# i2Nav-WHU/IC-GVINS

Measured on NVIDIA H100. Metric: frames/sec (KLT+BA) 1280x560 300-feat 10-KF window, higher is better.
Workload: dtype u8/int32 fixed point + f32 (KLT), f64 (BA)

## Files before the change

### ic_gvins_b200/_lib.py

```python
from __future__ import annotations

import ctypes as C
import os

_HERE = os.path.dirname(os.path.abspath(__file__))
LIB_PATH = os.path.join(_HERE, "libicgvins_b200_prof.so" if os.environ.get("ICG_LIB_VARIANT") == "prof" else "libicgvins_b200.so")

u8p = C.POINTER(C.c_uint8)
f32p = C.POINTER(C.c_float)
f64p = C.POINTER(C.c_double)
i32p = C.POINTER(C.c_int32)
vp = C.c_void_p

_lib = None


class IcgError(RuntimeError):
    pass


def lib() -> C.CDLL:
    global _lib
    if _lib is None:
        if not os.path.exists(LIB_PATH):
            raise IcgError(f"{LIB_PATH} not built: run `python -m ic_gvins_b200.build` (there is no CPU fallback)")
        _lib = C.CDLL(LIB_PATH, mode=C.RTLD_GLOBAL)
        _declare(_lib)
        _declare_r2(_lib)
    return _lib


def check(rc: int, what: str = "") -> None:
    if rc != 0:
        msg = lib().icg_last_error().decode("utf-8", "replace")
        raise IcgError(f"{what} failed with code {rc}: {msg}")


def _declare(L: C.CDLL) -> None:
    L.icg_last_error.restype = C.c_char_p
    L.icg_version.restype = C.c_int
    L.icg_launch_count.restype = C.c_uint64
    L.icg_launch_count_reset.restype = None
    L.icg_klt_create.argtypes = [C.POINTER(vp), C.c_int, C.c_int, C.c_int, C.c_int, C.c_int, vp]
    L.icg_klt_destroy.argtypes = [vp]
    L.icg_klt_destroy.restype = None
    L.icg_klt_calc_optical_flow_pyr_lk.argtypes = [vp, vp, vp, C.c_int, vp, vp, vp, vp, C.c_int, C.c_int, C.c_int, C.c_int,
                                                   C.c_double, C.c_int]
    L.icg_klt_track_fb.argtypes = [vp, vp, vp, C.c_int, vp, vp, vp, vp, C.c_int]
    L.icg_klt_upload.argtypes = [vp, C.c_int, vp, C.c_int]
    L.icg_klt_upload_level0.argtypes = [vp, C.c_int, vp, C.c_int]
    L.icg_klt_upload_batch.argtypes = [vp, C.c_int, C.c_int, vp, C.c_int]
    L.icg_klt_slot_level0.argtypes = [vp, C.c_int, C.POINTER(vp), C.POINTER(C.c_int)]
    L.icg_klt_slot_level.argtypes = [vp, C.c_int, C.c_int, C.POINTER(vp), C.POINTER(C.c_int), C.POINTER(C.c_int), C.POINTER(C.c_int)]
    L.icg_klt_build_pyramids.argtypes = [vp, C.c_int, C.c_int]
    L.icg_klt_track_batch_dev.argtypes = [vp, C.c_int, vp, vp, vp, vp, vp, vp, C.c_int]
    L.icg_klt_sync.argtypes = [vp]
    L.icg_klt_download_level.argtypes = [vp, C.c_int, C.c_int, vp, C.c_int]
    L.icg_detect_create.argtypes = [C.POINTER(vp), C.c_int, C.c_int, C.c_int, C.c_int, C.c_int, C.c_int, vp]
    L.icg_detect_destroy.argtypes = [vp]
    L.icg_detect_destroy.restype = None
    L.icg_detect_blocks.argtypes = [vp, vp, vp, C.c_int, C.c_int, vp, vp, C.c_double, C.c_double, C.c_int, vp, vp]
    L.icg_detect_blocks_dev.argtypes = [vp, C.c_int, vp, C.c_int, C.c_size_t, vp, C.c_int, vp, vp, C.c_double, C.c_double, C.c_int, vp, vp]
    L.icg_corner_subpix.argtypes = [vp, vp, C.c_int, vp, C.c_int]
    L.icg_detect_features.argtypes = [vp, vp, C.c_int, vp, C.c_int, vp, C.c_int, C.c_int, C.c_int, C.c_int, vp, vp]
    L.icg_detect_features_dev.argtypes = [vp, C.c_int, vp, C.c_int, C.c_size_t, vp, vp, vp, vp, vp, vp, vp, vp, C.c_int, vp, vp]
    L.icg_detect_mask_dev.argtypes = [vp, C.c_int, C.POINTER(vp), C.POINTER(C.c_int)]
    L.icg_camera_undistort_points.argtypes = [vp, vp, C.c_int]
    L.icg_camera_distort_points.argtypes = [vp, vp, C.c_int]
    L.icg_camera_distort_camera_points.argtypes = [vp, vp, vp, C.c_int]
    L.icg_camera_pixel2cam.argtypes = [vp, vp, vp, C.c_int]
    L.icg_camera_world2pixel.argtypes = [vp, vp, vp, vp, vp, C.c_int]
    L.icg_tracking_histogram.argtypes = [vp, C.c_int, C.c_int, C.c_int, vp]
    L.icg_triangulate_points.argtypes = [vp, vp, vp, vp, C.c_int, vp]
    L.icg_find_fundamental_mat_ransac.argtypes = [vp, vp, C.c_int, C.c_double, C.c_double, C.c_int, vp, vp]
    L.icg_clahe_create.argtypes = [C.POINTER(vp), C.c_int, C.c_int, C.c_int, C.c_int, C.c_double, C.c_int, vp]
    L.icg_clahe_destroy.argtypes = [vp]
    L.icg_clahe_destroy.restype = None
    L.icg_clahe_apply.argtypes = [vp, vp, C.c_int, vp, C.c_int]
    L.icg_clahe_apply_dev.argtypes = [vp, vp, C.c_int, vp, C.c_int]
    L.icg_clahe_sync.argtypes = [vp]
    L.icg_imu_preintegrate.argtypes = [vp, vp, vp, vp, vp, C.c_int, vp, vp]
    L.icg_ba_create.argtypes = [C.POINTER(vp), C.c_int, C.c_int, C.c_int, C.c_int, C.c_int, C.c_int, C.c_int, vp]
    L.icg_ba_destroy.argtypes = [vp]
    L.icg_ba_destroy.restype = None
    L.icg_ba_solve.argtypes = [vp, C.c_int, vp, C.c_int, vp]
    L.icg_ba_upload.argtypes = [vp, C.c_int, vp]
    L.icg_ba_run.argtypes = [vp, C.c_int, C.c_int]
    L.icg_ba_download.argtypes = [vp, C.c_int, vp, vp]
    L.icg_ba_sync.argtypes = [vp]
    L.icg_ba_shard_export.argtypes = [vp, C.c_int, C.c_int, vp]
    L.icg_ba_shard_connect.argtypes = [vp, vp]
    L.icg_ba_shard_error.argtypes = [vp]
    L.icg_ba_shard_leave.argtypes = [vp]
    L.icg_ba_gvins_optimization.argtypes = [vp, C.c_int, vp, C.c_int, vp, vp]
    L.icg_ba_run_gvins.argtypes = [vp, C.c_int, C.c_int]
    L.icg_ba_gvins_optimization_begin.argtypes = [vp, C.c_int, vp, C.c_int]
    L.icg_ba_gvins_optimization_end.argtypes = [vp, C.c_int, vp, vp, vp]
    L.icg_ba_residual_costs.argtypes = [vp, vp, vp, vp]
    L.icg_ba_reproj_evaluate.argtypes = [vp, vp, vp, vp, vp, vp, vp, C.c_double, vp, vp]
    L.icg_ba_imu_evaluate.argtypes = [vp, vp, vp, vp, vp, vp, vp, vp]
    L.icg_ba_marginalize.argtypes = [vp, C.c_int, vp, vp, vp]
    L.icg_ba_marginalize_resident.argtypes = [vp, C.c_int, vp, vp, vp]
    L.icg_ba_gnss_evaluate.argtypes = [vp, vp, vp, vp, vp, vp, vp]
    L.icg_ba_pose_prior_evaluate.argtypes = [vp, vp, vp, vp, vp, vp]
    L.icg_ba_mix_prior_evaluate.argtypes = [vp, vp, vp, vp, vp, vp]
    L.icg_ba_imu_error_evaluate.argtypes = [vp, vp, vp, vp]
    L.icg_ba_marg_factor_evaluate.argtypes = [vp, C.c_int, C.c_int, vp, vp, vp, vp, vp, vp, vp]


def _declare_r2(L: C.CDLL) -> None:
    L.icg_clahe_apply_batch_dev.argtypes = [vp, C.c_int, vp, C.c_int, C.c_size_t, vp, C.c_int, C.c_size_t, vp]
    L.icg_geom_create.argtypes = [C.POINTER(vp), C.c_int, vp]
    L.icg_geom_destroy.argtypes = [vp]
    L.icg_geom_destroy.restype = None
    L.icg_geom_undistort_points.argtypes = [vp, vp, vp, C.c_int]
    L.icg_geom_distort_points.argtypes = [vp, vp, vp, C.c_int]
    L.icg_geom_find_fundamental_mat_ransac.argtypes = [vp, vp, vp, C.c_int, C.c_double, C.c_double, C.c_int, vp, vp]
    L.icg_geom_triangulate_points.argtypes = [vp, vp, vp, vp, vp, C.c_int, vp]
    L.icg_geom_imu_preintegrate_batch.argtypes = [vp, C.c_int, vp, vp, vp, vp, vp, vp, vp, vp]
    L.icg_geom_find_fundamental_mat_ransac_batch.argtypes = [vp, C.c_int, vp, vp, vp, vp, vp, C.c_int, vp, vp, vp, vp]
    L.icg_klt_track_frames_dev.argtypes = [vp, C.c_int, vp, vp, vp, vp, vp, vp, vp, vp]
    L.icg_klt_track_frame.argtypes = [vp, vp, C.c_int, vp, C.c_int, vp, vp, vp, vp]
    L.icg_klt_triangulate_dev.argtypes = [vp, C.c_int, vp, vp, vp, vp, vp, C.c_int, vp, vp, vp]
    L.icg_klt_triangulate.argtypes = [vp, vp, C.c_int, vp, C.c_int, vp, vp, vp]
    L.icg_ba_update_and_cull_resident.argtypes = [vp, C.c_int, vp, vp, C.c_double, vp]
    L.icg_ba_marginalize_resident_culled.argtypes = [vp, C.c_int, vp, vp, vp, vp, vp]
    L.icg_ba_reintegrate_resident.argtypes = [vp, C.c_int, vp, vp, vp, vp]
    L.icg_ba_slide_resident.argtypes = [vp, C.c_int, vp, vp]
    L.icg_ba_slide_integrate_resident.argtypes = [vp, C.c_int, vp, vp, vp, vp, vp]


class SlideWindow(C.Structure):
    _fields_ = [("node_src", i32p), ("lm_src", i32p), ("f_src", i32p), ("imu_src", i32p), ("gnss_src", i32p), ("prior_from_marg", C.c_int32)]


SLIDE_CHAIN, SLIDE_ROW = -2, -3


class SlideIntegrate(C.Structure):
    _fields_ = [("imu_from", i32p), ("state16", f64p), ("gravity3", f64p), ("normal", u8p), ("imu", f64p), ("imu_off", i32p),
                ("node_from_imu", u8p), ("gnss_node", i32p), ("gnss_dt", f64p),
                ("status", C.POINTER(C.c_int8)), ("blob_out", f64p), ("end_state10", f64p)]


EXPORTS = [
    "icg_last_error", "icg_version", "icg_launch_count", "icg_launch_count_reset",
    "icg_klt_create", "icg_klt_destroy", "icg_klt_calc_optical_flow_pyr_lk", "icg_klt_track_fb", "icg_klt_upload",
    "icg_klt_upload_level0", "icg_klt_upload_batch", "icg_klt_slot_level0", "icg_klt_slot_level", "icg_klt_build_pyramids",
    "icg_klt_track_batch_dev", "icg_klt_sync", "icg_klt_download_level",
    "icg_detect_create", "icg_detect_destroy", "icg_detect_blocks", "icg_detect_blocks_dev", "icg_corner_subpix",
    "icg_detect_features", "icg_detect_features_dev", "icg_detect_mask_dev",
    "icg_camera_undistort_points", "icg_camera_distort_points", "icg_camera_distort_camera_points", "icg_camera_pixel2cam", "icg_camera_world2pixel", "icg_tracking_histogram", "icg_find_fundamental_mat_ransac", "icg_triangulate_points",
    "icg_clahe_create", "icg_clahe_destroy", "icg_clahe_apply", "icg_clahe_apply_dev", "icg_clahe_apply_batch_dev", "icg_geom_create", "icg_geom_destroy", "icg_geom_undistort_points", "icg_geom_distort_points", "icg_geom_find_fundamental_mat_ransac", "icg_geom_triangulate_points", "icg_geom_imu_preintegrate_batch", "icg_clahe_sync",
    "icg_geom_find_fundamental_mat_ransac_batch", "icg_klt_track_frames_dev", "icg_klt_track_frame",
    "icg_klt_triangulate_dev", "icg_klt_triangulate",
    "icg_imu_preintegrate", "icg_ba_create", "icg_ba_destroy", "icg_ba_solve", "icg_ba_upload", "icg_ba_run", "icg_ba_download",
    "icg_ba_sync", "icg_ba_shard_export", "icg_ba_shard_connect", "icg_ba_shard_error", "icg_ba_shard_leave", "icg_ba_gvins_optimization", "icg_ba_run_gvins", "icg_ba_gvins_optimization_begin", "icg_ba_gvins_optimization_end", "icg_ba_residual_costs", "icg_ba_reproj_evaluate", "icg_ba_imu_evaluate", "icg_ba_marginalize", "icg_ba_marginalize_resident", "icg_ba_update_and_cull_resident", "icg_ba_marginalize_resident_culled", "icg_ba_reintegrate_resident", "icg_ba_slide_resident", "icg_ba_slide_integrate_resident", "icg_ba_gnss_evaluate", "icg_ba_pose_prior_evaluate", "icg_ba_mix_prior_evaluate", "icg_ba_imu_error_evaluate", "icg_ba_marg_factor_evaluate",
]
```

### ic_gvins_b200/csrc/ba.cu

```cuda
#include <cooperative_groups.h>
#include <unistd.h>
#include <math.h>
#include <stdlib.h>
#include <string.h>

#include <algorithm>
#include <string>
#include <thread>
#include <vector>

#include "ba_cull.cuh"
#include "ba_slide.cuh"
#include "preint.cuh"
#include "ba_math.cuh"
#include "common.cuh"
#include "geom_core.cuh"

namespace icg {
using namespace bam;
namespace cg = cooperative_groups;

constexpr int BA_SPLIT_W = 4;
constexpr int BA_CHOL_NB = 8;
constexpr int BA_MARG_MAXB = 72;
constexpr int BA_MAX_NODES = 32;

struct BaCaps {
    int NW, K, L, F, G, R;
    int NCV, N, NS, NCA, RJ, LP, NVB;
    int GQ;
};

struct WinDims {
    int K, L, F, n_imu, n_gnss, marg_r, marg_nb;
    int ext_const, td_const, reproj_huber, gnss_huber, has_imu_error, has_pose_prior, has_mix_prior;
    double reproj_sinv;
};

struct LmState {
    double radius, decrease_factor, x_cost, x_norm, cand_cost, model_cost_change, step_norm, gmax, initial_cost;
    double cost_cam[2];
    int iter, n_success, n_invalid, done, need_lin, last_success, first, step_valid, fresh_lin, max_iter, chol_ok;
    int lin_buf;
};

struct ShardDev {
    int split;
    int PK, BS, RV;
    double *peer[8];
    size_t off_inbox, off_bcast, off_scal, off_flagA, off_flagB, off_flagC;
    double *redv;
    int *err;
    double *slm;
    int *slm_cnt;
};

struct BaDev {
    ShardDev S;
    WinDims *dims;
    LmState *st;
    double *pose, *mix, *ext, *rho;
    double *pose_c, *mix_c, *ext_c, *rho_c;
    double *pose_0, *mix_0, *ext_0, *rho_0;
    uint8_t *f_active_0;
    double *gnss_std_0;
    uint8_t *f_active;
    int *lm_off;
    int *lm_perm;
    int *vb_lm0;
    int *ref_nrun;
    int *f_meta_s;
    double *f_const_s;
    int *vis_ord;
    int *part_off, *pair_ro, *npairs;
    double *gpart;
    int *vis_cnt;
    double *Mp[2];
    double *AW[2];
    double *costf[2];
    double *hl[2], *gl[2];
    double *Hc[2], *gc[2];
    double *scale_l, *scale_c;
    double *Hs;
    double *visv;
    double *imu_blob, *imu_U;
    int *gnss_node;
    double *gnss_blh, *gnss_std, *lever;
    double *pose_prior, *pose_prior_sinfo, *mix_prior, *mix_prior_std;
    int *marg_type, *marg_node;
    double *marg_x0, *marg_H0, *marg_b0, *marg_c0;
    double *cost_part;
    double *red2;
    int rank, world;
    double *step_c, *step_l;
    double *Sglobal;
    unsigned long long *clk;
};

__device__ __forceinline__ double *lin_Mp(const BaCaps &C, const BaDev &D, int b, int w) { return D.Mp[b] + (size_t) w * C.K * (C.K - 1) * 210; }
__device__ __forceinline__ double *lin_AW(const BaCaps &C, const BaDev &D, int b, int w) { return D.AW[b] + (size_t) w * C.LP * C.NCA; }
__device__ __forceinline__ double *lin_costf(const BaCaps &C, const BaDev &D, int b, int w) { return D.costf[b] + (size_t) w * C.F; }
__device__ __forceinline__ double *lin_hl(const BaCaps &C, const BaDev &D, int b, int w) { return D.hl[b] + (size_t) w * C.L; }
__device__ __forceinline__ double *lin_gl(const BaCaps &C, const BaDev &D, int b, int w) { return D.gl[b] + (size_t) w * C.L; }
__device__ __forceinline__ double *lin_Hc(const BaCaps &C, const BaDev &D, int b, int w) { return D.Hc[b] + (size_t) w * C.NS * C.NS; }
__device__ __forceinline__ double *lin_gc(const BaCaps &C, const BaDev &D, int b, int w) { return D.gc[b] + (size_t) w * C.NS; }

__device__ __forceinline__ int col_pose(int k) { return 6 * k; }
__device__ __forceinline__ int col_ext(int K) { return 6 * K; }
__device__ __forceinline__ int col_td(int K) { return 6 * K + 6; }
__device__ __forceinline__ int col_mix(int K, int k) { return 6 * K + 7 + 9 * k; }

__device__ __forceinline__ int jc_off(int a) { return a < 18 ? (a / 6) * 12 + (a % 6) : 36 + 2 * (a - 18); }
__device__ __forceinline__ int jc_row1(int a) { return a < 18 ? 6 : 1; }
__device__ __forceinline__ int tri20(int la, int lb) {
    return la * 20 - la * (la - 1) / 2 + (lb - la);
}
__device__ __forceinline__ void dmma884(double &c0, double &c1, double a, double b) {
    asm volatile("mma.sync.aligned.m8n8k4.row.col.f64.f64.f64.f64 {%0,%1}, {%2}, {%3}, {%0,%1};" : "+d"(c0), "+d"(c1) : "d"(a), "d"(b));
}
constexpr int LV_LD = 45;
constexpr size_t LV_SMEM = sizeof(double) * (128 * LV_LD + (BA_MAX_NODES + 1) * NODE_FRAME_LD);
__global__ void __launch_bounds__(128, 4) ba_lin_vis(BaCaps C, BaDev D, int at_cand) {
    extern __shared__ double lv_sm[];
    __shared__ int s_ord[128], s_gbeg[BA_MAX_NODES], s_gend[BA_MAX_NODES], s_last, s_p0, s_np;
    double (*s_rec)[LV_LD] = (double (*)[LV_LD]) lv_sm;
    double (*s_frame)[NODE_FRAME_LD] = (double (*)[NODE_FRAME_LD]) (lv_sm + 128 * LV_LD);
    const int w = blockIdx.y;
    const LmState &st = D.st[w];
    if (st.done || !(at_cand ? st.step_valid : st.need_lin)) return;
    const int b = at_cand ? 1 - st.lin_buf : st.lin_buf;
    const double *pose = at_cand ? D.pose_c : D.pose, *xext = at_cand ? D.ext_c : D.ext, *rho = at_cand ? D.rho_c : D.rho;
    const int *vb = D.vb_lm0 + (size_t) w * C.NVB;
    if ((int) blockIdx.x >= vb[C.NVB - 1]) return;
    const WinDims dm = D.dims[w];
    const int tid = threadIdx.x;
    const int *off = D.lm_off + (size_t) w * (C.L + 1);
    const int pA = vb[blockIdx.x], pB = vb[blockIdx.x + 1];
    const int s0 = off[pA], nslot = off[pB] - s0;
    if (tid <= dm.K) node_frame(tid < dm.K ? pose + ((size_t) w * C.K + tid) * 7 : xext + (size_t) w * 8, s_frame[tid]);
    if (tid < BA_MAX_NODES) s_gbeg[tid] = s_gend[tid] = 0;
    if (tid == 0) s_np = 0;
    __syncthreads();
    if (tid < nslot) {
        const int q = s0 + tid;
        double r[2], Ji[12], Jj[12], Je[12], Jr[2], Jt[2], cost = 0;
        const int4 meta = ((const int4 *) D.f_meta_s)[(size_t) w * C.F + q];
        const int i = meta.y, j = meta.z, f = meta.w;
        if (D.f_active[(size_t) w * C.F + f] != 0) {
            const double *ext = xext + (size_t) w * 8;
            reproj_eval_frames(s_frame[i], s_frame[j], s_frame[dm.K], rho[(size_t) w * C.L + meta.x], ext[7],
                               D.f_const_s + ((size_t) w * C.F + q) * 14, dm.reproj_sinv, true, r, Ji, Jj, Je, Jr, Jt);
            if (dm.ext_const)
                for (int k = 0; k < 12; k++) Je[k] = 0;
            if (dm.td_const) Jt[0] = Jt[1] = 0;
            double sq = r[0] * r[0] + r[1] * r[1], sc = 1.0;
            if (dm.reproj_huber)
                huber(sq, cost, sc);
            else
                cost = 0.5 * sq;
            if (sc != 1.0) {
                for (int k = 0; k < 12; k++) Ji[k] *= sc, Jj[k] *= sc, Je[k] *= sc;
                Jr[0] *= sc, Jr[1] *= sc, Jt[0] *= sc, Jt[1] *= sc, r[0] *= sc, r[1] *= sc;
            }
        } else {
            for (int k = 0; k < 12; k++) Ji[k] = Jj[k] = Je[k] = 0;
            Jr[0] = Jr[1] = Jt[0] = Jt[1] = r[0] = r[1] = 0;
        }
        lin_costf(C, D, b, w)[f] = cost;
        double *sr = s_rec[tid];
#pragma unroll
        for (int k = 0; k < 12; k++) sr[k] = Ji[k], sr[12 + k] = Jj[k], sr[24 + k] = Je[k];
        sr[36] = Jt[0], sr[37] = Jt[1], sr[38] = r[0], sr[39] = r[1];
        sr[40] = Jr[0], sr[41] = Jr[1], sr[42] = (double) j, sr[43] = (double) i;
    }
    __syncthreads();
    const int lane = tid & 31, warp = tid >> 5;
    if (nslot > 0) {
        if (tid < nslot) {
            const int *ord = D.vis_ord + (size_t) w * C.F + s0;
            const int v = ord[tid], ob = (int) s_rec[v & 255][42];
            s_ord[tid] = v;
            if (tid == 0 || (int) s_rec[ord[tid - 1] & 255][42] != ob) s_gbeg[ob] = tid;
            if (tid == nslot - 1 || (int) s_rec[ord[tid + 1] & 255][42] != ob) s_gend[ob] = tid + 1;
        }
        __syncthreads();
        const int kk = lane & 3, g = lane >> 2;
        int o[3];
#pragma unroll
        for (int t = 0; t < 3; t++) {
            const int a = 8 * t + g;
            o[t] = a < 20 ? jc_off(a) + (kk & 1) * jc_row1(a) : -1;
        }
        for (int ob = warp; ob < dm.K; ob += 4) {
            const int beg = s_gbeg[ob], end = s_gend[ob];
            if (beg == end) continue;
            double c00[2] = {0, 0}, c01[2] = {0, 0}, c02[2] = {0, 0}, c11[2] = {0, 0}, c12[2] = {0, 0}, c22[2] = {0, 0};
            constexpr int UNR = 2;
            for (int base = beg; base < end; base += 2 * UNR) {
                double x[UNR][3];
#pragma unroll
                for (int u = 0; u < UNR; u++) {
                    const int q = base + 2 * u + (kk >> 1);
                    const bool ok = q < end;
                    const double *rec = s_rec[ok ? s_ord[q] & 255 : 0];
#pragma unroll
                    for (int t = 0; t < 3; t++) x[u][t] = (ok && o[t] >= 0) ? rec[o[t]] : 0.0;
                }
#pragma unroll
                for (int u = 0; u < UNR; u++) {
                    dmma884(c00[0], c00[1], x[u][0], x[u][0]);
                    dmma884(c01[0], c01[1], x[u][0], x[u][1]);
                    dmma884(c02[0], c02[1], x[u][0], x[u][2]);
                    dmma884(c11[0], c11[1], x[u][1], x[u][1]);
                    dmma884(c12[0], c12[1], x[u][1], x[u][2]);
                    dmma884(c22[0], c22[1], x[u][2], x[u][2]);
                }
            }
            double *pp = D.gpart + ((size_t) w * C.GQ + (s_ord[beg] >> 8)) * 210;
            auto put = [&](int ti, int tj, const double *c) {
#pragma unroll
                for (int e = 0; e < 2; e++) {
                    const int la = 8 * ti + g, lb = 8 * tj + 2 * kk + e;
                    if (la <= lb && lb < 20) pp[tri20(la, lb)] = c[e];
                }
            };
            put(0, 0, c00), put(0, 1, c01), put(0, 2, c02), put(1, 1, c11), put(1, 2, c12), put(2, 2, c22);
        }
        __threadfence();
    }
    const int *perm = D.lm_perm + (size_t) w * C.L;
    const int K = dm.K, NCV = 6 * K + 7, NCA = 4 * ((NCV + 1 + 3) / 4);
    const int grp = tid >> 3, sl = tid & 7;
    int o0[3], o1[3];
#pragma unroll
    for (int t = 0; t < 3; t++) {
        const int c = sl + 8 * t;
        o0[t] = c < 19 ? jc_off(c) : 38, o1[t] = c < 19 ? o0[t] + jc_row1(c) : 39;
    }
    for (int pl = pA + grp; pl < pB; pl += 16) {
        const int l = perm[pl], f0 = off[pl] - s0, nf = off[pl + 1] - off[pl];
        double *row = lin_AW(C, D, b, w) + (size_t) l * C.NCA;
        for (int c = sl; c < NCA; c += 8) row[c] = 0.0;
        __syncwarp(0xffu << (tid & 24));
        double acc[3] = {0, 0, 0};
        for (int q = 0; q < nf; q++) {
            const double *rec = s_rec[f0 + q];
            const double r0 = rec[40], r1 = rec[41];
            const int ob = (int) rec[42];
#pragma unroll
            for (int t = 0; t < 3; t++) {
                const int c = sl + 8 * t;
                if (c == 20) {
                    acc[t] += r0 * r0 + r1 * r1;
                } else if (c < 20) {
                    const double v = rec[o0[t]] * r0 + rec[o1[t]] * r1;
                    if (c >= 6 && c < 12)
                        row[col_pose(ob) + c - 6] = v;
                    else
                        acc[t] += v;
                }
            }
        }
        const int ref = nf > 0 ? (int) s_rec[f0][43] : 0;
#pragma unroll
        for (int t = 0; t < 3; t++) {
            const int c = sl + 8 * t;
            if (nf > 0) {
                if (c < 6) row[col_pose(ref) + c] = acc[t];
                else if (c >= 12 && c < 18) row[col_ext(K) + c - 12] = acc[t];
                else if (c == 18) row[col_td(K)] = acc[t];
            }
            if (c == 19) {
                row[NCV] = acc[t];
                lin_gl(C, D, b, w)[l] = acc[t];
            } else if (c == 20) {
                lin_hl(C, D, b, w)[l] = acc[t];
                if (st.first) D.scale_l[(size_t) w * C.L + l] = 1.0 / (1.0 + sqrt(acc[t]));
            }
        }
    }
    if (nslot == 0) return;
    const int rn = (int) s_rec[0][43];
    __syncthreads();
    if (tid == 0) s_last = atomicAdd(D.vis_cnt + (size_t) w * C.K + rn, 1) == D.ref_nrun[(size_t) w * C.K + rn] - 1;
    __syncthreads();
    if (!s_last) return;
    __threadfence();
    if (tid == 0) D.vis_cnt[(size_t) w * C.K + rn] = 0;
    const int PM = C.K * (C.K - 1), P = D.npairs[w];
    const int *pro = D.pair_ro + (size_t) w * PM, *poff = D.part_off + (size_t) w * (PM + 1);
    for (int p = tid; p < P; p += 128)
        if ((pro[p] >> 8) == rn) {
            atomicAdd(&s_np, 1);
            if (p == 0 || (pro[p - 1] >> 8) != rn) s_p0 = p;
        }
    __syncthreads();
    const double *part = D.gpart + (size_t) w * C.GQ * 210;
    double *Mp = lin_Mp(C, D, b, w);
    for (int p = s_p0 + warp; p < s_p0 + s_np; p += 4) {
        const int k0 = poff[p], k1 = poff[p + 1];
        double acc[7];
#pragma unroll
        for (int j = 0; j < 7; j++) acc[j] = lane + 32 * j < 210 ? __ldcg(part + (size_t) k0 * 210 + lane + 32 * j) : 0.0;
        for (int k = k0 + 1; k < k1; k++) {
            double v[7];
#pragma unroll
            for (int j = 0; j < 7; j++) v[j] = lane + 32 * j < 210 ? __ldcg(part + (size_t) k * 210 + lane + 32 * j) : 0.0;
#pragma unroll
            for (int j = 0; j < 7; j++) acc[j] += v[j];
        }
#pragma unroll
        for (int j = 0; j < 7; j++)
            if (lane + 32 * j < 210) Mp[(size_t) p * 210 + lane + 32 * j] = acc[j];
    }
}


__device__ __forceinline__ void gram2_slots(const BaCaps &C, const BaDev &D, int w, int K, short *s_slot) {
    const int PM = C.K * (C.K - 1), P = D.npairs[w];
    const int *pro = D.pair_ro + (size_t) w * PM;
    for (int e = threadIdx.x; e < K * K; e += blockDim.x) s_slot[e] = -1;
    __syncthreads();
    for (int p = threadIdx.x; p < P; p += blockDim.x) s_slot[(pro[p] >> 8) * K + (pro[p] & 255)] = (short) p;
    __syncthreads();
}
__device__ __forceinline__ double gram2_entry(const BaCaps &C, const BaDev &D, int buf, int w, int K, const short *s_slot, int A, int B) {
    const int P = D.npairs[w];
    const double *Mp = lin_Mp(C, D, buf, w);
    const int bA = A < 6 * K ? A / 6 : K, bB = B < 6 * K ? B / 6 : K;
    const int a = A - 6 * bA, b = B - 6 * bB;
    const int ga = 12 + a, gb = 12 + b;
    double sum = 0;
    if (bA == K) {
        const int idx = tri20(ga, gb);
        double s4[4] = {0, 0, 0, 0};
        int p = 0;
        for (; p + 16 <= P; p += 16) {
            double v[16];
#pragma unroll
            for (int u = 0; u < 16; u++) v[u] = Mp[(size_t) (p + u) * 210 + idx];
#pragma unroll
            for (int u = 0; u < 16; u++) s4[u & 3] += v[u];
        }
        for (; p < P; p++) s4[p & 3] += Mp[(size_t) p * 210 + idx];
        sum = (s4[0] + s4[1]) + (s4[2] + s4[3]);
    } else if (bB == K || bB == bA) {
        const int i1 = tri20(a, bB == K ? gb : b), i2 = tri20(6 + a, bB == K ? gb : 6 + b);
        for (int o0 = 0; o0 < K; o0 += 8) {
            double v1[8], v2[8];
#pragma unroll
            for (int u = 0; u < 8; u++) {
                const int o = o0 + u;
                const int p1 = o < K ? s_slot[bA * K + o] : -1, p2 = o < K ? s_slot[o * K + bA] : -1;
                v1[u] = p1 >= 0 ? Mp[(size_t) p1 * 210 + i1] : 0.0;
                v2[u] = p2 >= 0 ? Mp[(size_t) p2 * 210 + i2] : 0.0;
            }
#pragma unroll
            for (int u = 0; u < 8; u++) sum += v1[u], sum += v2[u];
        }
    } else {
        const int p1 = s_slot[bA * K + bB], p2 = s_slot[bB * K + bA];
        if (p1 >= 0) sum += Mp[(size_t) p1 * 210 + tri20(a, 6 + b)];
        if (p2 >= 0) sum += Mp[(size_t) p2 * 210 + tri20(b, 6 + a)];
    }
    return sum;
}

__device__ __forceinline__ double block_sum(double v, double *s_red);
__device__ __forceinline__ double block_max(double v, double *s_red);
__device__ __forceinline__ double *x_inbox(const BaDev &D, int peer, int w, int from);
__device__ __forceinline__ int tri_idx(int A, int B, int ncv);

__device__ __forceinline__ void schur_store(const BaCaps &C, const BaDev &D, int buf, int w, int K, const short *s_slot, int A, int B, double cw) {
    const int NCV = 6 * K + 7;
    if (A == NCV) return;
    const size_t e = (size_t) w * C.NS * C.NS + (size_t) B * C.NS + A;
    const double hc = !D.S.split && B < NCV ? lin_Hc(C, D, buf, w)[(size_t) B * C.NS + A] : 0.0;
    const double cj = gram2_entry(C, D, buf, w, K, s_slot, A, B);
    if (D.S.split) {
        double *P = x_inbox(D, w % D.world, w, D.rank);
        const int TRI = NCV * (NCV + 1) / 2;
        if (B < NCV) {
            P[tri_idx(A, B, NCV)] = cj - cw;
            if (A == B) P[TRI + A] = cj;
        } else {
            P[TRI + NCV + A] = cj;
            P[TRI + 2 * NCV + A] = cw;
        }
    } else {
        double *V = D.visv + (size_t) w * 3 * C.NCV;
        if (B < NCV) {
            D.Hs[e] = hc + (cj - cw);
            if (A == B) V[A] = cj;
        } else {
            V[NCV + A] = cj, V[2 * NCV + A] = cw;
        }
    }
}

__device__ __forceinline__ void schur_scalars(const BaCaps &C, const BaDev &D, int w, const WinDims &dm, double *s_red) {
    const int tid = threadIdx.x;
    double c = 0, q = 0, gm = 0;
    const double *costf = lin_costf(C, D, 0, w), *gl = lin_gl(C, D, 0, w);
    for (int f = tid; f < dm.F; f += 256) c += costf[f];
    for (int l = tid; l < dm.L; l += 256) {
        const double r = D.rho[(size_t) w * C.L + l];
        q += r * r;
        gm = fmax(gm, fabs(gl[l]));
    }
    c = block_sum(c, s_red);
    q = block_sum(q, s_red);
    gm = block_max(gm, s_red);
    if (tid != 0) return;
    const int NCV = 6 * dm.K + 7, TRI = NCV * (NCV + 1) / 2;
    double *P = x_inbox(D, w % D.world, w, D.rank);
    P[TRI + 3 * NCV] = c, P[TRI + 3 * NCV + 1] = q, P[TRI + 3 * NCV + 2] = gm;
}

constexpr int SCHUR_RCH = 80;
constexpr int SCHUR_PASS = 16;
__global__ void __cluster_dims__(BA_SPLIT_W, 1, 1) __launch_bounds__(256) ba_schur_dmma(BaCaps C, BaDev D, int ld) {
    extern __shared__ double sA[];
    __shared__ short s_slot[32 * 32];
    __shared__ double s_red[40];
    cg::cluster_group cluster = cg::this_cluster();
    const int w = blockIdx.y, split = blockIdx.x;
    const LmState &st = D.st[w];
    if (st.done) return;
    const WinDims dm = D.dims[w];
    const int NCV = 6 * dm.K + 7, NCA = 4 * ((NCV + 1 + 3) / 4);
    const int T2 = (NCA + 15) / 16, nsuper = T2 * (T2 + 1) / 2;
    const int tid = threadIdx.x, lane = tid & 31, warp = tid >> 5, g = lane >> 2, kk = lane & 3;
    double *sphi = sA + (size_t) SCHUR_RCH * ld;
    const int b = st.lin_buf;
    const double *A = lin_AW(C, D, b, w), *hl = lin_hl(C, D, b, w);
    const double radius = st.radius;
    const int nsteps = (dm.L + 3) / 4;
    const int r_beg = 4 * (int) ((long long) nsteps * split / BA_SPLIT_W), r_end = min(dm.L, 4 * (int) ((long long) nsteps * (split + 1) / BA_SPLIT_W));
    const int npass = (nsuper + SCHUR_PASS - 1) / SCHUR_PASS;
    gram2_slots(C, D, w, dm.K, s_slot);
    for (int pass = 0; pass < npass; pass++) {
        if (pass > 0) cluster.barrier_wait();
        int si[2], sj[2];
        bool on[2];
#pragma unroll
        for (int h2 = 0; h2 < 2; h2++) {
            const int su = (2 * pass + h2) * 8 + warp;
            on[h2] = su < nsuper;
            int a = 0, e = on[h2] ? su : 0;
            while (e >= T2 - a) e -= T2 - a, a++;
            si[h2] = a, sj[h2] = a + e;
        }
        double acc[2][4][2];
#pragma unroll
        for (int h2 = 0; h2 < 2; h2++)
#pragma unroll
            for (int q = 0; q < 4; q++) acc[h2][q][0] = acc[h2][q][1] = 0;
        for (int r0 = r_beg; r0 < r_end; r0 += SCHUR_RCH) {
            const int nr = min(SCHUR_RCH, r_end - r0), nr4 = (nr + 3) & ~3;
            __syncthreads();
            for (int rb = warp; rb < nr4; rb += 8 * 4) {
                double v[4][3];
#pragma unroll
                for (int u = 0; u < 4; u++) {
                    const int rr = rb + 8 * u;
#pragma unroll
                    for (int cchunk = 0; cchunk < 3; cchunk++) {
                        const int c = lane + 32 * cchunk;
                        v[u][cchunk] = (rr < nr && c < NCA) ? A[(size_t) (r0 + rr) * C.NCA + c] : 0.0;
                    }
                }
#pragma unroll
                for (int u = 0; u < 4; u++) {
                    const int rr = rb + 8 * u;
#pragma unroll
                    for (int cchunk = 0; cchunk < 3; cchunk++) {
                        const int c = lane + 32 * cchunk;
                        if (rr < nr4 && c < ld) sA[(size_t) rr * ld + c] = v[u][cchunk];
                    }
                }
                for (int c = lane + 96; c < ld; c += 32)
                    for (int u = 0; u < 4; u++) {
                        const int rr = rb + 8 * u;
                        if (rr < nr4) sA[(size_t) rr * ld + c] = (rr < nr && c < NCA) ? A[(size_t) (r0 + rr) * C.NCA + c] : 0.0;
                    }
            }
            for (int rr = tid; rr < nr4; rr += 256) {
                double ph = 0;
                if (rr < nr) {
                    const int l = r0 + rr;
                    const double sl = D.scale_l[(size_t) w * C.L + l], hs = sl * sl * hl[l];
                    ph = sl * sl / (hs + fmin(fmax(hs, 1e-6), 1e32) / radius);
                }
                sphi[rr] = ph;
            }
            __syncthreads();
            for (int ks = 0; ks < nr4 / 4; ks++) {
                const double *row = sA + (size_t) (4 * ks + kk) * ld;
                const double ph = sphi[4 * ks + kk];
#pragma unroll
                for (int h2 = 0; h2 < 2; h2++) {
                    if (!on[h2]) continue;
                    const double xb0 = row[16 * sj[h2] + g], xb1 = row[16 * sj[h2] + 8 + g];
                    const double a0 = row[16 * si[h2] + g] * ph, a1 = row[16 * si[h2] + 8 + g] * ph;
                    dmma884(acc[h2][0][0], acc[h2][0][1], a0, xb0);
                    dmma884(acc[h2][1][0], acc[h2][1][1], a0, xb1);
                    dmma884(acc[h2][2][0], acc[h2][2][1], a1, xb0);
                    dmma884(acc[h2][3][0], acc[h2][3][1], a1, xb1);
                }
            }
        }
        __syncthreads();
#pragma unroll
        for (int h2 = 0; h2 < 2; h2++) {
            if (!on[h2]) continue;
#pragma unroll
            for (int q = 0; q < 4; q++)
#pragma unroll
                for (int e = 0; e < 2; e++) sA[(h2 * 8 + warp) * 256 + 64 * q + 32 * e + lane] = acc[h2][q][e];
        }
        cluster.sync();
        const int nslot = min(SCHUR_PASS, nsuper - SCHUR_PASS * pass);
        double cw[SCHUR_PASS / BA_SPLIT_W];
#pragma unroll
        for (int j = 0; j < SCHUR_PASS / BA_SPLIT_W; j++) {
            const int sl = split + BA_SPLIT_W * j;
            double p[BA_SPLIT_W];
#pragma unroll
            for (int k = 0; k < BA_SPLIT_W; k++) p[k] = sl < nslot ? cluster.map_shared_rank(sA, k)[sl * 256 + tid] : 0.0;
            cw[j] = 0;
#pragma unroll
            for (int k = 0; k < BA_SPLIT_W; k++) cw[j] += p[k];
        }
        cluster.barrier_arrive();
        const int q = tid >> 6, r_in = 8 * (q >> 1) + ((tid & 31) >> 2), c_in = 8 * (q & 1) + 2 * (tid & 3) + ((tid >> 5) & 1);
#pragma unroll
        for (int j = 0; j < SCHUR_PASS / BA_SPLIT_W; j++) {
            const int sl = split + BA_SPLIT_W * j;
            if (sl >= nslot) break;
            int a = 0, e = SCHUR_PASS * pass + sl;
            while (e >= T2 - a) e -= T2 - a, a++;
            const int r = 16 * a + r_in, cc = 16 * (a + e) + c_in;
            if (r <= cc && cc <= NCV) schur_store(C, D, b, w, dm.K, s_slot, r, cc, cw[j]);
        }
    }
    if (split == 0 && D.S.split) schur_scalars(C, D, w, dm, s_red);
    cluster.barrier_wait();
}

constexpr double IMU_GB_STD = 7200 / 3600.0 * 3.14159265358979323846 / 180.0;
constexpr double IMU_AB_STD = 2.0e4 * 1.0e-5;

__device__ void imu_factor_warp(const double *blob, const double *U, const double *pose0, const double *mix0, const double *pose1,
                                const double *mix1, bool want_j, double *rw, double *Jw, int lane) {
    __shared__ ImuMid s_mid[16];
    double *raw_r = rw + 15;
    const int wslot = (threadIdx.x >> 5) & 15;
    if (want_j)
        for (int e = lane; e < 450; e += 32) Jw[e] = 0;
    __syncwarp();
    if (lane == 0) {
        ImuMid M;
        imu_residual_raw(blob, pose0, mix0, pose1, mix1, raw_r, M);
        if (want_j) imu_jacobian_raw(blob, M, Jw);
        s_mid[wslot] = M;
    }
    __syncwarp();
    if (want_j && lane < 30) {
        for (int i = 0; i < 15; i++) {
            double s = 0;
            for (int k = i; k < 15; k++) s += U[i * 15 + k] * Jw[k * 30 + lane];
            Jw[i * 30 + lane] = s;
        }
    }
    if (lane < 15) {
        double s = 0;
        for (int k = lane; k < 15; k++) s += U[lane * 15 + k] * raw_r[k];
        rw[lane] = s;
    }
    __syncwarp();
}

__device__ void marg_dx(const BaCaps &C, const BaDev &D, int w, const WinDims &dm, const double *pose, const double *mix, const double *ext, double *dx,
                        int *colmap, int tid, int nthreads) {
    const int *type = D.marg_type + (size_t) w * BA_MARG_MAXB, *node = D.marg_node + (size_t) w * BA_MARG_MAXB;
    const double *x0 = D.marg_x0 + (size_t) w * BA_MARG_MAXB * 9;
    if (tid == 0) {
        int col = 0, xo = 0;
        for (int b = 0; b < dm.marg_nb; b++) {
            int t = type[b], nd = node[b];
            if (t == 0 || t == 2) {
                const double *x = t == 0 ? pose + nd * 7 : ext;
                const double *xl = x0 + xo;
                Q dq = qmul(qinv(pose_q(xl)), pose_q(x));
                V3 a = 2.0 * qv(dq);
                if (dq.w < 0) a = -a;
                for (int k = 0; k < 3; k++) dx[col + k] = x[k] - xl[k];
                dx[col + 3] = a.x, dx[col + 4] = a.y, dx[col + 5] = a.z;
                int base = t == 0 ? col_pose(nd) : col_ext(dm.K);
                for (int k = 0; k < 6; k++) colmap[col + k] = (t == 2 && dm.ext_const) ? -1 : base + k;
                col += 6, xo += 7;
            } else if (t == 1) {
                for (int k = 0; k < 9; k++) dx[col + k] = mix[nd * 9 + k] - x0[xo + k], colmap[col + k] = col_mix(dm.K, nd) + k;
                col += 9, xo += 9;
            } else {
                dx[col] = ext[7] - x0[xo];
                colmap[col] = dm.td_const ? -1 : col_td(dm.K);
                col += 1, xo += 1;
            }
        }
    }
}

__device__ __forceinline__ void red_add(double *p, double v) { asm volatile("red.global.add.f64 [%0], %1;" ::"l"(p), "d"(v) : "memory"); }

__device__ double cam_factors(const BaCaps &C, const BaDev &D, int w, const WinDims &dm, const double *pose, const double *mix, const double *ext,
                              bool lin, int b, double *smem) {
// ... 672 lines not shown
    const LmState &st = D.st[w];
    if (st.done || !st.step_valid) return;
    const WinDims dm = D.dims[w];
    const double *pose = D.pose_c + (size_t) w * C.K * 7, *ext = D.ext_c + (size_t) w * 8, *rho = D.rho_c + (size_t) w * C.L;
    double *part = D.cost_part + (size_t) w * (nblk_vis + 1);
    const int q = blockIdx.x * 256 + threadIdx.x;
    __shared__ double s_frame[BA_MAX_NODES + 1][NODE_FRAME_LD];
    if ((int) threadIdx.x <= dm.K) node_frame((int) threadIdx.x < dm.K ? pose + threadIdx.x * 7 : ext, s_frame[threadIdx.x]);
    __syncthreads();
    double cost = 0;
    int4 meta = make_int4(0, 0, 0, 0);
    if (q < dm.F) meta = ((const int4 *) D.f_meta_s)[(size_t) w * C.F + q];
    if (q < dm.F && D.f_active[(size_t) w * C.F + meta.w]) {
        double r[2];
        reproj_eval_frames(s_frame[meta.y], s_frame[meta.z], s_frame[dm.K], rho[meta.x], ext[7], D.f_const_s + ((size_t) w * C.F + q) * 14, dm.reproj_sinv,
                           false, r, nullptr, nullptr, nullptr, nullptr, nullptr);
        double sq = r[0] * r[0] + r[1] * r[1], sc;
        if (dm.reproj_huber)
            huber(sq, cost, sc);
        else
            cost = 0.5 * sq;
    }
    cost = block_sum(cost, s_red);
    if (threadIdx.x == 0) part[blockIdx.x] = cost;
}

__global__ void __launch_bounds__(128) ba_accept(BaCaps C, BaDev D) {
    __shared__ int s_accept;
    __shared__ double s_camsq, s_rhosq;
    __shared__ double s_red[40];
    const int w = blockIdx.x, tid = threadIdx.x;
    LmState &st = D.st[w];
    if (st.done) return;
    const WinDims dm = D.dims[w];
    const double *R2 = D.red2 + (size_t) w * 4;
    {
        const double *pose = D.pose + (size_t) w * C.K * 7, *mix = D.mix + (size_t) w * C.K * 9, *ext = D.ext + (size_t) w * 8;
        double s = 0;
        for (int e = tid; e < dm.K * 7; e += 128) s += pose[e] * pose[e];
        for (int e = tid; e < dm.K * 9; e += 128) s += mix[e] * mix[e];
        if (tid < 7 && !dm.ext_const) s += ext[tid] * ext[tid];
        if (tid == 7 && !dm.td_const) s += ext[7] * ext[7];
        s = block_sum(s, s_red);
        double q = 0;
        for (int l = tid; l < dm.L; l += 128) q += D.rho[(size_t) w * C.L + l] * D.rho[(size_t) w * C.L + l];
        q = block_sum(q, s_red);
        if (tid == 0) s_camsq = s, s_rhosq = q;
    }
    extern __shared__ double s_warp[];
    const int lane = tid & 31, warp = tid >> 5, ngrp = (dm.F + 31) / 32;
    if (st.step_valid) {
        const double *costf = lin_costf(C, D, 1 - st.lin_buf, w);
        const int4 *meta = (const int4 *) D.f_meta_s + (size_t) w * C.F;
#pragma unroll 4
        for (int g = warp; g < ngrp; g += 4) {
            const int q = 32 * g + lane;
            double v = q < dm.F ? costf[meta[q].w] : 0.0;
            for (int o = 16; o > 0; o >>= 1) v += __shfl_down_sync(0xffffffffu, v, o);
            if (lane == 0) s_warp[g] = v;
        }
    }
    __syncthreads();
    if (tid == 0) {
        s_accept = 0;
        const double mcc = R2[0], sn = R2[1], nfin = R2[2];
        double cand = 0;
        if (st.step_valid) {
            for (int g0 = 0; g0 < ngrp; g0 += 8) {
                double t = 0;
                for (int k = 0; k < 8; k++) t += g0 + k < ngrp ? s_warp[g0 + k] : 0.0;
                cand += t;
            }
            cand += st.cost_cam[1 - st.lin_buf];
        }
        if (!st.chol_ok || nfin != 0.0 || !(mcc > 0.0)) {
            st.step_valid = 0;
            st.n_invalid++;
            if (st.n_invalid >= 5) st.done = 3;
            st.radius *= 0.5;
            st.last_success = 0;
        } else {
            st.n_invalid = 0;
            st.model_cost_change = mcc;
            st.step_norm = sqrt(sn);
            st.x_norm = sqrt(s_camsq + s_rhosq);
            st.cand_cost = cand;
            if (st.step_norm <= 1e-8 * (st.x_norm + 1e-8)) {
                st.done = 2;
            } else if (fabs(st.x_cost - cand) <= 1e-6 * st.x_cost) {
                st.done = 2;
            } else {
                const double rel = (st.x_cost - cand) / mcc;
                if (rel > 1e-3) {
                    s_accept = 1;
                    st.n_success++;
                    double t = 2.0 * rel - 1.0;
                    st.radius = fmin(1e16, st.radius / fmax(1.0 / 3.0, 1.0 - t * t * t));
                    st.decrease_factor = 2.0;
                    st.last_success = 1;
                    st.fresh_lin = 1;
                    st.lin_buf ^= 1;
                } else {
                    st.radius = st.radius / st.decrease_factor;
                    st.decrease_factor *= 2.0;
                    st.last_success = 0;
                    st.need_lin = 0;
                }
            }
        }
    }
    __syncthreads();
    if (!s_accept) return;
    double *pose = D.pose + (size_t) w * C.K * 7, *mix = D.mix + (size_t) w * C.K * 9, *ext = D.ext + (size_t) w * 8, *rho = D.rho + (size_t) w * C.L;
    const double *pose_c = D.pose_c + (size_t) w * C.K * 7, *mix_c = D.mix_c + (size_t) w * C.K * 9, *ext_c = D.ext_c + (size_t) w * 8, *rho_c = D.rho_c + (size_t) w * C.L;
    for (int e = tid; e < dm.K * 7; e += 128) pose[e] = pose_c[e];
    for (int e = tid; e < dm.K * 9; e += 128) mix[e] = mix_c[e];
    if (tid < 8) ext[tid] = ext_c[tid];
    for (int e = tid; e < dm.L; e += 128) rho[e] = rho_c[e];
}

__global__ void ba_reset_state(BaDev D, LmState *save, int n, int max_iter) {
    int w = blockIdx.x * blockDim.x + threadIdx.x;
    if (w >= n) return;
    if (save) save[w] = D.st[w];
    LmState st;
    memset(&st, 0, sizeof(st));
    st.radius = 1e4, st.decrease_factor = 2.0;
    st.need_lin = 1, st.fresh_lin = 1, st.first = 1, st.last_success = 1, st.max_iter = max_iter;
    D.st[w] = st;
}

__global__ void __launch_bounds__(128) ba_chi2_cull(BaCaps C, BaDev D, int *counters) {
    const int w = blockIdx.y;
    WinDims &dm = D.dims[w];
    const int t = blockIdx.x * 128 + threadIdx.x;
    const double *pose = D.pose + (size_t) w * C.K * 7, *ext = D.ext + (size_t) w * 8, *rho = D.rho + (size_t) w * C.L;
    int4 meta = make_int4(0, 0, 0, 0);
    if (t < dm.F) meta = ((const int4 *) D.f_meta_s)[(size_t) w * C.F + t];
    if (t < dm.F && D.f_active[(size_t) w * C.F + meta.w]) {
        double r[2];
        reproj_eval(pose + meta.y * 7, pose + meta.z * 7, ext, rho[meta.x], ext[7], D.f_const_s + ((size_t) w * C.F + t) * 14, dm.reproj_sinv, false, r, nullptr,
                    nullptr, nullptr, nullptr, nullptr);
        if ((r[0] * r[0] + r[1] * r[1]) > 5.991) {
            D.f_active[(size_t) w * C.F + meta.w] = 0;
            atomicAdd(&counters[2 * w], 1);
        }
    }
    if (t < dm.n_gnss) {
        double r[3];
        double *sd = D.gnss_std + ((size_t) w * C.G + t) * 3;
        gnss_eval(pose + D.gnss_node[(size_t) w * C.G + t] * 7, D.gnss_blh + ((size_t) w * C.G + t) * 3, sd, D.lever + (size_t) w * 3, false, r, nullptr);
        double chi2 = r[0] * r[0] + r[1] * r[1] + r[2] * r[2];
        if (chi2 > 7.815) {
            double sc = sqrt(chi2 / 7.815);
            sd[0] *= sc, sd[1] *= sc, sd[2] *= sc;
            atomicAdd(&counters[2 * w + 1], 1);
        }
    }
}
__global__ void ba_set_gnss_huber(BaDev D, int n, int v) {
    int w = blockIdx.x * blockDim.x + threadIdx.x;
    if (w < n) D.dims[w].gnss_huber = v;
}

__global__ void ba_residual_costs_kernel(BaCaps C, BaDev D, double *reproj_cost, double *gnss_cost) {
    const int w = 0;
    const WinDims dm = D.dims[w];
    const int t = blockIdx.x * blockDim.x + threadIdx.x;
    const double *pose = D.pose, *ext = D.ext, *rho = D.rho;
    if (t < dm.F) {
        double r[2];
        const int4 meta = ((const int4 *) D.f_meta_s)[t];
        reproj_eval(pose + meta.y * 7, pose + meta.z * 7, ext, rho[meta.x], ext[7], D.f_const_s + (size_t) t * 14, dm.reproj_sinv, false, r, nullptr, nullptr,
                    nullptr, nullptr, nullptr);
        reproj_cost[meta.w] = 0.5 * (r[0] * r[0] + r[1] * r[1]);
    }
    if (t < dm.n_gnss) {
        double r[3];
        gnss_eval(pose + D.gnss_node[t] * 7, D.gnss_blh + t * 3, D.gnss_std + t * 3, D.lever, false, r, nullptr);
        gnss_cost[t] = 0.5 * (r[0] * r[0] + r[1] * r[1] + r[2] * r[2]);
    }
}

__global__ void ba_reproj_eval_kernel(const double *in , double *out ) {
    double r[2], Ji[12], Jj[12], Je[12], Jr[2], Jt[2];
    reproj_eval(in, in + 7, in + 14, in[22], in[23], in + 24, 1.0 / in[38], true, r, Ji, Jj, Je, Jr, Jt);
    out[0] = r[0], out[1] = r[1];
    double *o = out + 2;
    const double *src[3] = {Ji, Jj, Je};
    for (int b = 0; b < 3; b++)
        for (int rr = 0; rr < 2; rr++) {
            for (int c = 0; c < 6; c++) o[b * 14 + rr * 7 + c] = src[b][rr * 6 + c];
            o[b * 14 + rr * 7 + 6] = 0.0;
        }
    o[42] = Jr[0], o[43] = Jr[1], o[44] = Jt[0], o[45] = Jt[1];
}

__global__ void ba_imu_eval_kernel(const double *blob, const double *U, const double *x , double *out ) {
    __shared__ double s_buf[480];
    imu_factor_warp(blob, U, x, x + 7, x + 16, x + 23, true, s_buf, s_buf + 30, threadIdx.x);
    for (int e = threadIdx.x; e < 15; e += 32) out[e] = s_buf[e];
    for (int e = threadIdx.x; e < 450; e += 32) out[15 + e] = s_buf[30 + e];
}

__global__ void ba_small_factor_eval_kernel(int kind, const double *in, double *out) {
    if (kind == 0) {
        gnss_eval(in, in + 7, in + 10, in + 13, true, out, out + 3);
    } else if (kind == 1) {
        pose_prior_eval(in, in + 7, in + 14, true, out, out + 6);
    } else if (kind == 2) {
        for (int k = 0; k < 9; k++) out[k] = (in[k] - in[9 + k]) / in[18 + k], out[9 + k] = 1.0 / in[18 + k];
    } else {
        for (int k = 0; k < 3; k++) {
            out[k] = in[3 + k] / IMU_GB_STD, out[3 + k] = in[6 + k] / IMU_AB_STD;
            out[6 + k] = 1.0 / IMU_GB_STD, out[9 + k] = 1.0 / IMU_AB_STD;
        }
    }
}

__global__ void ba_marg_factor_eval_kernel(const double *in, double *out) {
    extern __shared__ double s_dx[];
    const int r = (int) in[0], nb = (int) in[1];
    const double *types = in + 2;
    int tot = 0;
    for (int b = 0; b < nb; b++) tot += ((int) types[b] == 1) ? 9 : ((int) types[b] == 3) ? 1 : 7;
    const double *x = types + nb, *x0 = x + tot, *e0 = x0 + tot, *J0 = e0 + r;
    if (threadIdx.x == 0) {
        int col = 0, xo = 0;
        for (int b = 0; b < nb; b++) {
            const int t = (int) types[b];
            if (t == 0 || t == 2) {
                Q dq = qmul(qinv(pose_q(x0 + xo)), pose_q(x + xo));
                V3 a = 2.0 * qv(dq);
                if (dq.w < 0) a = -a;
                for (int k = 0; k < 3; k++) s_dx[col + k] = x[xo + k] - x0[xo + k];
                s_dx[col + 3] = a.x, s_dx[col + 4] = a.y, s_dx[col + 5] = a.z;
                col += 6, xo += 7;
            } else {
                const int g = t == 1 ? 9 : 1;
                for (int k = 0; k < g; k++) s_dx[col + k] = x[xo + k] - x0[xo + k];
                col += g, xo += g;
            }
        }
    }
    __syncthreads();
    for (int i = threadIdx.x; i < r; i += blockDim.x) {
        double sum = e0[i];
        for (int k = 0; k < r; k++) sum += J0[(size_t) i * r + k] * s_dx[k];
        out[i] = sum;
    }
}

}

#include "ba_split.cuh"
#include "ba_marg.cuh"

using namespace icg;

namespace {
bool host_imu_sqrt_info(const double *cov, double *U) {
    double work[675];
    return gc::imu_sqrt_info(cov, U, work);
}

template <typename T>
struct HostDev {
    T *h = nullptr, *d = nullptr;
    size_t n = 0;
    int alloc(size_t count) {
        n = count;
        if (cudaMallocHost(&h, sizeof(T) * count) != cudaSuccess) return ICG_ENOMEM;
        if (cudaMalloc(&d, sizeof(T) * count) != cudaSuccess) return ICG_ENOMEM;
        memset(h, 0, sizeof(T) * count);
        return ICG_OK;
    }
    void release() {
        if (h) cudaFreeHost(h);
        if (d) cudaFree(d);
        h = d = nullptr;
    }
    cudaError_t up(cudaStream_t s, size_t count = 0) { return cudaMemcpyAsync(d, h, sizeof(T) * (count ? count : n), cudaMemcpyHostToDevice, s); }
    cudaError_t down(cudaStream_t s, size_t count = 0) { return cudaMemcpyAsync(h, d, sizeof(T) * (count ? count : n), cudaMemcpyDeviceToHost, s); }
};
}

struct icg_ba {
    BaCaps C;
    BaDev D;
    int device = 0;
    cudaStream_t stream = nullptr;
    cudaStream_t stream_cam = nullptr;
    cudaEvent_t ev_fork = nullptr, ev_join = nullptr;
    bool own_stream = false;
    int nblk_vis = 0;
    int cur_windows = 0;
    size_t smem_cam, smem_solve, smem_schur;
    int ld_schur;
    int use_global_S;
    HostDev<WinDims> dims;
    HostDev<LmState> st;
    HostDev<double> pose, mix, ext, rho, imu_blob, imu_U, gnss_blh, gnss_std, lever, pose_prior, pose_prior_sinfo, mix_prior, mix_prior_std, marg_x0,
        marg_H0, marg_b0, marg_c0;
    HostDev<int> f_meta_s, vb_lm0, ref_nrun;
    HostDev<double> f_const_s;
    HostDev<int> lm_off, lm_perm, lm_fidx, gnss_node, marg_type, marg_node, part_off, pair_ro, vis_ord, npairs;
    HostDev<uint8_t> f_active;
    std::vector<void *> dev_only;
    HostDev<double> scratch;
    HostDev<LmState> st_save;
    HostDev<int> cull_counters;
    double *xbuf = nullptr;
    size_t xbuf_doubles = 0;
    int x_world = 0;
    void *ipc_opened[8] = {nullptr, nullptr, nullptr, nullptr, nullptr, nullptr, nullptr, nullptr};
    unsigned long long epoch = 0;
    size_t smem_solve_cam = 0, smem_step_lm = 0;
    bool solve_cam_dsm = false;
    size_t smem_solve_cam_dsm = 0;
    bool prof = false;
    std::vector<cudaEvent_t> prof_ev;
    std::vector<int> prof_tag;
    size_t prof_used = 0;
    int prof_skip = 1;
    double prof_ms[16] = {0};
    long prof_cnt[16] = {0};
    bool marg_ready = false;
    MargDev M{};
    int marg_nw = 0;
    int marg_cluster_ok = -1;
    HostDev<int> marg_map;
    HostDev<double> marg_oJ0, marg_oe0, marg_oHp, marg_obp;
    HostDev<uint8_t> marg_fmask;
    unsigned char *cull_h = nullptr, *cull_d = nullptr;
    size_t cull_cap = 0;
    unsigned char *reint_h = nullptr, *reint_d = nullptr;
    size_t reint_cap = 0;
    int marg_res_n = 0;
    std::vector<int> marg_res_m, marg_res_r, marg_res_nb;
    unsigned char *slide_h = nullptr, *slide_d = nullptr;
    size_t slide_cap = 0;
    double *slide_old = nullptr, *fc_alt = nullptr;
    cudaEvent_t slide_ev = nullptr;
};

extern "C" {
static void prof_collect(icg_ba *h);
static void prof_print(icg_ba *h);
}

static int dmalloc(icg_ba *h, double **p, size_t n) {
    if (cudaMalloc(p, sizeof(double) * n) != cudaSuccess) {
        set_error("icg_ba_create: cudaMalloc of %zu doubles failed", n);
        return ICG_ENOMEM;
    }
    cudaMemsetAsync(*p, 0, sizeof(double) * n, h->stream);
    h->dev_only.push_back(*p);
    return ICG_OK;
}

static int cam_threads(const icg_ba *h) { return h->D.world >= 4 ? CAM_THREADS : 160; }

extern "C" {
static int split_setup(icg_ba *h, int rank, int world);
static void split_release(icg_ba *h);

int icg_imu_preintegrate(const double *state16, const double *iewn3, const double *gravity3, const double *noise5, const double *imu, int n, double *blob,
                         double *end_state10) {
    if (!state16 || !gravity3 || !noise5 || !imu || !blob || n < 1) {
        set_error("icg_imu_preintegrate: bad arguments");
        return ICG_EINVAL;
    }
    gc::preintegrate_core(state16, iewn3, gravity3, noise5, imu, n, blob, end_state10);
    return ICG_OK;
}

static int ba_create_body(icg_ba *h, int max_windows, int max_K, int max_L, int max_F, int max_gnss, int max_marg_r, void *stream);

int icg_ba_create(icg_ba **out, int max_windows, int max_K, int max_L, int max_F, int max_gnss, int max_marg_r, int device, void *stream) {
    if (!out || max_windows < 1 || max_K < 2 || max_K > 32 || max_L < 0 || max_F < 0 || max_gnss < 0 || max_marg_r < 0) {
        set_error("icg_ba_create: bad arguments");
        return ICG_EINVAL;
    }
    int ndev = 0;
    if (cudaGetDeviceCount(&ndev) != cudaSuccess || ndev == 0) {
        set_error("icg_ba_create: no CUDA device (this library has no CPU fallback)");
        return ICG_ENODEVICE;
    }
    if (device < 0 || device >= ndev) {
        set_error("icg_ba_create: device %d out of range", device);
        return ICG_EINVAL;
    }
    ICG_CUDA(cudaSetDevice(device));
    cudaDeviceProp prop;
    ICG_CUDA(cudaGetDeviceProperties(&prop, device));
    if (prop.major != 9 || prop.minor != 0) {
        set_error("icg_ba_create: device is sm_%d%d; this library is built for sm_90a only", prop.major, prop.minor);
        return ICG_ENODEVICE;
    }
    icg_ba *h = new icg_ba();
    h->device = device;
    const int rc_init = ba_create_body(h, max_windows, max_K, max_L, max_F, max_gnss, max_marg_r, stream);
    if (rc_init != ICG_OK) {
        icg_ba_destroy(h);
        return rc_init;
    }
    *out = h;
    return ICG_OK;
}

static int ba_create_body(icg_ba *h, int max_windows, int max_K, int max_L, int max_F, int max_gnss, int max_marg_r, void *stream) {
    if (stream) {
        h->stream = (cudaStream_t) stream;
    } else {
        ICG_CUDA(cudaStreamCreateWithFlags(&h->stream, cudaStreamNonBlocking));
        h->own_stream = true;
    }
    {
        int prio_lo = 0, prio_hi = 0;
        ICG_CUDA(cudaDeviceGetStreamPriorityRange(&prio_lo, &prio_hi));
        ICG_CUDA(cudaStreamCreateWithPriority(&h->stream_cam, cudaStreamNonBlocking, prio_hi));
    }
    ICG_CUDA(cudaEventCreateWithFlags(&h->ev_fork, cudaEventDisableTiming));
    ICG_CUDA(cudaEventCreateWithFlags(&h->ev_join, cudaEventDisableTiming));
    h->prof = getenv("ICG_BA_PROFILE") != nullptr;
    if (h->prof) {
        double *ck = nullptr;
        if (dmalloc(h, &ck, 48) != ICG_OK) return ICG_ENOMEM;
        h->D.clk = (unsigned long long *) ck;
    }
    if (getenv("ICG_BA_PROFILE_SKIP")) h->prof_skip = atoi(getenv("ICG_BA_PROFILE_SKIP"));
    BaCaps &C = h->C;
    max_L = std::max(1, max_L), max_F = std::max(1, max_F);
    C.NW = max_windows, C.K = max_K, C.L = max_L, C.F = max_F, C.G = std::max(1, max_gnss), C.R = std::max(1, max_marg_r);
    C.NCV = 6 * max_K + 7, C.N = 15 * max_K + 7, C.NS = (C.N + 3) & ~3, C.NCA = 4 * ((C.NCV + 1 + 3) / 4);
    C.RJ = (2 * max_F + 31) & ~31, C.LP = (max_L + 31) & ~31;
    C.NVB = (max_F + 127 - max_K) / (128 - max_K) + max_L / 128 + 4 + max_K;
    C.GQ = std::max(1, std::min(max_F, (C.NVB - 2) * (max_K - 1)));
    h->nblk_vis = (max_F + 255) / 256;
    const size_t NW = max_windows;
#define HD(field, count)                                                       \
    if (h->field.alloc(count) != ICG_OK) {                                     \
        set_error("icg_ba_create: allocation of " #field " failed");           \
        return ICG_ENOMEM;                                                     \
    }
    HD(dims, NW) HD(st, NW) HD(pose, NW * C.K * 7) HD(mix, NW * C.K * 9) HD(ext, NW * 8) HD(rho, NW * C.L)
    HD(imu_blob, NW * C.K * ICG_IMU_BLOB_DOUBLES) HD(imu_U, NW * C.K * 225) HD(gnss_blh, NW * C.G * 3) HD(gnss_std, NW * C.G * 3) HD(lever, NW * 3)
    HD(pose_prior, NW * 7) HD(pose_prior_sinfo, NW * 6) HD(mix_prior, NW * 9) HD(mix_prior_std, NW * 9) HD(marg_x0, NW * BA_MARG_MAXB * 9)
    HD(marg_H0, NW * C.R * C.R) HD(marg_b0, NW * C.R) HD(marg_c0, NW)
    HD(lm_off, NW * (C.L + 1)) HD(lm_perm, NW * C.L) HD(lm_fidx, NW * C.F) HD(gnss_node, NW * C.G) HD(marg_type, NW * BA_MARG_MAXB) HD(marg_node, NW * BA_MARG_MAXB) HD(f_active, NW * C.F)
    HD(scratch, 1024) HD(st_save, NW) HD(cull_counters, 2 * NW) HD(f_meta_s, NW * C.F * 4) HD(vb_lm0, NW * C.NVB) HD(ref_nrun, NW * C.K) HD(f_const_s, NW * C.F * 14)
    HD(part_off, NW * ((size_t) C.K * (C.K - 1) + 1)) HD(pair_ro, NW * (size_t) C.K * (C.K - 1)) HD(vis_ord, NW * C.F) HD(npairs, NW)
#undef HD
    ICG_CUDA(cudaMemsetAsync(h->st.d, 0, sizeof(LmState) * NW, h->stream));
    BaDev &D = h->D;
    D.rank = 0, D.world = 1;
    D.dims = h->dims.d, D.st = h->st.d, D.pose = h->pose.d, D.mix = h->mix.d, D.ext = h->ext.d, D.rho = h->rho.d;
    D.f_active = h->f_active.d;
    D.part_off = h->part_off.d, D.pair_ro = h->pair_ro.d, D.vis_ord = h->vis_ord.d, D.npairs = h->npairs.d;
    D.f_meta_s = h->f_meta_s.d, D.vb_lm0 = h->vb_lm0.d, D.ref_nrun = h->ref_nrun.d, D.f_const_s = h->f_const_s.d;
    D.lm_off = h->lm_off.d, D.lm_perm = h->lm_perm.d, D.imu_blob = h->imu_blob.d, D.imu_U = h->imu_U.d;
    D.gnss_node = h->gnss_node.d, D.gnss_blh = h->gnss_blh.d, D.gnss_std = h->gnss_std.d, D.lever = h->lever.d;
    D.pose_prior = h->pose_prior.d, D.pose_prior_sinfo = h->pose_prior_sinfo.d, D.mix_prior = h->mix_prior.d, D.mix_prior_std = h->mix_prior_std.d;
    D.marg_type = h->marg_type.d, D.marg_node = h->marg_node.d, D.marg_x0 = h->marg_x0.d, D.marg_H0 = h->marg_H0.d, D.marg_b0 = h->marg_b0.d, D.marg_c0 = h->marg_c0.d;
    int rc = ICG_OK;
#define DM(field, count) \
    if (rc == ICG_OK) rc = dmalloc(h, &D.field, count);
    DM(pose_c, NW * C.K * 7) DM(mix_c, NW * C.K * 9) DM(ext_c, NW * 8) DM(rho_c, NW * C.L)
    DM(pose_0, NW * C.K * 7) DM(mix_0, NW * C.K * 9) DM(ext_0, NW * 8) DM(rho_0, NW * C.L)
    DM(AW[0], NW * C.NCA * C.LP) DM(Mp[0], NW * (size_t) C.K * (C.K - 1) * 210) DM(visv, NW * 3 * C.NCV)
    DM(gpart, NW * (size_t) C.GQ * 210) DM(costf[0], NW * C.F) DM(hl[0], NW * C.L) DM(gl[0], NW * C.L) DM(scale_l, NW * C.L) DM(scale_c, NW * C.NS)
    DM(Hc[0], NW * C.NS * C.NS) DM(gc[0], NW * C.NS) DM(Hs, NW * C.NS * C.NS) DM(cost_part, NW * (h->nblk_vis + 1)) DM(red2, NW * 4) DM(step_c, NW * C.NS) DM(step_l, NW * C.L)
#undef DM
    if (rc == ICG_OK) rc = dmalloc(h, &D.gnss_std_0, NW * C.G * 3);
    if (rc == ICG_OK) {
        double *cnt = nullptr;
        rc = dmalloc(h, &cnt, (NW * C.K + 1) / 2);
        D.vis_cnt = (int *) cnt;
    }
    if (rc == ICG_OK) {
        double *fa0 = nullptr;
        rc = dmalloc(h, &fa0, (NW * C.F + 7) / 8 + 1);
        D.f_active_0 = (uint8_t *) fa0;
    }
    if (rc != ICG_OK) return rc;
    h->smem_cam = sizeof(double) * ((size_t) C.K * 480 + (size_t) C.G * 24 + 48 + 16 + 2 * (size_t) C.R + 8) + sizeof(int) * (size_t) C.R + 64;
    size_t vec = sizeof(double) * (40 + 5 * (size_t) C.NS);
    size_t packed = sizeof(double) * ((size_t) (C.N + 1) * (C.N + 2) / 2);
    h->use_global_S = (vec + packed > 220 * 1024) ? 1 : 0;
    h->smem_solve = vec + (h->use_global_S ? 0 : packed);
    D.Sglobal = nullptr;
    memset(&D.S, 0, sizeof(D.S));
    if (h->use_global_S) {
        rc = split_setup(h, 0, 1);
        if (rc != ICG_OK) return rc;
    } else {
        ICG_CUDA(raise_dynamic_smem((const void *) ba_solve, (size_t) (h->smem_solve)));
    }
    h->ld_schur = 16 * ((C.NCA + 15) / 16) + 8;
    h->smem_schur = sizeof(double) * std::max((size_t) SCHUR_RCH * h->ld_schur + SCHUR_RCH, (size_t) SCHUR_PASS * 256);
    ICG_CUDA(raise_dynamic_smem((const void *) ba_schur_dmma, (size_t) (h->smem_schur)));
    ICG_CUDA(cudaFuncSetAttribute(ba_schur_dmma, cudaFuncAttributePreferredSharedMemoryCarveout, cudaSharedmemCarveoutMaxShared));
    ICG_CUDA(raise_dynamic_smem((const void *) ba_lin_cam, (size_t) (h->smem_cam)));
    ICG_CUDA(raise_dynamic_smem((const void *) ba_cost_cam, (size_t) (h->smem_cam)));
    ICG_CUDA(raise_dynamic_smem((const void *) ba_lin_vis, LV_SMEM));
    ICG_CUDA(cudaStreamSynchronize(h->stream));
    h->cur_windows = 0;
    return ICG_OK;
}

void icg_ba_destroy(icg_ba *h) {
    if (!h) return;
    cudaSetDevice(h->device);
    if (h->stream) cudaStreamSynchronize(h->stream);
    prof_collect(h);
    prof_print(h);
    for (cudaEvent_t e : h->prof_ev) cudaEventDestroy(e);
    h->dims.release(), h->st.release(), h->pose.release(), h->mix.release(), h->ext.release(), h->rho.release();
    h->imu_blob.release(), h->imu_U.release(), h->gnss_blh.release(), h->gnss_std.release(), h->lever.release(), h->pose_prior.release();
    h->pose_prior_sinfo.release(), h->mix_prior.release(), h->mix_prior_std.release(), h->marg_x0.release(), h->marg_H0.release(), h->marg_b0.release();
    h->marg_c0.release(), h->lm_off.release(), h->lm_perm.release(), h->lm_fidx.release(), h->gnss_node.release();
    h->f_meta_s.release(), h->vb_lm0.release(), h->ref_nrun.release(), h->f_const_s.release(), h->marg_type.release(), h->marg_node.release(), h->f_active.release(), h->scratch.release(), h->st_save.release(), h->cull_counters.release(), h->part_off.release(), h->pair_ro.release(), h->vis_ord.release(), h->npairs.release();
    split_release(h);
    if (h->marg_ready) h->marg_map.release(), h->marg_oJ0.release(), h->marg_oe0.release(), h->marg_oHp.release(), h->marg_obp.release(), h->marg_fmask.release();
    for (double *p : {h->M.H0, h->M.b0, h->M.G1, h->M.V1, h->M.lam1, h->M.Z})
        if (p) cudaFree(p);
    if (h->cull_h) cudaFreeHost(h->cull_h);
    if (h->cull_d) cudaFree(h->cull_d);
    if (h->reint_h) cudaFreeHost(h->reint_h);
    if (h->reint_d) cudaFree(h->reint_d);
    if (h->slide_h) cudaFreeHost(h->slide_h);
    if (h->slide_d) cudaFree(h->slide_d);
    if (h->slide_old) cudaFree(h->slide_old);
    if (h->fc_alt) cudaFree(h->fc_alt);
    if (h->slide_ev) cudaEventDestroy(h->slide_ev);
    for (void *p : h->dev_only) cudaFree(p);
    if (h->stream_cam) cudaStreamSynchronize(h->stream_cam), cudaStreamDestroy(h->stream_cam);
    if (h->ev_fork) cudaEventDestroy(h->ev_fork);
    if (h->ev_join) cudaEventDestroy(h->ev_join);
    if (h->own_stream && h->stream) cudaStreamDestroy(h->stream);
    delete h;
}

#define PK_FAIL(code, ...)                          \
    do {                                            \
        char eb_[512];                              \
        snprintf(eb_, sizeof(eb_), __VA_ARGS__);    \
        err = eb_;                                  \
        return code;                                \
    } while (0)
static int pack_window(icg_ba *h, int w, const icg_ba_problem &p, bool values, std::string &err) {
        const BaCaps &C = h->C;
        if (p.K < 2 || p.K > C.K || p.L < 0 || p.L > C.L || p.F < 0 || p.F > C.F || p.n_imu < 0 || p.n_imu > p.K - 1 || p.n_gnss < 0 || p.n_gnss > C.G ||
            p.marg_r < 0 || p.marg_r > C.R || p.marg_nblocks < 0 || p.marg_nblocks > 2 * C.K + 2 || !p.pose || !p.mix || !p.ext || (p.L > 0 && !p.invdepth) ||
            (p.F > 0 && (!p.f_lm || !p.f_ref || !p.f_obs || !p.f_const))) {
            PK_FAIL(ICG_EINVAL, "icg_ba_upload: window %d exceeds the handle's capacity or has null parameter arrays (K=%d L=%d F=%d gnss=%d marg_r=%d)", w, p.K, p.L, p.F,
                      p.n_gnss, p.marg_r);
        }
        WinDims &d = h->dims.h[w];
        d.K = p.K, d.L = p.L, d.F = p.F, d.n_imu = p.n_imu, d.n_gnss = p.n_gnss, d.marg_r = p.marg_r, d.marg_nb = p.marg_nblocks;
        d.ext_const = p.ext_const != 0, d.td_const = p.td_const != 0, d.reproj_huber = p.reproj_huber != 0, d.gnss_huber = p.gnss_huber != 0;
        d.has_imu_error = p.has_imu_error != 0, d.has_pose_prior = p.has_pose_prior != 0, d.has_mix_prior = p.has_mix_prior != 0;
        d.reproj_sinv = 1.0 / p.reproj_std;
        if (values) {
            memcpy(h->pose.h + (size_t) w * C.K * 7, p.pose, sizeof(double) * 7 * p.K);
            memcpy(h->mix.h + (size_t) w * C.K * 9, p.mix, sizeof(double) * 9 * p.K);
        }
        memcpy(h->ext.h + (size_t) w * 8, p.ext, sizeof(double) * 8);
        if (values && p.L > 0) memcpy(h->rho.h + (size_t) w * C.L, p.invdepth, sizeof(double) * p.L);
        for (int f = 0; f < p.F; f++) {
            if (p.f_lm[f] < 0 || p.f_lm[f] >= p.L || p.f_ref[f] < 0 || p.f_ref[f] >= p.K || p.f_obs[f] < 0 || p.f_obs[f] >= p.K || p.f_ref[f] == p.f_obs[f]) {
                PK_FAIL(ICG_EINVAL, "icg_ba_upload: window %d factor %d has invalid indices", w, f);
            }
        }
        std::vector<int> refof(p.L, -1);
        {
            std::vector<unsigned> seen((size_t) p.L, 0u);
            for (int f = 0; f < p.F; f++) {
                const int l = p.f_lm[f];
                if (refof[l] < 0) refof[l] = p.f_ref[f];
                if (refof[l] != p.f_ref[f] || (seen[l] >> p.f_obs[f]) & 1u) {
                    PK_FAIL(ICG_EINVAL, "icg_ba_upload: window %d factor %d: landmark %d has two reference nodes or two observations in node %d", w, f, l, p.f_obs[f]);
                }
                seen[l] |= 1u << p.f_obs[f];
            }
        }
        if (p.f_active)
            memcpy(h->f_active.h + (size_t) w * C.F, p.f_active, p.F);
        else
            memset(h->f_active.h + (size_t) w * C.F, 1, p.F);
        int *perm = h->lm_perm.h + (size_t) w * C.L;
        std::vector<int> pos_of(p.L);
        {
            std::vector<int> kcur(p.K + 2, 0);
            for (int l = 0; l < p.L; l++) kcur[(refof[l] < 0 ? p.K : refof[l]) + 1]++;
            for (int k = 0; k <= p.K; k++) kcur[k + 1] += kcur[k];
            for (int l = 0; l < p.L; l++) pos_of[l] = kcur[refof[l] < 0 ? p.K : refof[l]]++, perm[pos_of[l]] = l;
        }
        int *off = h->lm_off.h + (size_t) w * (C.L + 1), *fidx = h->lm_fidx.h + (size_t) w * C.F;
        for (int l = 0; l <= p.L; l++) off[l] = 0;
        for (int f = 0; f < p.F; f++) off[pos_of[p.f_lm[f]] + 1]++;
        for (int l = 0; l < p.L; l++) off[l + 1] += off[l];
        int *vbh = h->vb_lm0.h + (size_t) w * C.NVB, *meta = h->f_meta_s.h + (size_t) w * C.F * 4;
        int nrun = 0;
        {
            std::vector<int> cur(off, off + p.L);
            for (int f = 0; f < p.F; f++) fidx[cur[pos_of[p.f_lm[f]]]++] = f;
            int *nrun_of = h->ref_nrun.h + (size_t) w * C.K;
            for (int k = 0; k < C.K; k++) nrun_of[k] = 0;
            int l0 = 0;
            while (l0 < p.L) {
                const int ref = refof[perm[l0]];
                int l1 = l0;
                while (l1 < p.L && refof[perm[l1]] == ref && off[l1 + 1] - off[l0] <= 128) l1++;
                if (l1 == l0 || nrun >= C.NVB - 2) PK_FAIL(ICG_EINVAL, "icg_ba_upload: window %d: landmark %d has more than 128 factors or the run table overflows", w, perm[l0]);
                if (ref >= 0) nrun_of[ref]++;
                vbh[nrun++] = l0;
                l0 = l1;
            }
            vbh[nrun] = p.L;
            vbh[C.NVB - 1] = nrun;
            double *fcs = h->f_const_s.h + (size_t) w * C.F * 14;
            for (int q = 0; q < p.F; q++) {
                const int f = fidx[q];
                meta[4 * q] = p.f_lm[f], meta[4 * q + 1] = p.f_ref[f], meta[4 * q + 2] = p.f_obs[f], meta[4 * q + 3] = f;
                if (values) memcpy(fcs + (size_t) q * 14, p.f_const + (size_t) f * 14, sizeof(double) * 14);
            }
        }
        {
            const int PM = C.K * (C.K - 1);
            int *poff = h->part_off.h + (size_t) w * (PM + 1), *pro = h->pair_ro.h + (size_t) w * PM, *ord = h->vis_ord.h + (size_t) w * C.F;
            std::vector<int> slot((size_t) p.K * p.K, -1);
            for (int f = 0; f < p.F; f++) slot[(size_t) p.f_ref[f] * p.K + p.f_obs[f]] = 0;
            int P = 0;
            for (int key = 0; key < p.K * p.K; key++)
                if (slot[key] == 0) slot[key] = P, pro[P++] = ((key / p.K) << 8) | (key % p.K);
            std::vector<int> npart(P, 0);
            for (int r = 0; r < nrun; r++) {
                unsigned seen = 0u;
                for (int q = off[vbh[r]]; q < off[vbh[r + 1]]; q++) seen |= 1u << meta[4 * q + 2];
                for (int k = 0; k < p.K; k++)
                    if ((seen >> k) & 1u) npart[slot[(size_t) refof[perm[vbh[r]]] * p.K + k]]++;
            }
            poff[0] = 0;
            for (int i = 0; i < P; i++) poff[i + 1] = poff[i] + npart[i];
            std::vector<int> cur(poff, poff + P), start(p.K), pidx(p.K);
            for (int r = 0; r < nrun; r++) {
                const int a = off[vbh[r]], b = off[vbh[r + 1]];
                if (a == b) continue;
                const int ref = meta[4 * a + 1];
                std::fill(start.begin(), start.end(), 0);
                for (int q = a; q < b; q++) start[meta[4 * q + 2]]++;
                for (int k = 0, t = 0; k < p.K; k++) {
                    const int c = start[k];
                    start[k] = t, t += c;
                    if (c) pidx[k] = cur[slot[(size_t) ref * p.K + k]]++;
                }
                for (int q = a; q < b; q++) {
                    const int k = meta[4 * q + 2];
                    ord[a + start[k]++] = (q - a) | (pidx[k] << 8);
                }
            }
            h->npairs.h[w] = P;
        }
        for (int k = 0; values && k < p.n_imu; k++) {
            const double *b = p.imu_blob + (size_t) k * ICG_IMU_BLOB_DOUBLES;
            memcpy(h->imu_blob.h + ((size_t) w * C.K + k) * ICG_IMU_BLOB_DOUBLES, b, sizeof(double) * ICG_IMU_BLOB_DOUBLES);
            if (!host_imu_sqrt_info(b + 252, h->imu_U.h + ((size_t) w * C.K + k) * 225)) {
                PK_FAIL(ICG_EINVAL, "icg_ba_upload: window %d IMU factor %d has a non positive-definite covariance", w, k);
            }
        }
        for (int g = 0; g < p.n_gnss; g++) {
            if (p.gnss_node[g] < 0 || p.gnss_node[g] >= p.K) {
                PK_FAIL(ICG_EINVAL, "icg_ba_upload: window %d GNSS factor %d has an invalid node", w, g);
            }
            h->gnss_node.h[(size_t) w * C.G + g] = p.gnss_node[g];
        }
        if (values && p.n_gnss) {
            memcpy(h->gnss_blh.h + (size_t) w * C.G * 3, p.gnss_blh, sizeof(double) * 3 * p.n_gnss);
            memcpy(h->gnss_std.h + (size_t) w * C.G * 3, p.gnss_std, sizeof(double) * 3 * p.n_gnss);
        }
        memcpy(h->lever.h + (size_t) w * 3, p.lever, sizeof(double) * 3);
        if (p.has_pose_prior) {
            memcpy(h->pose_prior.h + (size_t) w * 7, p.pose_prior, sizeof(double) * 7);
            for (int k = 0; k < 6; k++) h->pose_prior_sinfo.h[(size_t) w * 6 + k] = 1.0 / p.pose_prior_std[k];
        }
        if (p.has_mix_prior) {
            memcpy(h->mix_prior.h + (size_t) w * 9, p.mix_prior, sizeof(double) * 9);
            memcpy(h->mix_prior_std.h + (size_t) w * 9, p.mix_prior_std, sizeof(double) * 9);
        }
        if (p.marg_r > 0) {
            const int r = p.marg_r;
            int tot = 0, cols = 0;
            for (int b = 0; b < p.marg_nblocks; b++) {
                int t = p.marg_block_type[b];
                if (t < 0 || t > 3 || ((t == 0 || t == 1) && (p.marg_block_node[b] < 0 || p.marg_block_node[b] >= p.K))) {
                    PK_FAIL(ICG_EINVAL, "icg_ba_upload: window %d marginalization block %d invalid", w, b);
                }
                tot += (t == 0 || t == 2) ? 7 : t == 1 ? 9 : 1;
                cols += (t == 0 || t == 2) ? 6 : t == 1 ? 9 : 1;
                h->marg_type.h[(size_t) w * BA_MARG_MAXB + b] = t;
                h->marg_node.h[(size_t) w * BA_MARG_MAXB + b] = p.marg_block_node[b];
            }
            if (cols != r || tot > BA_MARG_MAXB * 9) {
                PK_FAIL(ICG_EINVAL, "icg_ba_upload: window %d marginalization prior size mismatch (blocks give %d columns, marg_r=%d)", w, cols, r);
            }
            memcpy(h->marg_x0.h + (size_t) w * BA_MARG_MAXB * 9, p.marg_x0, sizeof(double) * tot);
            if (!values) return ICG_OK;
            double *H0 = h->marg_H0.h + (size_t) w * C.R * C.R, *b0 = h->marg_b0.h + (size_t) w * C.R;
            for (int i = 0; i < r; i++) {
                for (int j = i; j < r; j++) {
                    double s = 0;
                    for (int k = 0; k < r; k++) s += p.marg_J0[(size_t) k * r + i] * p.marg_J0[(size_t) k * r + j];
                    H0[(size_t) i * r + j] = H0[(size_t) j * r + i] = s;
                }
                double s = 0;
                for (int k = 0; k < r; k++) s += p.marg_J0[(size_t) k * r + i] * p.marg_e0[k];
                b0[i] = s;
            }
            double c0 = 0;
            for (int k = 0; k < r; k++) c0 += p.marg_e0[k] * p.marg_e0[k];
            h->marg_c0.h[w] = c0;
        }
            return ICG_OK;
}
#undef PK_FAIL

static int pack_windows(icg_ba *h, int n, const icg_ba_problem *P, bool values) {
    const int nthreads = std::max(1, std::min({n / 4, 16, (int) std::thread::hardware_concurrency()}));
    std::vector<int> rcs(nthreads, ICG_OK);
    std::vector<std::string> errs(nthreads);
    auto worker = [&](int t) {
        for (int w = t; w < n; w += nthreads) {
            const int rc = pack_window(h, w, P[w], values, errs[t]);
            if (rc != ICG_OK) {
                rcs[t] = rc;
                return;
            }
        }
    };
    std::vector<std::thread> th;
    for (int t = 1; t < nthreads; t++) th.emplace_back(worker, t);
    worker(0);
    for (auto &x : th) x.join();
    for (int t = 0; t < nthreads; t++)
        if (rcs[t] != ICG_OK) {
            set_error("%s", errs[t].c_str());
            return rcs[t];
        }
    return ICG_OK;
}

static int upload_structure(icg_ba *h, int n) {
    const BaCaps &C = h->C;
    cudaStream_t s = h->stream;
    const size_t nn = (size_t) n, PM = (size_t) C.K * (C.K - 1);
#define UP(field, stride) ICG_CUDA(h->field.up(s, nn * (size_t) (stride)))
    UP(dims, 1); UP(ext, 8);
    UP(f_active, C.F);
    UP(f_meta_s, C.F * 4); UP(vb_lm0, C.NVB); UP(lm_off, C.L + 1); UP(lm_perm, C.L); UP(ref_nrun, C.K); UP(part_off, PM + 1); UP(pair_ro, PM); UP(vis_ord, C.F);
    UP(npairs, 1); UP(gnss_node, C.G); UP(lever, 3);
    UP(pose_prior, 7); UP(pose_prior_sinfo, 6); UP(mix_prior, 9); UP(mix_prior_std, 9);
    UP(marg_type, BA_MARG_MAXB); UP(marg_node, BA_MARG_MAXB); UP(marg_x0, BA_MARG_MAXB * 9);
#undef UP
    return ICG_OK;
}

static int keep_pristine(icg_ba *h, int n) {
    const BaCaps &C = h->C;
    const BaDev &D = h->D;
    cudaStream_t s = h->stream;
    ICG_CUDA(cudaMemcpyAsync(D.pose_0, D.pose, sizeof(double) * (size_t) n * C.K * 7, cudaMemcpyDeviceToDevice, s));
    ICG_CUDA(cudaMemcpyAsync(D.mix_0, D.mix, sizeof(double) * (size_t) n * C.K * 9, cudaMemcpyDeviceToDevice, s));
    ICG_CUDA(cudaMemcpyAsync(D.ext_0, D.ext, sizeof(double) * (size_t) n * 8, cudaMemcpyDeviceToDevice, s));
    ICG_CUDA(cudaMemcpyAsync(D.rho_0, D.rho, sizeof(double) * (size_t) n * C.L, cudaMemcpyDeviceToDevice, s));
    ICG_CUDA(cudaMemcpyAsync(D.f_active_0, D.f_active, (size_t) n * C.F, cudaMemcpyDeviceToDevice, s));
    ICG_CUDA(cudaMemcpyAsync(D.gnss_std_0, D.gnss_std, sizeof(double) * (size_t) n * C.G * 3, cudaMemcpyDeviceToDevice, s));
    return ICG_OK;
}

int icg_ba_upload(icg_ba *h, int n, const icg_ba_problem *P) {
    if (!h || !P || n < 1 || n > h->C.NW) {
        set_error("icg_ba_upload: bad arguments (n=%d, capacity %d)", n, h ? h->C.NW : 0);
        return ICG_EINVAL;
    }
    ICG_CUDA(cudaSetDevice(h->device));
    const BaCaps &C = h->C;
    h->marg_res_n = 0;
    int rc = pack_windows(h, n, P, true);
    if (rc != ICG_OK) return rc;
    rc = upload_structure(h, n);
    if (rc != ICG_OK) return rc;
    cudaStream_t s = h->stream;
    const size_t nn = (size_t) n;
#define UP(field, stride) ICG_CUDA(h->field.up(s, nn * (size_t) (stride)))
    UP(pose, C.K * 7); UP(mix, C.K * 9); UP(rho, C.L); UP(f_const_s, C.F * 14); UP(imu_blob, C.K * ICG_IMU_BLOB_DOUBLES); UP(imu_U, C.K * 225);
    UP(gnss_blh, C.G * 3); UP(gnss_std, C.G * 3); UP(marg_H0, (size_t) C.R * C.R); UP(marg_b0, C.R); UP(marg_c0, 1);
#undef UP
    rc = keep_pristine(h, n);
    if (rc != ICG_OK) return rc;
    h->cur_windows = n;
    return ICG_OK;
}

static const char *PROF_NAMES[16] = {"(gap/other)", "lin_vis", "lin_lm", "lin at candidate", "","schur_dmma (+ epilogue)", "join lin_cam + lin_done",
                                     "signal", "solve", "cost (+cost_cam)", "exchange", "accept", "reduce", "join gram chain", "step_lm", ""};
static void prof_mark(icg_ba *h, int tag) {
    if (!h->prof) return;
    if (h->prof_used == h->prof_ev.size()) {
        cudaEvent_t e;
        cudaEventCreate(&e);
        h->prof_ev.push_back(e);
        h->prof_tag.push_back(0);
    }
    h->prof_tag[h->prof_used] = tag;
    cudaEventRecord(h->prof_ev[h->prof_used++], h->stream);
}
static void prof_collect(icg_ba *h) {
    if (!h->prof) return;
    if (h->prof_used && h->prof_skip > 0) {
        h->prof_skip--;
        h->prof_used = 0;
        return;
    }
    for (size_t i = 1; i < h->prof_used; i++) {
        float ms = 0;
        if (cudaEventElapsedTime(&ms, h->prof_ev[i - 1], h->prof_ev[i]) == cudaSuccess) {
            h->prof_ms[h->prof_tag[i]] += ms;
            h->prof_cnt[h->prof_tag[i]]++;
        }
    }
    h->prof_used = 0;
}
static void prof_print(icg_ba *h) {
    if (!h->prof) return;
    double tot = 0;
    for (int t = 0; t < 16; t++) tot += h->prof_ms[t];
    fprintf(stderr, "[icg_ba profile] handle %p, %d windows: stage totals over all recorded LM sequences (ms, mean us, share)\n", (void *) h, h->cur_windows);
    for (int t = 0; t < 16; t++)
        if (h->prof_cnt[t])
            fprintf(stderr, "  %-28s %9.3f ms  %8.1f us  %5.1f %%\n", PROF_NAMES[t], h->prof_ms[t], 1e3 * h->prof_ms[t] / h->prof_cnt[t], 100.0 * h->prof_ms[t] / tot);
    if (h->D.clk) {
        unsigned long long ck[48];
        if (cudaMemcpy(ck, h->D.clk, sizeof(ck), cudaMemcpyDeviceToHost) == cudaSuccess) {
            static const char *cn[6] = {"factor evaluation", "prior product + cost", "zero H_c", "prior blocks", "IMU J^T J", "GNSS / prior diagonals"};
            fprintf(stderr, "[icg_ba profile] ba_lin_cam phases of window 0 (SM cycles per call, mean):\n");
            for (int k = 0; k < 6; k++)
                if (ck[24 + k]) fprintf(stderr, "  %-28s %9.0f cycles\n", cn[k], (double) ck[16 + k] / (double) ck[24 + k]);
            if (h->D.S.split) {
                static const char *sn_l2[6] = {"per panel: stage B operand", "per panel: warp 0 tile + factor", "per panel: tiles + barrier 1", "per panel: row solve + barrier 2", "whole factorisation", ""};
                static const char *sn_dsm[6] = {"assembly", "per panel: warp 0 tile + factor", "per panel: until block barrier", "per panel: row solve + cl. barrier", "whole factorisation", "backward substitution"};
                const char **sn = h->solve_cam_dsm ? sn_dsm : sn_l2;
                fprintf(stderr, "[icg_ba profile] %s phases of window 0 (SM cycles, mean):\n", h->solve_cam_dsm ? "ba_solve_cam_dsm" : "ba_solve_cam");
                for (int k = 0; k < 6; k++)
                    if (ck[8 + k]) fprintf(stderr, "  %-34s %9.0f cycles\n", sn[k], (double) ck[k] / (double) ck[8 + k]);
                static const char *sn2[5] = {"(unused)", "(unused)", "per panel: warp 0 diagonal-tile update", "per panel: warp 0 loads + 8x8 factorisation", "per panel: warp 0 write-back"};
                for (int k = 0; k < 5 && h->solve_cam_dsm; k++)
                    if (ck[40 + k]) fprintf(stderr, "  %-50s %9.0f cycles\n", sn2[k], (double) ck[32 + k] / (double) ck[40 + k]);
            }
            static const char *nm[8] = {"gradient / cost / tests", "assembly", "Cholesky", "camera back-substitution", "landmark back-substitution", "candidate + reductions",
                                        "  per panel: warp 0 tile+factor", "  per panel: row solve phase"};
            if (!h->D.S.split) fprintf(stderr, "[icg_ba profile] ba_solve phases of window 0 (SM cycles per call, mean):\n");
            for (int k = 0; k < 8 && !h->D.S.split; k++)
                if (ck[8 + k]) fprintf(stderr, "  %-28s %9.0f cycles\n", nm[k], (double) ck[k] / (double) ck[8 + k]);
        }
    }
}

static int enqueue_lm_split(icg_ba *h, int max_num_iterations);

static int alloc_lin_buf2(icg_ba *h) {
    BaDev &D = h->D;
    if (D.Mp[1]) return ICG_OK;
    const BaCaps &C = h->C;
    const size_t NW = C.NW;
    int rc = ICG_OK;
#define DM(field, count) \
    if (rc == ICG_OK) rc = dmalloc(h, &D.field, count);
    DM(AW[1], NW * C.NCA * C.LP) DM(Mp[1], NW * (size_t) C.K * (C.K - 1) * 210) DM(costf[1], NW * C.F) DM(hl[1], NW * C.L) DM(gl[1], NW * C.L)
    DM(Hc[1], NW * C.NS * C.NS) DM(gc[1], NW * C.NS)
#undef DM
    return rc;
}

static int enqueue_lm(icg_ba *h, int max_num_iterations) {
    if (h->D.S.split) return enqueue_lm_split(h, max_num_iterations);
    int rc = alloc_lin_buf2(h);
    if (rc != ICG_OK) return rc;
    const BaCaps &C = h->C;
    const BaDev &D = h->D;
    const int n = h->cur_windows;
    cudaStream_t s = h->stream;
    const dim3 g_vis(C.NVB - 2, n);
    auto enqueue_lin = [&](int at_cand) -> int {
        ICG_CUDA(cudaEventRecord(h->ev_fork, s));
        ICG_CUDA(cudaStreamWaitEvent(h->stream_cam, h->ev_fork, 0));
        ba_lin_cam<<<n, cam_threads(h), h->smem_cam, h->stream_cam>>>(C, D, at_cand);
        ICG_CUDA(cudaEventRecord(h->ev_join, h->stream_cam));
        prof_mark(h, 0);
        ba_lin_vis<<<g_vis, 128, LV_SMEM, s>>>(C, D, at_cand);
        prof_mark(h, at_cand ? 3 : 1);
        ICG_CUDA(cudaStreamWaitEvent(s, h->ev_join, 0));
        prof_mark(h, at_cand ? 3 : 6);
        count_launch(2);
        return ICG_OK;
    };
    rc = enqueue_lin(0);
    if (rc != ICG_OK) return rc;
    for (int it = 0; it <= max_num_iterations; it++) {
        ba_schur_dmma<<<dim3(BA_SPLIT_W, n), 256, h->smem_schur, s>>>(C, D, h->ld_schur);
        prof_mark(h, 5);
        ba_solve<<<n, SOLVE_THREADS, h->smem_solve, s>>>(C, D);
        prof_mark(h, 8);
        count_launch(2);
        if (it == max_num_iterations) break;
        rc = enqueue_lin(1);
        if (rc != ICG_OK) return rc;
        ba_accept<<<n, 128, sizeof(double) * 8 * h->nblk_vis, s>>>(C, D);
        prof_mark(h, 11);
        count_launch();
    }
    ICG_CHECK_LAUNCH();
    return ICG_OK;
}

static void split_release(icg_ba *h) {
    for (int r = 0; r < 8; r++)
        if (h->ipc_opened[r]) cudaIpcCloseMemHandle(h->ipc_opened[r]), h->ipc_opened[r] = nullptr;
    if (h->xbuf) cudaFree(h->xbuf), h->xbuf = nullptr;
    if (h->D.S.redv) cudaFree(h->D.S.redv), h->D.S.redv = nullptr;
    if (h->D.S.err) cudaFree(h->D.S.err), h->D.S.err = nullptr;
    if (h->D.S.slm) cudaFree(h->D.S.slm), h->D.S.slm = nullptr;
    if (h->D.S.slm_cnt) cudaFree(h->D.S.slm_cnt), h->D.S.slm_cnt = nullptr;
    if (h->D.Sglobal) cudaFree(h->D.Sglobal), h->D.Sglobal = nullptr;
    h->D.S.split = 0;
}

static int split_setup(icg_ba *h, int rank, int world) {
    if (world < 1 || world > 8 || rank < 0 || rank >= world) {
        set_error("split pipeline: rank %d / world %d out of range (<= 8 GPUs of one box)", rank, world);
        return ICG_EINVAL;
    }
    ICG_CUDA(cudaSetDevice(h->device));
    ICG_CUDA(cudaStreamSynchronize(h->stream));
    split_release(h);
    const BaCaps &C = h->C;
    ShardDev &S = h->D.S;
    const size_t NW = C.NW, G = world;
    const size_t TRI = (size_t) C.NCV * (C.NCV + 1) / 2;
    S.PK = (int) ((TRI + 3 * (size_t) C.NCV + 4 + 3) & ~(size_t) 3);
    S.BS = (SPLIT_HDR + C.NS + 3) & ~3;
    S.RV = (3 * C.NCV + 4 + 3) & ~3;
    const size_t NWo = (NW + G - 1) / G;
    size_t off = 0;
    S.off_inbox = off, off += NWo * G * S.PK;
    S.off_bcast = off, off += NW * S.BS;
    S.off_scal = off, off += NW * G * SPLIT_SCAL;
    S.off_flagA = off, off += 8;
    S.off_flagB = off, off += (NW + 3) & ~(size_t) 3;
    S.off_flagC = off, off += (NW * G + 3) & ~(size_t) 3;
    h->xbuf_doubles = off;
    if (cudaMalloc(&h->xbuf, sizeof(double) * off) != cudaSuccess || cudaMalloc(&S.redv, sizeof(double) * NW * S.RV) != cudaSuccess ||
        cudaMalloc(&S.err, sizeof(int) * 4) != cudaSuccess || cudaMalloc(&S.slm, sizeof(double) * NW * STEP_SLICES * 8) != cudaSuccess ||
        cudaMalloc(&S.slm_cnt, sizeof(int) * NW) != cudaSuccess ||
        cudaMalloc(&h->D.Sglobal, sizeof(double) * NWo * split_S_stride(C)) != cudaSuccess) {
        set_error("split pipeline: allocation of the exchange buffers failed (%zu doubles)", off);
        return ICG_ENOMEM;
    }
    ICG_CUDA(cudaMemset(h->xbuf, 0, sizeof(double) * off));
    ICG_CUDA(cudaMemset(S.redv, 0, sizeof(double) * NW * S.RV));
    ICG_CUDA(cudaMemset(S.err, 0, sizeof(int) * 4));
    ICG_CUDA(cudaMemset(S.slm, 0, sizeof(double) * NW * STEP_SLICES * 8));
    ICG_CUDA(cudaMemset(S.slm_cnt, 0, sizeof(int) * NW));
    for (int r = 0; r < 8; r++) S.peer[r] = nullptr;
    S.peer[rank] = h->xbuf;
    S.split = 1;
    h->D.rank = rank, h->D.world = world;
    h->x_world = world;
    h->epoch = 0;
    {
        const size_t ldbp = ((size_t) (C.N + 15) / 16) * 16 + 8;
        const size_t bs = (size_t) SPLIT_BS_ROWS * (C.NS + 1), base = 8 * ldbp + 64;
        h->smem_solve_cam = sizeof(double) * (40 + 4 * (size_t) C.NS + std::max(bs, base));
    }
    h->smem_step_lm = sizeof(double) * (40 + (size_t) C.NS);
    h->smem_solve_cam_dsm = sizeof(double) * dsm_smem_doubles(C);
    h->solve_cam_dsm = h->smem_solve_cam_dsm <= 227 * 1024 && C.N <= 32 * 11;
    if (h->solve_cam_dsm) ICG_CUDA(raise_dynamic_smem((const void *) ba_solve_cam_dsm, h->smem_solve_cam_dsm));
    ICG_CUDA(raise_dynamic_smem((const void *) ba_solve_cam, (size_t) (h->smem_solve_cam)));
    ICG_CUDA(cudaFuncSetAttribute(ba_solve_cam, cudaFuncAttributeNonPortableClusterSizeAllowed, 0));
    ICG_CUDA(raise_dynamic_smem((const void *) ba_step_lm, (size_t) (h->smem_step_lm)));
    return ICG_OK;
}

static int launch_solve_cam(icg_ba *h, int n, unsigned long long epoch) {
    cudaLaunchConfig_t cfg;
    memset(&cfg, 0, sizeof(cfg));
    cfg.gridDim = dim3((unsigned) (n * SPLIT_CLUSTER)), cfg.blockDim = dim3(SOLVE_THREADS);
    cfg.dynamicSmemBytes = h->solve_cam_dsm ? h->smem_solve_cam_dsm : h->smem_solve_cam, cfg.stream = h->stream;
    cudaLaunchAttribute at[1];
    at[0].id = cudaLaunchAttributeClusterDimension;
    at[0].val.clusterDim.x = SPLIT_CLUSTER, at[0].val.clusterDim.y = 1, at[0].val.clusterDim.z = 1;
    cfg.attrs = at, cfg.numAttrs = 1;
    if (h->solve_cam_dsm) ICG_CUDA(cudaLaunchKernelEx(&cfg, ba_solve_cam_dsm, h->C, h->D, epoch));
    else ICG_CUDA(cudaLaunchKernelEx(&cfg, ba_solve_cam, h->C, h->D, epoch));
    return ICG_OK;
}

static int enqueue_lm_split(icg_ba *h, int max_num_iterations) {
    const BaCaps &C = h->C;
    const BaDev &D = h->D;
    const int n = h->cur_windows;
    cudaStream_t s = h->stream;
    for (int r = 0; r < D.world; r++)
        if (!D.S.peer[r]) {
            set_error("landmark-sharded solve: peer %d is not connected (icg_ba_shard_connect)", r);
            return ICG_EINVAL;
        }
    const dim3 g_vis(C.NVB - 2, n), g_cost(h->nblk_vis, n), g_nn(((C.NCV + 1) * (C.NCV + 1) + 255) / 256, n);
    for (int it = 0; it <= max_num_iterations; it++) {
        const unsigned long long epoch = ++h->epoch;
        ICG_CUDA(cudaEventRecord(h->ev_fork, s));
        ICG_CUDA(cudaStreamWaitEvent(h->stream_cam, h->ev_fork, 0));
        ba_lin_cam<<<n, cam_threads(h), h->smem_cam, h->stream_cam>>>(C, D, 0);
        ICG_CUDA(cudaEventRecord(h->ev_join, h->stream_cam));
        prof_mark(h, 0);
        ba_lin_vis<<<g_vis, 128, LV_SMEM, s>>>(C, D, 0);
        prof_mark(h, 1);
        ba_schur_dmma<<<dim3(BA_SPLIT_W, n), 256, h->smem_schur, s>>>(C, D, h->ld_schur);
        prof_mark(h, 5);
        ba_signal<<<1, 32, 0, s>>>(D, epoch);
        prof_mark(h, 7);
        ICG_CUDA(cudaStreamWaitEvent(s, h->ev_join, 0));
        prof_mark(h, 6);
        ba_reduce<<<g_nn, 256, 0, s>>>(C, D, epoch);
        prof_mark(h, 12);
        int rc = launch_solve_cam(h, n, epoch);
        if (rc != ICG_OK) return rc;
        prof_mark(h, 8);
        ba_step_lm<<<dim3(n, STEP_SLICES), SOLVE_THREADS, h->smem_step_lm, s>>>(C, D, epoch);
        prof_mark(h, 14);
        count_launch(7);
        if (it == max_num_iterations) break;
        ICG_CUDA(cudaEventRecord(h->ev_fork, s));
        ICG_CUDA(cudaStreamWaitEvent(h->stream_cam, h->ev_fork, 0));
        ba_cost_cam<<<n, cam_threads(h), h->smem_cam, h->stream_cam>>>(C, D, h->nblk_vis);
        ICG_CUDA(cudaEventRecord(h->ev_join, h->stream_cam));
        ba_cost<<<g_cost, 256, 0, s>>>(C, D, h->nblk_vis);
        ICG_CUDA(cudaStreamWaitEvent(s, h->ev_join, 0));
        prof_mark(h, 9);
        ba_exchange<<<(n + 63) / 64, 64, 0, s>>>(C, D, n, h->nblk_vis, epoch);
        prof_mark(h, 10);
        ba_accept_split<<<n, 128, 0, s>>>(C, D, epoch);
        prof_mark(h, 11);
        count_launch(4);
    }
    ICG_CHECK_LAUNCH();
    return ICG_OK;
}

static int restore_params(icg_ba *h) {
    const BaCaps &C = h->C;
    const BaDev &D = h->D;
    const int n = h->cur_windows;
    cudaStream_t s = h->stream;
    ICG_CUDA(cudaMemcpyAsync(D.pose, D.pose_0, sizeof(double) * (size_t) n * C.K * 7, cudaMemcpyDeviceToDevice, s));
    ICG_CUDA(cudaMemcpyAsync(D.mix, D.mix_0, sizeof(double) * (size_t) n * C.K * 9, cudaMemcpyDeviceToDevice, s));
    ICG_CUDA(cudaMemcpyAsync(D.ext, D.ext_0, sizeof(double) * (size_t) n * 8, cudaMemcpyDeviceToDevice, s));
    ICG_CUDA(cudaMemcpyAsync(D.rho, D.rho_0, sizeof(double) * (size_t) n * C.L, cudaMemcpyDeviceToDevice, s));
    ICG_CUDA(cudaMemcpyAsync(D.f_active, D.f_active_0, (size_t) n * C.F, cudaMemcpyDeviceToDevice, s));
    ICG_CUDA(cudaMemcpyAsync(D.gnss_std, D.gnss_std_0, sizeof(double) * (size_t) n * C.G * 3, cudaMemcpyDeviceToDevice, s));
    ICG_CUDA(h->dims.up(s, n));
    return ICG_OK;
}

int icg_ba_run(icg_ba *h, int max_num_iterations, int restart) {
    if (!h || h->cur_windows < 1 || max_num_iterations < 0) {
        set_error("icg_ba_run: no problems uploaded");
        return ICG_EINVAL;
    }
    ICG_CUDA(cudaSetDevice(h->device));
    const int n = h->cur_windows;
    if (restart) {
        int rc = restore_params(h);
        if (rc != ICG_OK) return rc;
    }
    ba_reset_state<<<(n + 127) / 128, 128, 0, h->stream>>>(h->D, nullptr, n, max_num_iterations);
    count_launch();
    return enqueue_lm(h, max_num_iterations);
}

int icg_ba_run_gvins(icg_ba *h, int num_iterations, int restart) {
    if (!h || h->cur_windows < 1 || num_iterations < 1) {
        set_error("icg_ba_run_gvins: no problems uploaded");
        return ICG_EINVAL;
    }
    ICG_CUDA(cudaSetDevice(h->device));
    const BaCaps &C = h->C;
    const int n = h->cur_windows;
    const int first = num_iterations / 4, second = num_iterations - first;
    if (restart) {
        int rc = restore_params(h);
        if (rc != ICG_OK) return rc;
    }
    cudaStream_t s = h->stream;
    ba_set_gnss_huber<<<(n + 127) / 128, 128, 0, s>>>(h->D, n, 1);
    ba_reset_state<<<(n + 127) / 128, 128, 0, s>>>(h->D, nullptr, n, first);
    count_launch(2);
    int rc = enqueue_lm(h, first);
    if (rc != ICG_OK) return rc;
    ICG_CUDA(cudaMemsetAsync(h->cull_counters.d, 0, sizeof(int) * 2 * (size_t) n, s));
    const dim3 g_cull((std::max(C.F, C.G) + 127) / 128, n);
    ba_chi2_cull<<<g_cull, 128, 0, s>>>(C, h->D, h->cull_counters.d);
    ba_set_gnss_huber<<<(n + 127) / 128, 128, 0, s>>>(h->D, n, 0);
    ba_reset_state<<<(n + 127) / 128, 128, 0, s>>>(h->D, h->st_save.d, n, second);
    count_launch(3);
    return enqueue_lm(h, second);
}

int icg_ba_download(icg_ba *h, int n, const icg_ba_problem *P, icg_ba_summary *summaries) {
    if (!h || n < 1 || n > h->cur_windows) {
        set_error("icg_ba_download: bad arguments");
        return ICG_EINVAL;
    }
    ICG_CUDA(cudaSetDevice(h->device));
    const BaCaps &C = h->C;
    cudaStream_t s = h->stream;
    ICG_CUDA(h->pose.down(s, (size_t) n * C.K * 7)); ICG_CUDA(h->mix.down(s, (size_t) n * C.K * 9)); ICG_CUDA(h->ext.down(s, (size_t) n * 8));
    ICG_CUDA(h->rho.down(s, (size_t) n * C.L)); ICG_CUDA(h->st.down(s, n));
    ICG_CUDA(cudaStreamSynchronize(s));
    if (h->D.S.split && icg_ba_shard_error(h) != 0) {
        set_error("icg_ba_download: a peer exchange of the split pipeline timed out (a rank of the shard group did not run the same sequence)");
        return ICG_ECUDA;
    }
    for (int w = 0; w < n; w++) {
        if (P) {
            const icg_ba_problem &p = P[w];
            memcpy(p.pose, h->pose.h + (size_t) w * C.K * 7, sizeof(double) * 7 * p.K);
            memcpy(p.mix, h->mix.h + (size_t) w * C.K * 9, sizeof(double) * 9 * p.K);
            memcpy(p.ext, h->ext.h + (size_t) w * 8, sizeof(double) * 8);
            if (p.L > 0) memcpy(p.invdepth, h->rho.h + (size_t) w * C.L, sizeof(double) * p.L);
        }
        if (summaries) {
            const LmState &st = h->st.h[w];
            icg_ba_summary &o = summaries[w];
            o.iterations = st.iter, o.num_successful_steps = st.n_success;
            o.termination = st.done == 2 ? 1 : st.done == 3 ? 2 : 0;
            o.reserved = 0;
            o.initial_cost = st.initial_cost, o.final_cost = st.x_cost, o.final_radius = st.radius;
        }
    }
    return ICG_OK;
}

int icg_ba_solve(icg_ba *h, int n_windows, const icg_ba_problem *problems, int max_num_iterations, icg_ba_summary *summaries) {
    int rc = icg_ba_upload(h, n_windows, problems);
    if (rc != ICG_OK) return rc;
    rc = icg_ba_run(h, max_num_iterations, 0);
    if (rc != ICG_OK) return rc;
    return icg_ba_download(h, n_windows, problems, summaries);
}

static void fill_summary(const LmState &st, icg_ba_summary &o) {
    o.iterations = st.iter, o.num_successful_steps = st.n_success;
    o.termination = st.done == 2 ? 1 : st.done == 3 ? 2 : 0;
    o.reserved = 0;
    o.initial_cost = st.initial_cost, o.final_cost = st.x_cost, o.final_radius = st.radius;
}

int icg_ba_gvins_optimization_begin(icg_ba *h, int n_windows, const icg_ba_problem *problems, int num_iterations) {
    int rc = icg_ba_upload(h, n_windows, problems);
    if (rc != ICG_OK) return rc;
    return icg_ba_run_gvins(h, num_iterations, 0);
}

int icg_ba_gvins_optimization_end(icg_ba *h, int n_windows, const icg_ba_problem *problems, icg_ba_summary *summaries, int32_t *culled) {
    if (!h || !problems || n_windows < 1 || n_windows > h->cur_windows) {
        set_error("icg_ba_gvins_optimization_end: bad arguments");
        return ICG_EINVAL;
    }
    ICG_CUDA(cudaSetDevice(h->device));
    const BaCaps &C = h->C;
    cudaStream_t s = h->stream;
    ICG_CUDA(h->st_save.down(s, n_windows));
    ICG_CUDA(h->cull_counters.down(s, 2 * (size_t) n_windows));
    ICG_CUDA(h->f_active.down(s, (size_t) n_windows * C.F));
    ICG_CUDA(h->gnss_std.down(s, (size_t) n_windows * C.G * 3));
    std::vector<icg_ba_summary> second(n_windows);
    int rc = icg_ba_download(h, n_windows, problems, second.data());
    if (rc != ICG_OK) return rc;
    for (int w = 0; w < n_windows; w++) {
        const icg_ba_problem &p = problems[w];
        if (p.f_active) memcpy(const_cast<uint8_t *>(p.f_active), h->f_active.h + (size_t) w * C.F, p.F);
        if (p.n_gnss) memcpy(const_cast<double *>(p.gnss_std), h->gnss_std.h + (size_t) w * C.G * 3, sizeof(double) * 3 * p.n_gnss);
        if (summaries) {
            fill_summary(h->st_save.h[w], summaries[2 * w]);
            summaries[2 * w + 1] = second[w];
        }
        if (culled) culled[2 * w] = h->cull_counters.h[2 * w], culled[2 * w + 1] = h->cull_counters.h[2 * w + 1];
    }
    return ICG_OK;
}

int icg_ba_gvins_optimization(icg_ba *h, int n_windows, const icg_ba_problem *problems, int num_iterations, icg_ba_summary *summaries,
                              int32_t *culled) {
    int rc = icg_ba_gvins_optimization_begin(h, n_windows, problems, num_iterations);
    if (rc != ICG_OK) return rc;
    return icg_ba_gvins_optimization_end(h, n_windows, problems, summaries, culled);
}

constexpr int MARG_MAXN = 512;

static int marg_alloc(icg_ba *h) {
    if (h->marg_ready) return ICG_OK;
    const BaCaps &C = h->C;
    MargDev &M = h->M;
    const size_t NW = C.NW;
    M.rcap = C.N, M.mcap = 0, M.n0cap = 0;
    M.map_stride = MARG_MAP_HDR + 2 * C.K + C.L;
    if (h->marg_map.alloc(NW * M.map_stride) != ICG_OK || h->marg_oJ0.alloc(NW * (size_t) M.rcap * M.rcap) != ICG_OK || h->marg_oe0.alloc(NW * M.rcap) != ICG_OK ||
        h->marg_oHp.alloc(NW * (size_t) M.rcap * M.rcap) != ICG_OK || h->marg_obp.alloc(NW * M.rcap) != ICG_OK || h->marg_fmask.alloc(NW * C.F) != ICG_OK) {
        set_error("icg_ba_marginalize: workspace allocation failed");
        return ICG_ENOMEM;
    }
    M.map = h->marg_map.d, M.J0 = h->marg_oJ0.d, M.e0 = h->marg_oe0.d, M.Hp = h->marg_oHp.d, M.bp = h->marg_obp.d;
    int rc = ICG_OK;
    double *fl = nullptr;
#define DM(ptr, count) \
    if (rc == ICG_OK) rc = dmalloc(h, &ptr, count);
    DM(M.G2, NW * (size_t) M.rcap * M.rcap) DM(M.V2, NW * (size_t) M.rcap * M.rcap) DM(M.lam2, NW * M.rcap) DM(fl, NW * 2)
#undef DM
    if (rc != ICG_OK) return rc;
    M.flags = (int *) fl;
    const size_t smem = sizeof(double) * (8 * 480 + 2 * (size_t) C.R) + sizeof(int) * (size_t) C.R + 64;
    ICG_CUDA(raise_dynamic_smem((const void *) marg_assemble, (size_t) (smem)));
    h->marg_ready = true;
    return ICG_OK;
}

static int marg_grow(icg_ba *h, int n, int max_m, int max_n0) {
    MargDev &M = h->M;
    if (n <= h->marg_nw && max_m <= M.mcap && max_n0 <= M.n0cap) return ICG_OK;
    const int nw = std::max(n, h->marg_nw), mcap = std::max(max_m, M.mcap), n0cap = std::max(max_n0, M.n0cap);
    ICG_CUDA(cudaStreamSynchronize(h->stream));
    for (double **p : {&M.H0, &M.b0, &M.G1, &M.V1, &M.lam1, &M.Z}) {
        if (*p) cudaFree(*p);
        *p = nullptr;
    }
    h->marg_nw = 0, M.mcap = 0, M.n0cap = 0;
    const size_t NW = nw;
    const size_t count[6] = {NW * n0cap * n0cap, NW * n0cap, NW * mcap * mcap, NW * mcap * mcap, NW * mcap, NW * mcap * (M.rcap + 1)};
    double **ptr[6] = {&M.H0, &M.b0, &M.G1, &M.V1, &M.lam1, &M.Z};
    for (int k = 0; k < 6; k++) {
        if (cudaMalloc(ptr[k], sizeof(double) * std::max<size_t>(1, count[k])) != cudaSuccess) {
            *ptr[k] = nullptr;
            set_error("icg_ba_marginalize: workspace allocation of %zu doubles failed (%d windows, m <= %d, m + r <= %d)", count[k], nw, mcap, n0cap);
            return ICG_ENOMEM;
        }
        ICG_CUDA(cudaMemsetAsync(*ptr[k], 0, sizeof(double) * std::max<size_t>(1, count[k]), h->stream));
    }
    h->marg_nw = nw, M.mcap = mcap, M.n0cap = n0cap;
    return ICG_OK;
}

static int marginalize_body(icg_ba *h, int n_windows, const icg_ba_problem *problems, const int32_t *num_marg, icg_ba_prior *out, bool resident,
                            const uint8_t *const *fmask = nullptr) {
    if (!h || !problems || !num_marg || !out || n_windows < 1 || n_windows > h->C.NW) {
        set_error("icg_ba_marginalize: bad arguments");
        return ICG_EINVAL;
    }
    if (h->D.world > 1) {
        set_error("icg_ba_marginalize: not available on a landmark-sharded handle (icg_ba_shard_leave first)");
        return ICG_EUNSUPPORTED;
    }
    int rc = ICG_OK;
    h->marg_res_n = 0;
    if (resident) {
        if (h->cur_windows != n_windows) {
            set_error("icg_ba_marginalize_resident: the handle holds %d uploaded windows, the call names %d", h->cur_windows, n_windows);
            return ICG_EINVAL;
        }
        ICG_CUDA(cudaSetDevice(h->device));
    } else {
        rc = icg_ba_upload(h, n_windows, problems);
        if (rc != ICG_OK) return rc;
    }
    rc = marg_alloc(h);
    if (rc != ICG_OK) return rc;
    const BaCaps &C = h->C;
    MargDev &M = h->M;
    const int n = n_windows;
    for (int w = 0; w < n; w++) {
        const icg_ba_problem &p = problems[w];
        const int nm = num_marg[w];
        icg_ba_prior &o = out[w];
        if (nm < 1 || nm >= p.K || !o.block_type || !o.block_node || !o.x0 || !o.J0 || !o.e0 || o.rcap < 15 * (p.K - nm) + 7) {
            set_error("icg_ba_marginalize: window %d: num_marg=%d out of range or output arrays missing / too small (rcap=%d)", w, nm, o.rcap);
            return ICG_EINVAL;
        }
        int *map = h->marg_map.h + (size_t) w * M.map_stride;
        int *pose_col = map + MARG_MAP_HDR, *mix_col = pose_col + C.K, *lm_col = mix_col + C.K;
        std::vector<char> tp(p.K, 0), tm(p.K, 0), tl(p.L, 0);
        const uint8_t *act = fmask ? fmask[w] : p.f_active;
        if (fmask) memcpy(h->marg_fmask.h + (size_t) w * C.F, act, p.F);
        bool any_vis = false;
        for (int f = 0; f < p.F; f++) {
            if ((act && !act[f]) || p.f_ref[f] >= nm) continue;
            tl[p.f_lm[f]] = 1, tp[p.f_obs[f]] = 1, any_vis = true;
        }
        bool has_ext = any_vis, has_td = any_vis;
        for (int f = 0; f < p.F; f++)
            if (!(act && !act[f]) && p.f_ref[f] < nm) tp[p.f_ref[f]] = 1;
        for (int k = 0; k < nm && k < p.n_imu; k++) tp[k] = tm[k] = tp[k + 1] = tm[k + 1] = 1;
        for (int g = 0; g < p.n_gnss; g++)
            if (p.gnss_node[g] < nm) tp[p.gnss_node[g]] = 1;
        if (p.has_pose_prior) tp[0] = 1;
        if (p.has_mix_prior) tm[0] = 1;
        for (int b = 0; b < p.marg_nblocks && p.marg_r > 0; b++) {
            const int t = p.marg_block_type[b], nd = p.marg_block_node[b];
            if (t == 0) tp[nd] = 1;
            else if (t == 1) tm[nd] = 1;
            else if (t == 2) has_ext = true;
            else has_td = true;
        }
        int idx = 0;
        for (int k = 0; k < C.K; k++) pose_col[k] = mix_col[k] = -1;
        for (int k = 0; k < nm; k++) {
            if (tp[k]) pose_col[k] = idx, idx += 6;
            if (tm[k]) mix_col[k] = idx, idx += 9;
        }
        for (int l = 0; l < C.L; l++) lm_col[l] = -1;
        for (int l = 0; l < p.L; l++)
            if (tl[l]) lm_col[l] = idx++;
        const int m = idx;
        int nb = 0, xo = 0;
        for (int k = nm; k < p.K; k++) {
            if (tp[k]) pose_col[k] = idx, idx += 6, o.block_type[nb] = 0, o.block_node[nb++] = k - nm, xo += 7;
            if (tm[k]) mix_col[k] = idx, idx += 9, o.block_type[nb] = 1, o.block_node[nb++] = k - nm, xo += 9;
        }
        int ext_col = -1, td_col = -1;
        if (has_ext) ext_col = idx, idx += 6, o.block_type[nb] = 2, o.block_node[nb++] = 0, xo += 7;
        if (has_td) td_col = idx, idx += 1, o.block_type[nb] = 3, o.block_node[nb++] = 0, xo += 1;
        if (ext_col < 0) ext_col = 0;
        if (td_col < 0) td_col = 0;
        map[0] = m, map[1] = idx - m, map[2] = idx, map[3] = nm, map[4] = ext_col, map[5] = td_col, map[6] = map[7] = 0;
        o.m = m, o.r = idx - m, o.nblocks = nb;
        if (m > MARG_MAXN || idx - m > MARG_MAXN) {
            set_error("icg_ba_marginalize: window %d: %s=%d exceeds the %d rows of the largest eigensolver kernel", w, m > MARG_MAXN ? "m" : "r",
                      m > MARG_MAXN ? m : idx - m, MARG_MAXN);
            return ICG_EUNSUPPORTED;
        }
    }
    int max_m = 0, max_r = 0, max_n0 = 0;
    for (int w = 0; w < n; w++) max_m = std::max(max_m, out[w].m), max_r = std::max(max_r, out[w].r), max_n0 = std::max(max_n0, out[w].m + out[w].r);
    rc = marg_grow(h, n, max_m, max_n0);
    if (rc != ICG_OK) return rc;
    cudaStream_t s = h->stream;
    if (h->marg_cluster_ok < 0) {
        const size_t csm = marg_cluster_smem(MARG_CLUSTER_MAXN);
        ICG_CUDA(raise_dynamic_smem((const void *) marg_jacobi_cluster, csm));
        cudaLaunchConfig_t cfg;
        memset(&cfg, 0, sizeof(cfg));
        cfg.gridDim = dim3(MARG_CLUSTER_CTAS), cfg.blockDim = dim3(MARG_CLUSTER_THREADS), cfg.dynamicSmemBytes = csm, cfg.stream = s;
        cudaLaunchAttribute at[1];
        at[0].id = cudaLaunchAttributeClusterDimension;
        at[0].val.clusterDim.x = MARG_CLUSTER_CTAS, at[0].val.clusterDim.y = 1, at[0].val.clusterDim.z = 1;
        cfg.attrs = at, cfg.numAttrs = 1;
        int nclusters = 0;
        h->marg_cluster_ok = cudaOccupancyMaxActiveClusters(&nclusters, marg_jacobi_cluster, &cfg) == cudaSuccess && nclusters > 0 ? 1 : 0;
        cudaGetLastError();
    }
    ICG_CUDA(h->marg_map.up(s, (size_t) n * M.map_stride));
    BaDev D = h->D;
    if (fmask) {
        ICG_CUDA(h->marg_fmask.up(s, (size_t) n * C.F));
        D.f_active = h->marg_fmask.d;
    }
    const size_t smem = sizeof(double) * (8 * 480 + 2 * (size_t) C.R) + sizeof(int) * (size_t) C.R + 64;
    marg_prepare<<<(n + 127) / 128, 128, 0, s>>>(D, M, n, 0);
    ba_lin_vis<<<dim3(C.NVB - 2, n), 128, LV_SMEM, s>>>(C, D, 0);
    marg_assemble<<<n, 256, smem, s>>>(C, D, M);
    auto jacobi = [&](int which, int nmax) -> int {
        const bool cluster_ok = nmax <= MARG_CLUSTER_MAXN && h->marg_cluster_ok == 1;
        if (cluster_ok && !getenv("ICG_MARG_GLOBAL_JACOBI") && (getenv("ICG_MARG_CLUSTER_JACOBI") || nmax > MARG_PAIR_MAXN)) {
            const size_t smem = marg_cluster_smem(nmax);
            cudaLaunchConfig_t cfg;
            memset(&cfg, 0, sizeof(cfg));
            cfg.gridDim = dim3((unsigned) (MARG_CLUSTER_CTAS * n)), cfg.blockDim = dim3(MARG_CLUSTER_THREADS), cfg.dynamicSmemBytes = smem, cfg.stream = s;
            cudaLaunchAttribute at[1];
            at[0].id = cudaLaunchAttributeClusterDimension;
            at[0].val.clusterDim.x = MARG_CLUSTER_CTAS, at[0].val.clusterDim.y = 1, at[0].val.clusterDim.z = 1;
            cfg.attrs = at, cfg.numAttrs = 1;
            ICG_CUDA(cudaLaunchKernelEx(&cfg, marg_jacobi_cluster, M, which));
        } else if (nmax <= MARG_CTA_MAXN && !getenv("ICG_MARG_GLOBAL_JACOBI") && !getenv("ICG_MARG_PAIR_JACOBI")) {
            const size_t smem = sizeof(double) * 2 * (size_t) nmax * nmax;
            ICG_CUDA(raise_dynamic_smem((const void *) marg_jacobi_cta, smem));
            marg_jacobi_cta<<<n, MARG_CTA_THREADS, smem, s>>>(M, which);
        } else if (nmax <= MARG_PAIR_MAXN && !getenv("ICG_MARG_GLOBAL_JACOBI")) {
            const size_t smem = sizeof(double) * ((size_t) nmax * nmax + 2 * (size_t) (nmax + 2));
            cudaLaunchConfig_t cfg;
            memset(&cfg, 0, sizeof(cfg));
            cfg.gridDim = dim3((unsigned) (2 * n)), cfg.blockDim = dim3(MARG_THREADS), cfg.dynamicSmemBytes = smem, cfg.stream = s;
            cudaLaunchAttribute at[1];
            at[0].id = cudaLaunchAttributeClusterDimension;
            at[0].val.clusterDim.x = 2, at[0].val.clusterDim.y = 1, at[0].val.clusterDim.z = 1;
            cfg.attrs = at, cfg.numAttrs = 1;
            ICG_CUDA(raise_dynamic_smem((const void *) marg_jacobi_pair, (size_t) (smem)));
            ICG_CUDA(cudaLaunchKernelEx(&cfg, marg_jacobi_pair, M, which));
        } else {
            marg_jacobi<<<n, MARG_THREADS, 0, s>>>(M, which);
        }
        return ICG_OK;
    };
    rc = jacobi(0, max_m);
    if (rc != ICG_OK) return rc;
    marg_schur<<<n, MARG_THREADS, 0, s>>>(M);
    rc = jacobi(1, max_r);
    if (rc != ICG_OK) return rc;
    marg_finish<<<n, MARG_THREADS, 0, s>>>(M);
    marg_prepare<<<(n + 127) / 128, 128, 0, s>>>(D, M, n, 1);
    ICG_CHECK_LAUNCH();
    count_launch(9);
    {
        const size_t pitch = sizeof(double) * (size_t) M.rcap * M.rcap, used = sizeof(double) * (size_t) max_r * max_r;
        bool want_Hp = false;
        for (int w = 0; w < n; w++) want_Hp = want_Hp || out[w].Hp != nullptr;
        if (used) ICG_CUDA(cudaMemcpy2DAsync(h->marg_oJ0.h, pitch, h->marg_oJ0.d, pitch, used, (size_t) n, cudaMemcpyDeviceToHost, s));
        ICG_CUDA(h->marg_oe0.down(s, (size_t) n * M.rcap));
        if (want_Hp && used) ICG_CUDA(cudaMemcpy2DAsync(h->marg_oHp.h, pitch, h->marg_oHp.d, pitch, used, (size_t) n, cudaMemcpyDeviceToHost, s));
        ICG_CUDA(h->marg_obp.down(s, (size_t) n * M.rcap));
    }
    ICG_CUDA(cudaStreamSynchronize(s));
    auto write_back = [&](int w) {
        const icg_ba_problem &p = problems[w];
        icg_ba_prior &o = out[w];
        const int nm = num_marg[w], r = o.r;
        int xo = 0;
        for (int b = 0; b < o.nblocks; b++) {
            const int t = o.block_type[b], nd = o.block_node[b] + nm;
            const double *src = t == 0 ? p.pose + 7 * nd : t == 1 ? p.mix + 9 * nd : t == 2 ? p.ext : p.ext + 7;
            const int gs = t == 1 ? 9 : t == 3 ? 1 : 7;
            memcpy(o.x0 + xo, src, sizeof(double) * gs);
            xo += gs;
        }
        if (o.m <= 0) return;
        memcpy(o.J0, h->marg_oJ0.h + (size_t) w * M.rcap * M.rcap, sizeof(double) * (size_t) r * r);
        memcpy(o.e0, h->marg_oe0.h + (size_t) w * M.rcap, sizeof(double) * r);
        if (o.Hp) memcpy(o.Hp, h->marg_oHp.h + (size_t) w * M.rcap * M.rcap, sizeof(double) * (size_t) r * r);
        if (o.bp) memcpy(o.bp, h->marg_obp.h + (size_t) w * M.rcap, sizeof(double) * r);
    };
    {
        const int nthreads = std::max(1, std::min({n / 8, 8, (int) std::thread::hardware_concurrency()}));
        auto worker = [&](int t) {
            for (int w = t; w < n; w += nthreads) write_back(w);
        };
        std::vector<std::thread> th;
        for (int t = 1; t < nthreads; t++) th.emplace_back(worker, t);
        worker(0);
        for (auto &x : th) x.join();
    }
    if (resident) {
        h->marg_res_m.resize(n), h->marg_res_r.resize(n), h->marg_res_nb.resize(n);
        for (int w = 0; w < n; w++) h->marg_res_m[w] = out[w].m, h->marg_res_r[w] = out[w].r, h->marg_res_nb[w] = out[w].nblocks;
        h->marg_res_n = n;
    }
    return ICG_OK;
}

int icg_ba_marginalize(icg_ba *h, int n_windows, const icg_ba_problem *problems, const int32_t *num_marg, icg_ba_prior *out) {
    return marginalize_body(h, n_windows, problems, num_marg, out, false);
}

int icg_ba_marginalize_resident(icg_ba *h, int n_windows, const icg_ba_problem *problems, const int32_t *num_marg, icg_ba_prior *out) {
    return marginalize_body(h, n_windows, problems, num_marg, out, true);
}

static int resident_single_rank(icg_ba *h, int n_windows, const icg_ba_problem *problems, const char *what) {
    if (!h || !problems || n_windows < 1) {
        set_error("%s: bad arguments", what);
        return ICG_EINVAL;
    }
    if (h->D.world > 1) {
        set_error("%s: not available on a landmark-sharded handle (icg_ba_shard_leave first)", what);
        return ICG_EUNSUPPORTED;
    }
    if (h->cur_windows != n_windows) {
        set_error("%s: the handle holds %d uploaded windows, the call names %d", what, h->cur_windows, n_windows);
        return ICG_EINVAL;
    }
    return ICG_OK;
}

int icg_ba_update_and_cull_resident(icg_ba *h, int n_windows, const icg_ba_problem *problems, const icg_camera *cam, double reprojection_error_std,
                                    icg_ba_cull_window *io) {
    int rc = resident_single_rank(h, n_windows, problems, "icg_ba_update_and_cull_resident");
    if (rc != ICG_OK) return rc;
    if (!cam || !io) {
        set_error("icg_ba_update_and_cull_resident: bad arguments");
        return ICG_EINVAL;
    }
    const BaCaps &C = h->C;
    const int n = n_windows;
    std::vector<CullWin> win(n);
    size_t nL = 0, nO = 0, nK = 0;
    for (int w = 0; w < n; w++) {
        const icg_ba_problem &p = problems[w];
        const icg_ba_cull_window &c = io[w];
        if (p.K < 2 || p.K > C.K || p.L < 0 || p.L > C.L || !c.cam_pose ||
            (p.L > 0 && (!c.lm_ref_node || !c.lm_ref_kp || !c.obs_off || !c.lm_pw || !c.lm_depth || !c.lm_outlier))) {
            set_error("icg_ba_update_and_cull_resident: window %d: sizes out of range or arrays missing", w);
            return ICG_EINVAL;
        }
        const int no = p.L > 0 ? c.obs_off[p.L] : 0;
        if (p.L > 0 && (c.obs_off[0] != 0 || no < 0 || no > INT32_MAX - (int64_t) nO || (no > 0 && (!c.obs_node || !c.obs_kp || !c.obs_outlier)))) {
            set_error("icg_ba_update_and_cull_resident: window %d: obs_off must start at 0 and observation arrays must be given", w);
            return ICG_EINVAL;
        }
        for (int l = 0; l < p.L; l++) {
            if (c.obs_off[l + 1] < c.obs_off[l] || c.lm_ref_node[l] < 0 || c.lm_ref_node[l] >= p.K) {
                set_error("icg_ba_update_and_cull_resident: window %d landmark %d: obs_off not monotone or reference node out of range", w, l);
                return ICG_EINVAL;
            }
        }
        for (int o = 0; o < no; o++)
            if (c.obs_node[o] < 0 || c.obs_node[o] >= p.K) {
                set_error("icg_ba_update_and_cull_resident: window %d observation %d: node %d out of range", w, o, c.obs_node[o]);
                return ICG_EINVAL;
            }
        CullWin &W = win[w];
        memcpy(W.R_bc, c.R_bc, sizeof(W.R_bc)), memcpy(W.t_bc, c.t_bc, sizeof(W.t_bc));
        W.td_bc = c.td_bc, W.K = p.K, W.L = p.L, W.estimate_ext = c.estimate_ext != 0, W.estimate_td = c.estimate_td != 0;
        W.lm0 = (int) nL, W.off0 = (int) (nL + w), W.obs0 = (int) nO, W.node0 = (int) nK;
        nL += p.L, nO += no, nK += p.K;
    }
    auto al = [](size_t b) { return (b + 15) & ~(size_t) 15; };
    size_t at = 0;
    auto take = [&](size_t bytes) {
        const size_t o = at;
        at += al(bytes);
        return o;
    };
    const size_t i_win = take(sizeof(CullWin) * n), i_ref = take(4 * nL), i_off = take(4 * (nL + n)), i_node = take(4 * nO), i_rkp = take(8 * nL),
                 i_kp = take(8 * nO);
    const size_t in_bytes = at;
    const size_t o_win = take(sizeof(CullOut) * n), o_pose = take(96 * nK), o_pw = take(24 * nL), o_depth = take(8 * nL), o_lmo = take(nL), o_obso = take(nO);
    const size_t out_bytes = at - in_bytes;
    ICG_CUDA(cudaSetDevice(h->device));
    cudaStream_t s = h->stream;
    if (at > h->cull_cap) {
        ICG_CUDA(cudaStreamSynchronize(s));
        if (h->cull_h) cudaFreeHost(h->cull_h), h->cull_h = nullptr;
        if (h->cull_d) cudaFree(h->cull_d), h->cull_d = nullptr;
        h->cull_cap = 0;
        const size_t cap = at + at / 4;
        if (cudaMallocHost(&h->cull_h, cap) != cudaSuccess || cudaMalloc(&h->cull_d, cap) != cudaSuccess) {
            set_error("icg_ba_update_and_cull_resident: staging allocation of %zu bytes failed", cap);
            return ICG_ENOMEM;
        }
        h->cull_cap = cap;
    }
    unsigned char *H = h->cull_h, *Dv = h->cull_d;
    memcpy(H + i_win, win.data(), sizeof(CullWin) * n);
    for (int w = 0; w < n; w++) {
        const icg_ba_problem &p = problems[w];
        const icg_ba_cull_window &c = io[w];
        const CullWin &W = win[w];
        if (p.L == 0) {
            ((int *) (H + i_off))[W.off0] = 0;
            continue;
        }
        const int no = c.obs_off[p.L];
        memcpy(H + i_ref + 4 * (size_t) W.lm0, c.lm_ref_node, 4 * (size_t) p.L);
        memcpy(H + i_off + 4 * (size_t) W.off0, c.obs_off, 4 * ((size_t) p.L + 1));
        memcpy(H + i_rkp + 8 * (size_t) W.lm0, c.lm_ref_kp, 8 * (size_t) p.L);
        if (no > 0) memcpy(H + i_node + 4 * (size_t) W.obs0, c.obs_node, 4 * (size_t) no), memcpy(H + i_kp + 8 * (size_t) W.obs0, c.obs_kp, 8 * (size_t) no);
    }
    ICG_CUDA(cudaMemcpyAsync(Dv, H, in_bytes, cudaMemcpyHostToDevice, s));
    CullArgs a;
    a.cam = *cam, a.std = reprojection_error_std;
    a.pose = h->D.pose, a.ext = h->D.ext, a.rho = h->D.rho, a.pose_stride = C.K * 7, a.rho_stride = C.L;
    a.win = (const CullWin *) (Dv + i_win), a.lm_ref_node = (const int *) (Dv + i_ref), a.obs_off = (const int *) (Dv + i_off);
    a.obs_node = (const int *) (Dv + i_node), a.lm_ref_kp = (const float *) (Dv + i_rkp), a.obs_kp = (const float *) (Dv + i_kp);
    a.out = (CullOut *) (Dv + o_win), a.cam_pose = (double *) (Dv + o_pose), a.lm_pw = (double *) (Dv + o_pw), a.lm_depth = (double *) (Dv + o_depth);
    a.lm_outlier = Dv + o_lmo, a.obs_outlier = Dv + o_obso;
    ICG_CUDA(launch_update_cull(a, n, s));
    count_launch();
    ICG_CUDA(cudaMemcpyAsync(H + in_bytes, Dv + in_bytes, out_bytes, cudaMemcpyDeviceToHost, s));
    ICG_CUDA(cudaStreamSynchronize(s));
    for (int w = 0; w < n; w++) {
        const icg_ba_problem &p = problems[w];
        icg_ba_cull_window &c = io[w];
        const CullWin &W = win[w];
        const CullOut &O = ((const CullOut *) (H + o_win))[w];
        memcpy(c.R_bc_out, O.R_bc, sizeof(c.R_bc_out)), memcpy(c.t_bc_out, O.t_bc, sizeof(c.t_bc_out));
        c.td_bc_out = O.td_bc, c.ext_accepted = O.ext_accepted;
        memcpy(c.counts, O.counts, sizeof(c.counts));
        memcpy(c.cam_pose, H + o_pose + 96 * (size_t) W.node0, 96 * (size_t) p.K);
        if (p.L == 0) continue;
        const int no = c.obs_off[p.L];
        memcpy(c.lm_pw, H + o_pw + 24 * (size_t) W.lm0, 24 * (size_t) p.L);
        memcpy(c.lm_depth, H + o_depth + 8 * (size_t) W.lm0, 8 * (size_t) p.L);
        memcpy(c.lm_outlier, H + o_lmo + W.lm0, p.L);
        if (no > 0) memcpy(c.obs_outlier, H + o_obso + W.obs0, no);
    }
    return ICG_OK;
}

int icg_ba_reintegrate_resident(icg_ba *h, int n_windows, const icg_ba_problem *problems, const double *noise5, const double *station3,
                                icg_ba_reint_window *io) {
    int rc = resident_single_rank(h, n_windows, problems, "icg_ba_reintegrate_resident");
    if (rc != ICG_OK) return rc;
    if (!noise5 || !station3 || !io) {
        set_error("icg_ba_reintegrate_resident: bad arguments");
        return ICG_EINVAL;
    }
    const BaCaps &C = h->C;
    const int n = n_windows;
    size_t n_items = 0, n_rows = 0;
    for (int w = 0; w < n; w++) {
        const icg_ba_problem &p = problems[w];
        const icg_ba_reint_window &c = io[w];
        if (p.K < 2 || p.K > C.K || p.n_imu < 0 || p.n_imu > p.K - 1) {
            set_error("icg_ba_reintegrate_resident: window %d: sizes out of range", w);
            return ICG_EINVAL;
        }
        if (!c.reintegrate || p.n_imu == 0) continue;
        if (!c.imu || !c.imu_off || !c.status || !c.blob_out) {
            set_error("icg_ba_reintegrate_resident: window %d: arrays missing", w);
            return ICG_EINVAL;
        }
        if (c.imu_off[0] < 0) {
            set_error("icg_ba_reintegrate_resident: window %d: imu_off[0] is negative", w);
            return ICG_EINVAL;
        }
        for (int k = 0; k < p.n_imu; k++)
            if (c.imu_off[k + 1] - c.imu_off[k] < 1) {
                set_error("icg_ba_reintegrate_resident: window %d factor %d: imu_off must give every interval at least one row", w, k);
                return ICG_EINVAL;
            }
        n_items += p.n_imu, n_rows += (size_t) (c.imu_off[p.n_imu] - c.imu_off[0]);
    }
    for (int w = 0; w < n; w++) io[w].count = 0;
    if (n_items == 0) return ICG_OK;
    if (n_items > INT32_MAX / 8 || n_rows > INT32_MAX / 8) {
        set_error("icg_ba_reintegrate_resident: too many factors or IMU rows in one call");
        return ICG_EINVAL;
    }
    auto al = [](size_t b) { return (b + 15) & ~(size_t) 15; };
    size_t at = 0;
    auto take = [&](size_t bytes) {
        const size_t o = at;
        at += al(bytes);
        return o;
    };
    const size_t i_item = take(sizeof(ReintItem) * n_items), i_rows = take(56 * n_rows), o_cnt = take(sizeof(int));
    const size_t o_status = take(n_items), o_ends = take(80 * n_items), o_item = take(4 * n_items), o_blob = take(sizeof(double) * ICG_IMU_BLOB_DOUBLES * n_items);
    ICG_CUDA(cudaSetDevice(h->device));
    cudaStream_t s = h->stream;
    if (at > h->reint_cap) {
        ICG_CUDA(cudaStreamSynchronize(s));
        if (h->reint_h) cudaFreeHost(h->reint_h), h->reint_h = nullptr;
        if (h->reint_d) cudaFree(h->reint_d), h->reint_d = nullptr;
        h->reint_cap = 0;
        const size_t cap = at + at / 4;
        if (cudaMallocHost(&h->reint_h, cap) != cudaSuccess || cudaMalloc(&h->reint_d, cap) != cudaSuccess) {
            set_error("icg_ba_reintegrate_resident: staging allocation of %zu bytes failed", cap);
            return ICG_ENOMEM;
        }
        h->reint_cap = cap;
    }
    unsigned char *H = h->reint_h, *Dv = h->reint_d;
    ReintItem *items = (ReintItem *) (H + i_item);
    std::vector<int> first(n, -1);
    {
        size_t it = 0, row = 0;
        for (int w = 0; w < n; w++) {
            const icg_ba_problem &p = problems[w];
            const icg_ba_reint_window &c = io[w];
            if (!c.reintegrate || p.n_imu == 0) continue;
            first[w] = (int) it;
            const int r0 = c.imu_off[0], nr = c.imu_off[p.n_imu] - r0;
            memcpy(H + i_rows + 56 * row, c.imu + 7 * (size_t) r0, 56 * (size_t) nr);
            for (int k = 0; k < p.n_imu; k++, it++)
                items[it] = ReintItem{w, k, (int) row + c.imu_off[k] - r0, c.imu_off[k + 1] - c.imu_off[k]};
            row += nr;
        }
    }
    *(int *) (H + o_cnt) = 0;
    ICG_CUDA(cudaMemcpyAsync(Dv, H, o_status, cudaMemcpyHostToDevice, s));
    PreintResident a;
    a.n = (int) n_items, a.item = (const ReintItem *) (Dv + i_item), a.imu = (const double *) (Dv + i_rows);
    a.pose = h->D.pose, a.mix = h->D.mix, a.blob = h->D.imu_blob, a.U = h->D.imu_U, a.K = C.K;
    for (int k = 0; k < 5; k++) a.noise5[k] = noise5[k];
    for (int k = 0; k < 3; k++) a.station[k] = station3[k];
    a.status = (int8_t *) (Dv + o_status), a.ends = (double *) (Dv + o_ends), a.out_blob = (double *) (Dv + o_blob), a.out_item = (int *) (Dv + o_item);
    a.counter = (int *) (Dv + o_cnt);
    ICG_CUDA(preint_resident_launch(a, s));
    count_launch();
    ICG_CUDA(cudaMemcpyAsync(H + o_cnt, Dv + o_cnt, o_blob - o_cnt, cudaMemcpyDeviceToHost, s));
    ICG_CUDA(cudaStreamSynchronize(s));
    const int n_done = *(const int *) (H + o_cnt);
    if (n_done < 0 || (size_t) n_done > n_items) {
        set_error("icg_ba_reintegrate_resident: inconsistent completion count %d", n_done);
        return ICG_ECUDA;
    }
    if (n_done > 0) {
        ICG_CUDA(cudaMemcpyAsync(H + o_blob, Dv + o_blob, sizeof(double) * ICG_IMU_BLOB_DOUBLES * (size_t) n_done, cudaMemcpyDeviceToHost, s));
        ICG_CUDA(cudaStreamSynchronize(s));
    }
    const int8_t *st = (const int8_t *) (H + o_status);
    const double *ends = (const double *) (H + o_ends);
    for (int q = 0; q < n_done; q++) {
        const ReintItem &it = items[((const int *) (H + o_item))[q]];
        memcpy(io[it.win].blob_out + (size_t) ICG_IMU_BLOB_DOUBLES * it.fac, H + o_blob + sizeof(double) * ICG_IMU_BLOB_DOUBLES * (size_t) q,
               sizeof(double) * ICG_IMU_BLOB_DOUBLES);
    }
    int bad_w = -1, bad_k = -1;
    for (int w = 0; w < n; w++) {
        if (first[w] < 0) continue;
        icg_ba_reint_window &c = io[w];
        for (int k = 0; k < problems[w].n_imu; k++) {
            const int q = first[w] + k;
            c.status[k] = st[q];
            if (st[q] != 0) {
                c.count++;
                if (c.end_state10) memcpy(c.end_state10 + 10 * (size_t) k, ends + 10 * (size_t) q, 80);
            }
            if (st[q] < 0 && bad_w < 0) bad_w = w, bad_k = k;
        }
    }
    if (bad_w >= 0) {
        set_error("icg_ba_reintegrate_resident: window %d IMU factor %d: the reintegrated covariance is not positive definite (the factor was kept)", bad_w,
                  bad_k);
        return ICG_EINVAL;
    }
    return ICG_OK;
}

int icg_ba_marginalize_resident_culled(icg_ba *h, int n_windows, const icg_ba_problem *problems, const int32_t *num_marg,
                                       const icg_ba_cull_window *culled, const uint8_t *const *node_in_map, icg_ba_prior *out) {
    int rc = resident_single_rank(h, n_windows, problems, "icg_ba_marginalize_resident_culled");
    if (rc != ICG_OK) return rc;
    if (!culled || !node_in_map) {
        set_error("icg_ba_marginalize_resident_culled: bad arguments");
        return ICG_EINVAL;
    }
    std::vector<std::vector<uint8_t>> masks(n_windows);
    std::vector<const uint8_t *> mp(n_windows);
    for (int w = 0; w < n_windows; w++) {
        const icg_ba_problem &p = problems[w];
        const icg_ba_cull_window &c = culled[w];
        if (!node_in_map[w] || (p.L > 0 && (!c.lm_ref_node || !c.obs_off || !c.lm_outlier)) || p.K > h->C.K || p.L > h->C.L || p.F > h->C.F ||
            (p.L > 0 && c.obs_off[p.L] > 0 && (!c.obs_node || !c.obs_factor || !c.obs_outlier))) {
            set_error("icg_ba_marginalize_resident_culled: window %d: arrays missing", w);
            return ICG_EINVAL;
        }
        std::vector<uint8_t> &m = masks[w];
        m.assign(p.F, 1);
        std::vector<uint8_t> lm_bad(p.L, 0);
        for (int l = 0; l < p.L; l++) {
            lm_bad[l] = c.lm_outlier[l] != 0;
            for (int o = c.obs_off[l]; o < c.obs_off[l + 1]; o++) {
                const int f = c.obs_factor[o], k = c.obs_node[o];
                if (f < -1 || f >= p.F || (f >= 0 && (p.f_lm[f] != l || p.f_obs[f] != k))) {
                    set_error("icg_ba_marginalize_resident_culled: window %d landmark %d: observation %d names factor %d of another landmark or node", w, l, o, f);
                    return ICG_EINVAL;
                }
                if (!c.obs_outlier[o]) continue;
                if (k == c.lm_ref_node[l]) lm_bad[l] = 1;
                if (f >= 0) m[f] = 0;
            }
        }
        for (int f = 0; f < p.F; f++)
            if (lm_bad[p.f_lm[f]] || !node_in_map[w][p.f_obs[f]]) m[f] = 0;
        mp[w] = m.data();
    }
    return marginalize_body(h, n_windows, problems, num_marg, out, true, mp.data());
}

static int slide_body(icg_ba *h, int n, const icg_ba_problem *next, const icg_ba_slide_window *carry, const icg_ba_slide_integrate *integ,
                      const double *noise5, const double *station3, const char *fn) {
    int rc = resident_single_rank(h, n, next, fn);
    if (rc != ICG_OK) return rc;
    if (!carry || (integ && (!noise5 || !station3))) {
        set_error("%s: bad arguments", fn);
        return ICG_EINVAL;
    }
    ICG_CUDA(cudaSetDevice(h->device));
    const BaCaps &C = h->C;
    const size_t NW = C.NW;
    for (int w = 0; w < n; w++) {
        const icg_ba_problem &p = next[w];
        if (!carry[w].prior_from_marg) continue;
        if (h->marg_res_n != n) {
            set_error("%s: window %d takes its prior from the marginalization, but no resident marginalization of these %d windows "
                      "ran since the last upload or slide", fn, w, n);
            return ICG_EINVAL;
        }
        if (h->marg_res_m[w] <= 0 || p.marg_r != h->marg_res_r[w] || p.marg_nblocks != h->marg_res_nb[w]) {
            set_error("%s: window %d: marg_r=%d / marg_nblocks=%d, but the resident marginalization left m=%d, r=%d / nblocks=%d", fn, w,
                      p.marg_r, p.marg_nblocks, h->marg_res_m[w], h->marg_res_r[w], h->marg_res_nb[w]);
            return ICG_EINVAL;
        }
    }
    const size_t o_mix = NW * C.K * 7, o_rho = o_mix + NW * C.K * 9, o_blob = o_rho + NW * C.L, o_U = o_blob + NW * C.K * ICG_IMU_BLOB_DOUBLES,
                 o_blh = o_U + NW * C.K * 225, o_std = o_blh + NW * C.G * 3, n_old = o_std + NW * C.G * 3;
    if (!h->slide_old && (cudaMalloc(&h->slide_old, sizeof(double) * n_old) != cudaSuccess ||
                          cudaMalloc(&h->fc_alt, sizeof(double) * NW * C.F * 14) != cudaSuccess)) {
        if (h->slide_old) cudaFree(h->slide_old), h->slide_old = nullptr;
        set_error("%s: allocation of the slide buffers failed", fn);
        return ICG_ENOMEM;
    }
    std::vector<WinDims> old_dims(h->dims.h, h->dims.h + n);
    std::vector<std::vector<int>> old_slot(n);
    for (int w = 0; w < n; w++) {
        old_slot[w].resize(old_dims[w].F);
        const int *fidx = h->lm_fidx.h + (size_t) w * C.F;
        for (int q = 0; q < old_dims[w].F; q++) old_slot[w][fidx[q]] = q;
    }
    auto fail = [&](int code) {
        memcpy(h->dims.h, old_dims.data(), sizeof(WinDims) * n);
        for (int w = 0; w < n; w++) {
            int *fidx = h->lm_fidx.h + (size_t) w * C.F;
            for (int f = 0; f < old_dims[w].F; f++) fidx[old_slot[w][f]] = f;
        }
        return code;
    };
    rc = pack_windows(h, n, next, false);
    if (rc != ICG_OK) return fail(rc);
    std::vector<SlideWin> wins(n);
    std::vector<size_t> vbase(n);
    size_t n_map = 0, n_val = 0;
    int max_elems = 0, max_r = 0;
    for (int w = 0; w < n; w++) {
        const icg_ba_problem &p = next[w];
        const icg_ba_slide_window &c = carry[w];
        const WinDims &od = old_dims[w];
        const int32_t *maps[5] = {c.node_src, c.lm_src, c.f_src, c.imu_src, c.gnss_src};
        const int cnt[5] = {p.K, p.L, p.F, p.n_imu, p.n_gnss}, lim[5] = {od.K, od.L, od.F, od.n_imu, od.n_gnss}, width[5] = {SLIDE_NODE, 1, 14, SLIDE_IMU, SLIDE_GNSS};
        static const char *names[5] = {"node_src", "lm_src", "f_src", "imu_src", "gnss_src"};
        vbase[w] = n_val;
        for (int t = 0; t < 5; t++)
            for (int i = 0; maps[t] && i < cnt[t]; i++) {
                if (maps[t][i] < -1 || maps[t][i] >= lim[t]) {
                    set_error("%s: window %d: %s[%d] = %d is out of range of the old window (%d)", fn, w, names[t], i, maps[t][i], lim[t]);
                    return fail(ICG_EINVAL);
                }
                if (maps[t][i] >= 0) continue;
                n_val += width[t];
            }
        for (int t = 0; t < 5; t++)
            if (!maps[t]) n_val += (size_t) width[t] * cnt[t];
        SlideWin &W = wins[w];
        W.K = p.K, W.L = p.L, W.F = p.F, W.n_imu = p.n_imu, W.n_gnss = p.n_gnss;
        W.node_map = (int) n_map, W.lm_map = W.node_map + p.K, W.slot_map = W.lm_map + p.L, W.imu_map = W.slot_map + p.F, W.gnss_map = W.imu_map + p.n_imu;
        n_map = (size_t) W.gnss_map + p.n_gnss;
        W.r = p.marg_r, W.from_marg = c.prior_from_marg != 0, W.j0 = W.e0 = 0;
        if (W.r > 0 && !W.from_marg) n_val += (size_t) W.r * W.r + W.r;
        max_elems = std::max(max_elems, SLIDE_NODE * p.K + p.L + 14 * p.F + SLIDE_IMU * p.n_imu + SLIDE_GNSS * p.n_gnss);
        max_r = std::max(max_r, W.r);
    }
    std::vector<std::vector<int>> item_of(integ ? n : 0);
    std::vector<int> iwin_of(integ ? n : 0, -1);
    std::vector<SlideIntWin> iwins;
    std::vector<size_t> row_base(integ ? n : 0), state_base(integ ? n : 0);
    size_t n_item = 0, n_align = 0, n_row = 0, n_state = 0;
    bool want_blob = false;
    for (int w = 0; integ && w < n; w++) {
        const icg_ba_problem &p = next[w];
        const icg_ba_slide_window &c = carry[w];
        const icg_ba_slide_integrate &g = integ[w];
        const int oK = old_dims[w].K;
        std::vector<int> &io = item_of[w];
        io.assign(p.n_imu, -1);
        const size_t item0 = n_item, align0 = n_align;
        row_base[w] = n_row, state_base[w] = n_state;
        for (int k = 0; g.imu_from && k < p.n_imu; k++) {
            const int src = g.imu_from[k];
            if ((c.imu_src && c.imu_src[k] >= 0) || src == -1) continue;
            if (src >= oK || (src < 0 && src != ICG_SLIDE_CHAIN && src != ICG_SLIDE_ROW)) {
                set_error("%s: window %d: imu_from[%d] = %d is out of range of the old window (%d)", fn, w, k, src, oK);
                return fail(ICG_EINVAL);
            }
            if (src == ICG_SLIDE_CHAIN && (k == 0 || io[k - 1] < 0)) {
                set_error("%s: window %d: imu_from[%d] is ICG_SLIDE_CHAIN, but no integrated factor precedes it", fn, w, k);
                return fail(ICG_EINVAL);
            }
            if (!g.gravity3 || !g.imu || !g.imu_off || (src == ICG_SLIDE_ROW && !g.state16)) {
                set_error("%s: window %d: arrays missing", fn, w);
                return fail(ICG_EINVAL);
            }
            if (g.imu_off[k] < 0 || (long long) g.imu_off[k + 1] - g.imu_off[k] < 1) {
                set_error("%s: window %d factor %d: imu_off must give every integrated interval at least one row", fn, w, k);
                return fail(ICG_EINVAL);
            }
            io[k] = (int) n_item++;
            n_row += (size_t) (g.imu_off[k + 1] - g.imu_off[k]);
            n_state += src == ICG_SLIDE_ROW;
        }
        for (int j = 0; g.node_from_imu && j < p.K; j++) {
            if ((c.node_src && c.node_src[j] >= 0) || !g.node_from_imu[j]) continue;
            if (j == 0 || j - 1 >= p.n_imu || io[j - 1] < 0) {
                set_error("%s: window %d: node_from_imu[%d] is set, but factor %d is not integrated", fn, w, j, j - 1);
                return fail(ICG_EINVAL);
            }
        }
        for (int q = 0; g.gnss_node && q < p.n_gnss; q++) {
            if ((c.gnss_src && c.gnss_src[q] >= 0) || g.gnss_node[q] == -1) continue;
            if (g.gnss_node[q] < -1 || g.gnss_node[q] >= oK) {
                set_error("%s: window %d: gnss_node[%d] = %d is out of range of the old window (%d)", fn, w, q, g.gnss_node[q], oK);
                return fail(ICG_EINVAL);
            }
            if (!g.gnss_dt) {
                set_error("%s: window %d: arrays missing", fn, w);
                return fail(ICG_EINVAL);
            }
            n_align++;
        }
        if (n_item == item0 && n_align == align0) continue;
        iwin_of[w] = (int) iwins.size();
        iwins.push_back(SlideIntWin{w, (int) item0, (int) (n_item - item0), (int) align0, (int) (n_align - align0)});
        want_blob = want_blob || (g.blob_out && n_item > item0);
    }
    if (n_val >= (size_t) INT32_MAX || n_map >= (size_t) INT32_MAX || n_row >= (size_t) INT32_MAX / 8 || n_item >= (size_t) INT32_MAX / 8) {
        set_error("%s: too many new value rows in one call", fn);
        return fail(ICG_EINVAL);
    }
    auto al = [](size_t b) { return (b + 15) & ~(size_t) 15; };
    const size_t b_map = al(sizeof(SlideWin) * n), b_val = b_map + al(sizeof(int) * n_map);
    size_t total = b_val + sizeof(double) * n_val;
    auto take = [&](size_t bytes) {
        const size_t o = al(total);
        total = o + bytes;
        return o;
    };
    size_t b_iw = 0, b_item = 0, b_align = 0, b_rows = 0, b_state = 0, b_status = 0, b_ends = 0, b_blob = 0;
    if (!iwins.empty()) {
        b_iw = take(sizeof(SlideIntWin) * iwins.size()), b_item = take(sizeof(SlideItem) * n_item), b_align = take(sizeof(SlideAlign) * n_align);
        b_rows = take(56 * n_row), b_state = take(128 * n_state);
    }
    const size_t in_end = total;
    if (!iwins.empty()) {
        b_status = take(n_item), b_ends = take(80 * n_item);
        if (want_blob) b_blob = take(sizeof(double) * ICG_IMU_BLOB_DOUBLES * n_item);
    }
    cudaStream_t s = h->stream;
    if (total > h->slide_cap) {
        ICG_CUDA(cudaStreamSynchronize(s));
        if (h->slide_h) cudaFreeHost(h->slide_h), h->slide_h = nullptr;
        if (h->slide_d) cudaFree(h->slide_d), h->slide_d = nullptr;
        h->slide_cap = 0;
        const size_t cap = total + total / 4;
        if (cudaMallocHost(&h->slide_h, cap) != cudaSuccess || cudaMalloc(&h->slide_d, cap) != cudaSuccess) {
            set_error("%s: staging allocation of %zu bytes failed", fn, cap);
            return fail(ICG_ENOMEM);
        }
        h->slide_cap = cap;
    } else if (h->slide_ev) {
        ICG_CUDA(cudaEventSynchronize(h->slide_ev));
    }
    if (!h->slide_ev) ICG_CUDA(cudaEventCreateWithFlags(&h->slide_ev, cudaEventDisableTiming));
    int *map = (int *) (h->slide_h + b_map);
    double *val = (double *) (h->slide_h + b_val);
    SlideItem *items = (SlideItem *) (h->slide_h + b_item);
    SlideAlign *aligns = (SlideAlign *) (h->slide_h + b_align);
    double *rows = (double *) (h->slide_h + b_rows), *states = (double *) (h->slide_h + b_state);
    auto stage_window = [&](int w, std::string &err) -> int {
        const icg_ba_problem &p = next[w];
        const icg_ba_slide_window &c = carry[w];
        const icg_ba_slide_integrate *g = integ && iwin_of[w] >= 0 ? &integ[w] : nullptr;
        SlideWin &W = wins[w];
        int vo = (int) vbase[w];
        auto stage = [&](const double *src, int count) {
            const int at = vo;
            memcpy(val + vo, src, sizeof(double) * count);
            vo += count;
            return -(at + 1);
        };
        std::vector<int> node_at(g ? p.K + 1 : 0, -1);
        for (int k = 0; k < p.K; k++) {
            if (c.node_src && c.node_src[k] >= 0) {
                map[W.node_map + k] = c.node_src[k];
                continue;
            }
            if (g && g->node_from_imu && g->node_from_imu[k]) {
                node_at[k] = vo, map[W.node_map + k] = -(vo + 1), vo += SLIDE_NODE;
                continue;
            }
            map[W.node_map + k] = stage(p.pose + 7 * (size_t) k, 7);
            stage(p.mix + 9 * (size_t) k, 9);
        }
        for (int l = 0; l < p.L; l++) map[W.lm_map + l] = c.lm_src && c.lm_src[l] >= 0 ? c.lm_src[l] : stage(p.invdepth + l, 1);
        const int *fidx = h->lm_fidx.h + (size_t) w * C.F;
        for (int q = 0; q < p.F; q++) {
            const int f = fidx[q];
            map[W.slot_map + q] = c.f_src && c.f_src[f] >= 0 ? old_slot[w][c.f_src[f]] : stage(p.f_const + 14 * (size_t) f, 14);
        }
        size_t row_at = g ? row_base[w] : 0, state_at = g ? state_base[w] : 0;
        for (int k = 0; k < p.n_imu; k++) {
            if (c.imu_src && c.imu_src[k] >= 0) {
                map[W.imu_map + k] = c.imu_src[k];
                continue;
            }
            if (g && item_of[w][k] >= 0) {
                SlideItem &it = items[item_of[w][k]];
                const int r0 = g->imu_off[k], nr = g->imu_off[k + 1] - r0;
                it.src = g->imu_from[k], it.row0 = (int) row_at, it.nrow = nr, it.state = -1, it.blob = vo, it.node = node_at[k + 1];
                it.normal = g->normal && g->normal[k] ? 1 : 0;
                for (int i = 0; i < 3; i++) it.grav[i] = g->gravity3[3 * (size_t) k + i];
                memcpy(rows + 7 * row_at, g->imu + 7 * (size_t) r0, 56 * (size_t) nr);
                row_at += nr;
                if (it.src == ICG_SLIDE_ROW) {
                    memcpy(states + 16 * state_at, g->state16 + 16 * (size_t) k, 128);
                    it.state = (int) (16 * state_at++);
                }
                map[W.imu_map + k] = -(vo + 1), vo += SLIDE_IMU;
                continue;
            }
            const double *b = p.imu_blob + (size_t) k * ICG_IMU_BLOB_DOUBLES;
            map[W.imu_map + k] = stage(b, ICG_IMU_BLOB_DOUBLES);
            if (!host_imu_sqrt_info(b + 252, val + vo)) {
                char eb[256];
                snprintf(eb, sizeof(eb), "%s: window %d IMU factor %d has a non positive-definite covariance", fn, w, k);
                err = eb;
                return ICG_EINVAL;
            }
            vo += 225;
        }
        int align_at = g ? iwins[iwin_of[w]].align0 : 0;
        for (int q = 0; q < p.n_gnss; q++) {
            if (c.gnss_src && c.gnss_src[q] >= 0) {
                map[W.gnss_map + q] = c.gnss_src[q];
                continue;
            }
            map[W.gnss_map + q] = stage(p.gnss_blh + 3 * (size_t) q, 3);
            stage(p.gnss_std + 3 * (size_t) q, 3);
            if (g && g->gnss_node && g->gnss_node[q] >= 0) aligns[align_at++] = SlideAlign{-(map[W.gnss_map + q] + 1), g->gnss_node[q], g->gnss_dt[q]};
        }
        if (W.r > 0 && !W.from_marg) {
            W.j0 = -(stage(p.marg_J0, W.r * W.r) + 1);
            W.e0 = -(stage(p.marg_e0, W.r) + 1);
        }
        return ICG_OK;
    };
    {
        const int nthreads = std::max(1, std::min({n / 4, 16, (int) std::thread::hardware_concurrency()}));
        std::vector<int> rcs(nthreads, ICG_OK);
        std::vector<std::string> errs(nthreads);
        auto worker = [&](int t) {
            for (int w = t; w < n && rcs[t] == ICG_OK; w += nthreads) rcs[t] = stage_window(w, errs[t]);
        };
        std::vector<std::thread> th;
        for (int t = 1; t < nthreads; t++) th.emplace_back(worker, t);
        worker(0);
        for (auto &x : th) x.join();
        for (int t = 0; t < nthreads; t++)
            if (rcs[t] != ICG_OK) {
                set_error("%s", errs[t].c_str());
                return fail(rcs[t]);
            }
    }
    memcpy(h->slide_h, wins.data(), sizeof(SlideWin) * n);
    if (integ) {
        if (!iwins.empty()) {
            memcpy(h->slide_h + b_iw, iwins.data(), sizeof(SlideIntWin) * iwins.size());
            PreintSlide a;
            a.n = (int) iwins.size(), a.win = (const SlideIntWin *) (h->slide_d + b_iw), a.item = (const SlideItem *) (h->slide_d + b_item);
            a.align = (const SlideAlign *) (h->slide_d + b_align), a.imu = (const double *) (h->slide_d + b_rows);
            a.state = (const double *) (h->slide_d + b_state), a.pose = h->D.pose, a.mix = h->D.mix, a.K = C.K, a.val = (double *) (h->slide_d + b_val);
            for (int k = 0; k < 5; k++) a.noise5[k] = noise5[k];
            for (int k = 0; k < 3; k++) a.station[k] = station3[k];
            a.status = (int8_t *) (h->slide_d + b_status), a.ends = (double *) (h->slide_d + b_ends);
            a.out_blob = want_blob ? (double *) (h->slide_d + b_blob) : nullptr;
            cudaError_t e = cudaMemcpyAsync(h->slide_d, h->slide_h, in_end, cudaMemcpyHostToDevice, s);
            if (e == cudaSuccess) e = preint_slide_launch(a, s);
            if (e == cudaSuccess) e = cudaMemcpyAsync(h->slide_h + b_status, h->slide_d + b_status, total - b_status, cudaMemcpyDeviceToHost, s);
            if (e == cudaSuccess) e = cudaStreamSynchronize(s);
            if (e != cudaSuccess) {
                set_error("%s: the integration on the device failed: %s", fn, cudaGetErrorString(e));
                return fail(ICG_ECUDA);
            }
            count_launch();
        }
        const int8_t *st = (const int8_t *) (h->slide_h + b_status);
        const double *ends = (const double *) (h->slide_h + b_ends), *blobs = (const double *) (h->slide_h + b_blob);
        int bad_w = -1, bad_k = -1;
        for (int w = 0; w < n; w++) {
            const icg_ba_slide_integrate &g = integ[w];
            for (int k = 0; k < next[w].n_imu; k++) {
                const int q = item_of[w][k];
                if (g.status) g.status[k] = q >= 0 ? st[q] : 0;
                if (q < 0) continue;
                if (g.end_state10) memcpy(g.end_state10 + 10 * (size_t) k, ends + 10 * (size_t) q, 80);
                if (g.blob_out) memcpy(g.blob_out + (size_t) ICG_IMU_BLOB_DOUBLES * k, blobs + (size_t) ICG_IMU_BLOB_DOUBLES * q, 8 * ICG_IMU_BLOB_DOUBLES);
                if (st[q] < 0 && bad_w < 0) bad_w = w, bad_k = k;
            }
        }
        if (bad_w >= 0) {
            set_error("%s: window %d IMU factor %d: the integrated covariance is not positive definite", fn, bad_w, bad_k);
            return fail(ICG_EINVAL);
        }
    }
    h->marg_res_n = 0;
    if (iwins.empty()) ICG_CUDA(cudaMemcpyAsync(h->slide_d, h->slide_h, in_end, cudaMemcpyHostToDevice, s));
    ICG_CUDA(cudaEventRecord(h->slide_ev, s));
    rc = upload_structure(h, n);
    if (rc != ICG_OK) return rc;
    BaDev &D = h->D;
    double *old = h->slide_old;
    const size_t nn = (size_t) n;
    auto d2d = [&](double *dst, const double *src, size_t count) { return cudaMemcpyAsync(dst, src, sizeof(double) * count, cudaMemcpyDeviceToDevice, s); };
    ICG_CUDA(d2d(old, D.pose, nn * C.K * 7));
    ICG_CUDA(d2d(old + o_mix, D.mix, nn * C.K * 9));
    ICG_CUDA(d2d(old + o_rho, D.rho, nn * C.L));
    ICG_CUDA(d2d(old + o_blob, D.imu_blob, nn * C.K * ICG_IMU_BLOB_DOUBLES));
    ICG_CUDA(d2d(old + o_U, D.imu_U, nn * C.K * 225));
    ICG_CUDA(d2d(old + o_blh, D.gnss_blh, nn * C.G * 3));
    ICG_CUDA(d2d(old + o_std, D.gnss_std, nn * C.G * 3));
    SlideArgs a;
    a.win = (const SlideWin *) h->slide_d, a.map = (const int *) (h->slide_d + b_map), a.val = (const double *) (h->slide_d + b_val);
    a.K = C.K, a.L = C.L, a.F = C.F, a.G = C.G, a.R = C.R;
    a.old_pose = old, a.old_mix = old + o_mix, a.old_rho = old + o_rho, a.old_fc = D.f_const_s, a.old_blob = old + o_blob, a.old_U = old + o_U;
    a.old_blh = old + o_blh, a.old_std = old + o_std;
    a.pose = D.pose, a.mix = D.mix, a.rho = D.rho, a.fc = h->fc_alt, a.blob = D.imu_blob, a.U = D.imu_U, a.blh = D.gnss_blh, a.std = D.gnss_std;
// ... 345 lines not shown
```

### include/icgvins_b200.h

```cpp
#ifndef ICGVINS_B200_H
#define ICGVINS_B200_H

#include <stddef.h>
#include <stdint.h>

#ifdef __cplusplus
extern "C" {
#endif

#define ICG_OK 0
#define ICG_EINVAL (-1)
#define ICG_ENODEVICE (-2)
#define ICG_ECUDA (-3)
#define ICG_EUNSUPPORTED (-4)
#define ICG_ENOMEM (-5)

#define ICG_OPTFLOW_USE_INITIAL_FLOW 4

const char *icg_last_error(void);
int icg_version(void);
uint64_t icg_launch_count(void);
void icg_launch_count_reset(void);

typedef struct icg_klt icg_klt;

int icg_klt_create(icg_klt **h, int width, int height, int n_slots, int max_points, int device, void *stream);
void icg_klt_destroy(icg_klt *h);

int icg_klt_calc_optical_flow_pyr_lk(icg_klt *h, const uint8_t *prev, const uint8_t *next, int stride,
                                     const float *prev_xy, float *next_xy, uint8_t *status, float *err, int n,
                                     int win, int max_level, int max_iter, double eps, int flags);

int icg_klt_track_fb(icg_klt *h, const uint8_t *prev, const uint8_t *next, int stride, const float *prev_xy,
                     float *next_xy, float *back_xy, uint8_t *status, int n);


int icg_klt_upload(icg_klt *h, int slot, const uint8_t *host_img, int stride);
int icg_klt_upload_level0(icg_klt *h, int slot, const uint8_t *host_img, int stride);
int icg_klt_upload_batch(icg_klt *h, int first_slot, int count, const uint8_t *const *host_imgs, int stride);
int icg_klt_download_level(icg_klt *h, int slot, int level, uint8_t *host_img, int stride);
int icg_klt_slot_level0(icg_klt *h, int slot, void **dev_ptr, int *pitch);
int icg_klt_slot_level(icg_klt *h, int slot, int level, void **dev_ptr, int *pitch, int *w, int *hgt);
int icg_klt_build_pyramids(icg_klt *h, int first_slot, int count);
int icg_klt_track_batch_dev(icg_klt *h, int n_total, const int32_t *dev_slots, const float *dev_prev_xy,
                            const float *dev_init_xy, float *dev_fwd_xy, float *dev_bwd_xy, uint8_t *dev_status,
                            int mode);
int icg_klt_sync(icg_klt *h);

typedef struct icg_camera {
    double fx, fy, cx, cy, skew;
    double k1, k2, p1, p2, k3;
} icg_camera;
int icg_camera_undistort_points(const icg_camera *c, float *pts_xy, int n);
int icg_camera_distort_points(const icg_camera *c, float *pts_xy, int n);
int icg_camera_distort_camera_points(const icg_camera *c, const double *pc_xyz, float *px_xy, int n);
int icg_camera_pixel2cam(const icg_camera *c, const float *px_xy, double *cam_xyz, int n);
int icg_camera_world2pixel(const icg_camera *c, const double *R9, const double *t3, const double *pw_xyz, float *px_xy, int n);

int icg_find_fundamental_mat_ransac(const float *pts1_xy, const float *pts2_xy, int n, double threshold, double confidence, int max_iters,
                                    uint8_t *status, double *F9);

int icg_triangulate_points(const double *Tcw0, const double *Tcw1, const double *pc0_xy, const double *pc1_xy, int n, double *pw_xyz);

int icg_tracking_histogram(const uint8_t *img, int width, int height, int stride, double *out);

typedef struct icg_geom icg_geom;
int icg_geom_create(icg_geom **h, int device, void *stream);
void icg_geom_destroy(icg_geom *h);
int icg_geom_undistort_points(icg_geom *h, const icg_camera *c, float *pts_xy, int n);
int icg_geom_distort_points(icg_geom *h, const icg_camera *c, float *pts_xy, int n);
int icg_geom_find_fundamental_mat_ransac(icg_geom *h, const float *pts1_xy, const float *pts2_xy, int n, double threshold, double confidence, int max_iters,
                                         uint8_t *status, double *F9);
int icg_geom_triangulate_points(icg_geom *h, const double *Tcw0, const double *Tcw1, const double *pc0_xy, const double *pc1_xy, int n, double *pw_xyz);
int icg_geom_imu_preintegrate_batch(icg_geom *h, int n_intervals, const double *state16, const double *iewn3, const double *gravity3, const double *noise5,
                                    const double *imu, const int32_t *imu_off, double *blobs_out, double *end_states10);

int icg_geom_find_fundamental_mat_ransac_batch(icg_geom *h, int n_sets, const int32_t *set_off, const float *dev_pts1_xy, const float *dev_pts2_xy,
                                               const double *threshold, const double *confidence, int max_iters, uint8_t *dev_mask,
                                               int32_t *dev_n_inliers, double *dev_F9, long long *dev_stats);

typedef struct icg_track_frame {
    int32_t prev_slot, cur_slot;
    icg_camera camera;
    double R_pre[9], R_cur[9], R_ref[9];
    double t_cur[3];
    double dt;
    int64_t ref_id;
    double fm_threshold;
} icg_track_frame;
typedef struct icg_track_map {
    const float *prev_xy, *prev_undis_xy;
    const double *pw;
    const float *ref_kp_xy;
    float *fwd_xy, *fwd_undis_xy;
    uint8_t *keep;
    float *cur_xy, *cur_undis_xy;
    double *velocity;
    int32_t *src;
} icg_track_map;
typedef struct icg_track_ref {
    const float *new_xy, *ref_xy;
    const int64_t *ref_frame_id;
    const double *velocity_ref;
    float *fwd_xy, *fwd_undis_xy;
    uint8_t *keep;
    float *cur_xy, *cur_undis_xy;
    double *velocity;
    float *ref_out_xy;
    int64_t *ref_frame_id_out;
    double *velocity_ref_out;
    int32_t *src;
} icg_track_ref;
int icg_klt_track_frames_dev(icg_klt *h, int n_streams, const icg_track_frame *params, const int32_t *map_off, const icg_track_map *map,
                             const int32_t *ref_off, const icg_track_ref *ref, int32_t *dev_n_out, double *dev_parallax, int32_t *dev_parallax_n);
int icg_klt_track_frame(icg_klt *h, const icg_track_frame *params, int n_map, const icg_track_map *map, int n_ref, const icg_track_ref *ref,
                        int32_t *n_out, double *parallax, int32_t *parallax_n);

typedef struct icg_tri_frame {
    icg_camera camera;
    double R_cur[9], t_cur[3];
    int64_t cur_id, ref_id;
    int32_t window_normal;
    int32_t triangulate;
    double reprojection_error_std;
} icg_tri_frame;
typedef struct icg_tri_keyframe {
    int64_t id;
    double R[9], t[3];
    int32_t in_map;
} icg_tri_keyframe;
typedef struct icg_tri_list {
    float *ref_out_xy;
    int64_t *ref_frame_id_out;
    float *cur_xy;
    double *velocity_ref_out;
    const double *velocity;
    int32_t *src;
} icg_tri_list;
typedef struct icg_tri_new {
    double *pw, *depth;
    float *ref_undis_xy, *ref_xy, *cur_undis_xy, *cur_xy;
    double *velocity_cur, *velocity_ref;
    int64_t *ref_frame_id;
    int32_t *src;
} icg_tri_new;
int icg_klt_triangulate_dev(icg_klt *h, int n_streams, const icg_tri_frame *params, const int32_t *kf_off, const icg_tri_keyframe *kf,
                            const int32_t *ref_off, const int32_t *dev_n_in, int n_in_stride, const icg_tri_list *list, const icg_tri_new *out,
                            int32_t *dev_counts);
int icg_klt_triangulate(icg_klt *h, const icg_tri_frame *params, int n_kf, const icg_tri_keyframe *kf, int n, const icg_tri_list *list,
                        const icg_tri_new *out, int32_t *counts);

typedef struct icg_clahe icg_clahe;
int icg_clahe_create(icg_clahe **h, int width, int height, int tiles_x, int tiles_y, double clip_limit, int device, void *stream);
void icg_clahe_destroy(icg_clahe *h);
int icg_clahe_apply(icg_clahe *h, const uint8_t *src, int src_stride, uint8_t *dst, int dst_stride);
int icg_clahe_apply_dev(icg_clahe *h, const uint8_t *dev_src, int src_pitch, uint8_t *dev_dst, int dst_pitch);
int icg_clahe_apply_batch_dev(icg_clahe *h, int n_frames, const uint8_t *dev_src, int src_pitch, size_t src_frame_stride, uint8_t *dev_dst, int dst_pitch,
                              size_t dst_frame_stride, double *hist_out);
int icg_clahe_sync(icg_clahe *h);

typedef struct icg_rect {
    int32_t x, y, w, h;
} icg_rect;
typedef struct icg_detect icg_detect;
int icg_detect_create(icg_detect **h, int width, int height, int max_blocks, int max_corners_per_block, int max_roi_pixels, int device, void *stream);
void icg_detect_destroy(icg_detect *h);
int icg_detect_blocks(icg_detect *h, const uint8_t *img, const uint8_t *mask, int stride, int n_blocks, const icg_rect *rois,
                      const int32_t *max_corners, double quality, double min_distance, int do_subpix, float *out_xy, int32_t *out_n);
int icg_detect_blocks_dev(icg_detect *h, int n_frames, const uint8_t *dev_img, int pitch, size_t frame_stride, const uint8_t *dev_mask, int n_blocks,
                          const icg_rect *rois, const int32_t *max_corners, double quality, double min_distance, int do_subpix, float *out_xy,
                          int32_t *out_n);
int icg_detect_features(icg_detect *h, const uint8_t *img, int stride, const float *feat_xy, int n_feat, const float *new_xy, int n_new,
                        int n_ref, int ismask, int max_features, float *out_xy, int32_t *out_n);
int icg_detect_features_dev(icg_detect *h, int n_frames, const uint8_t *dev_img, int pitch, size_t frame_stride,
                            const float *dev_feat_xy, const uint8_t *dev_feat_status, const int32_t *feat_off,
                            const float *dev_new_xy, const uint8_t *dev_new_status, const int32_t *new_off,
                            const int32_t *n_ref, const uint8_t *ismask, int max_features, float *dev_out_xy, int32_t *dev_out_n);
int icg_detect_mask_dev(icg_detect *h, int frame, void **dev_ptr, int *pitch);
int icg_corner_subpix(icg_detect *h, const uint8_t *img, int stride, float *corners_xy, int n);

#define ICG_IMU_BLOB_DOUBLES 480
typedef struct icg_ba_problem {
    int32_t K, L, F;
    double *pose;
    double *mix;
    double *ext;
    double *invdepth;
    int32_t ext_const, td_const;
    const int32_t *f_lm, *f_ref, *f_obs;
    const double *f_const;
    const uint8_t *f_active;
    double reproj_std;
    int32_t reproj_huber;
    int32_t n_imu;
    const double *imu_blob;
    int32_t has_imu_error;
    int32_t has_pose_prior;
    const double *pose_prior, *pose_prior_std;
    int32_t has_mix_prior;
    const double *mix_prior, *mix_prior_std;
    int32_t n_gnss;
    const int32_t *gnss_node;
    const double *gnss_blh, *gnss_std;
    double lever[3];
    int32_t gnss_huber;
    int32_t marg_r, marg_nblocks;
    const int32_t *marg_block_type, *marg_block_node;
    const double *marg_x0, *marg_J0, *marg_e0;
} icg_ba_problem;

typedef struct icg_ba_summary {
    int32_t iterations;
    int32_t num_successful_steps;
    int32_t termination;
    int32_t reserved;
    double initial_cost, final_cost, final_radius;
} icg_ba_summary;

int icg_imu_preintegrate(const double *state16, const double *iewn3, const double *gravity3, const double *noise5, const double *imu,
                         int n, double *blob_out, double *end_state10);

typedef struct icg_ba icg_ba;
int icg_ba_create(icg_ba **h, int max_windows, int max_K, int max_L, int max_F, int max_gnss, int max_marg_r, int device,
                  void *stream);
void icg_ba_destroy(icg_ba *h);
int icg_ba_solve(icg_ba *h, int n_windows, const icg_ba_problem *problems, int max_num_iterations, icg_ba_summary *summaries);
int icg_ba_upload(icg_ba *h, int n_windows, const icg_ba_problem *problems);
int icg_ba_run(icg_ba *h, int max_num_iterations, int restart);
int icg_ba_download(icg_ba *h, int n_windows, const icg_ba_problem *problems, icg_ba_summary *summaries);
int icg_ba_gvins_optimization(icg_ba *h, int n_windows, const icg_ba_problem *problems, int num_iterations, icg_ba_summary *summaries,
                              int32_t *culled);
int icg_ba_run_gvins(icg_ba *h, int num_iterations, int restart);
int icg_ba_gvins_optimization_begin(icg_ba *h, int n_windows, const icg_ba_problem *problems, int num_iterations);
int icg_ba_gvins_optimization_end(icg_ba *h, int n_windows, const icg_ba_problem *problems, icg_ba_summary *summaries, int32_t *culled);
int icg_ba_sync(icg_ba *h);
typedef struct icg_ba_prior {
    int32_t m, r, nblocks;
    int32_t rcap;
    int32_t *block_type, *block_node;
    double *x0, *J0, *e0;
    double *Hp, *bp;
} icg_ba_prior;
int icg_ba_marginalize(icg_ba *h, int n_windows, const icg_ba_problem *problems, const int32_t *num_marg, icg_ba_prior *out);
int icg_ba_marginalize_resident(icg_ba *h, int n_windows, const icg_ba_problem *problems, const int32_t *num_marg, icg_ba_prior *out);
typedef struct icg_ba_cull_window {
    double R_bc[9], t_bc[3], td_bc;
    int32_t estimate_ext, estimate_td;
    const int32_t *lm_ref_node;
    const float *lm_ref_kp;
    const int32_t *obs_off;
    const int32_t *obs_node;
    const float *obs_kp;
    const int32_t *obs_factor;
    double R_bc_out[9], t_bc_out[3], td_bc_out;
    int32_t ext_accepted;
    double *cam_pose;
    double *lm_pw, *lm_depth;
    uint8_t *lm_outlier;
    uint8_t *obs_outlier;
    int32_t counts[5];
} icg_ba_cull_window;
int icg_ba_update_and_cull_resident(icg_ba *h, int n_windows, const icg_ba_problem *problems, const icg_camera *cam, double reprojection_error_std,
                                    icg_ba_cull_window *io);
int icg_ba_marginalize_resident_culled(icg_ba *h, int n_windows, const icg_ba_problem *problems, const int32_t *num_marg,
                                       const icg_ba_cull_window *culled, const uint8_t *const *node_in_map, icg_ba_prior *out);
typedef struct icg_ba_reint_window {
    int32_t reintegrate;
    const double *imu;
    const int32_t *imu_off;
    int8_t *status;
    double *blob_out;
    double *end_state10;
    int32_t count;
} icg_ba_reint_window;
int icg_ba_reintegrate_resident(icg_ba *h, int n_windows, const icg_ba_problem *problems, const double *noise5, const double *station3,
                                icg_ba_reint_window *io);
typedef struct icg_ba_slide_window {
    const int32_t *node_src;
    const int32_t *lm_src;
    const int32_t *f_src;
    const int32_t *imu_src;
    const int32_t *gnss_src;
    int32_t prior_from_marg;
} icg_ba_slide_window;
int icg_ba_slide_resident(icg_ba *h, int n_windows, const icg_ba_problem *next, const icg_ba_slide_window *carry);
#define ICG_SLIDE_CHAIN (-2)
#define ICG_SLIDE_ROW (-3)
typedef struct icg_ba_slide_integrate {
    const int32_t *imu_from;
    const double *state16;
    const double *gravity3;
    const uint8_t *normal;
    const double *imu;
    const int32_t *imu_off;
    const uint8_t *node_from_imu;
    const int32_t *gnss_node;
    const double *gnss_dt;
    int8_t *status;
    double *blob_out;
    double *end_state10;
} icg_ba_slide_integrate;
int icg_ba_slide_integrate_resident(icg_ba *h, int n_windows, const icg_ba_problem *next, const icg_ba_slide_window *carry,
                                    const icg_ba_slide_integrate *integ, const double *noise5, const double *station3);
#define ICG_SHARD_BLOB_BYTES 128
int icg_ba_shard_export(icg_ba *h, int rank, int world, uint8_t *blob);
int icg_ba_shard_connect(icg_ba *h, const uint8_t *blobs);
int icg_ba_shard_error(icg_ba *h);
int icg_ba_shard_leave(icg_ba *h);
int icg_ba_residual_costs(icg_ba *h, const icg_ba_problem *problem, double *reproj_cost , double *gnss_cost );
int icg_ba_reproj_evaluate(icg_ba *h, const double *pose0, const double *pose1, const double *ext, const double *invdepth,
                           const double *td, const double *f_const14, double std, double *residuals, double **jacobians);
int icg_ba_imu_evaluate(icg_ba *h, const double *imu_blob, const double *pose0, const double *mix0, const double *pose1,
                        const double *mix1, double *residuals, double **jacobians);

int icg_ba_gnss_evaluate(icg_ba *h, const double *pose, const double *blh, const double *std3, const double *lever, double *residuals,
                         double **jacobians);
int icg_ba_pose_prior_evaluate(icg_ba *h, const double *pose, const double *prior7, const double *std6, double *residuals, double **jacobians);
int icg_ba_mix_prior_evaluate(icg_ba *h, const double *mix, const double *prior9, const double *std9, double *residuals, double **jacobians);
int icg_ba_imu_error_evaluate(icg_ba *h, const double *mix, double *residuals, double **jacobians);
int icg_ba_marg_factor_evaluate(icg_ba *h, int r, int nblocks, const int32_t *block_type, const double *const *parameters, const double *x0,
                                const double *J0, const double *e0, double *residuals, double **jacobians);

#ifdef __cplusplus
}
#endif
#endif
```

Before: 24610.

## Pack multiple landmark runs into each ba_lin_vis CTA bin and size grid to bins

Before, each ba_lin_vis CTA processed exactly one landmark run, and the grid was fixed at NVB-2 blocks per window. Now the host greedily packs consecutive runs into bins of at most 128 factors, stores precomputed int4 ranges, and launches only as many CTAs as the largest bin count. The kernel handles several reference nodes per CTA: group heads are found with a warp ballot, and arrival counters and partial sums are tracked per reference node. The intent is fewer, fuller CTAs and fewer early-exit blocks, at the cost of more complex per-CTA finalization logic and bookkeeping on the host.

```diff
diff --git a/ic_gvins_b200/_lib.py b/ic_gvins_b200/_lib.py
--- a/ic_gvins_b200/_lib.py
+++ b/ic_gvins_b200/_lib.py
@@ -85,6 +85,8 @@
     L.icg_ba_destroy.restype = None
     L.icg_ba_solve.argtypes = [vp, C.c_int, vp, C.c_int, vp]
     L.icg_ba_upload.argtypes = [vp, C.c_int, vp]
+    L.icg_ba_set_lin_vis_bin_runs.argtypes = [vp, C.c_int]
+    L.icg_ba_lin_vis_bins.argtypes = [C.c_int, C.c_int, vp, vp, C.c_int, vp, vp, vp, vp]
     L.icg_ba_run.argtypes = [vp, C.c_int, C.c_int]
     L.icg_ba_download.argtypes = [vp, C.c_int, vp, vp]
     L.icg_ba_sync.argtypes = [vp]
@@ -154,6 +156,6 @@
     "icg_clahe_create", "icg_clahe_destroy", "icg_clahe_apply", "icg_clahe_apply_dev", "icg_clahe_apply_batch_dev", "icg_geom_create", "icg_geom_destroy", "icg_geom_undistort_points", "icg_geom_distort_points", "icg_geom_find_fundamental_mat_ransac", "icg_geom_triangulate_points", "icg_geom_imu_preintegrate_batch", "icg_clahe_sync",
     "icg_geom_find_fundamental_mat_ransac_batch", "icg_klt_track_frames_dev", "icg_klt_track_frame",
     "icg_klt_triangulate_dev", "icg_klt_triangulate",
-    "icg_imu_preintegrate", "icg_ba_create", "icg_ba_destroy", "icg_ba_solve", "icg_ba_upload", "icg_ba_run", "icg_ba_download",
+    "icg_imu_preintegrate", "icg_ba_create", "icg_ba_destroy", "icg_ba_solve", "icg_ba_upload", "icg_ba_set_lin_vis_bin_runs", "icg_ba_lin_vis_bins", "icg_ba_run", "icg_ba_download",
     "icg_ba_sync", "icg_ba_shard_export", "icg_ba_shard_connect", "icg_ba_shard_error", "icg_ba_shard_leave", "icg_ba_gvins_optimization", "icg_ba_run_gvins", "icg_ba_gvins_optimization_begin", "icg_ba_gvins_optimization_end", "icg_ba_residual_costs", "icg_ba_reproj_evaluate", "icg_ba_imu_evaluate", "icg_ba_marginalize", "icg_ba_marginalize_resident", "icg_ba_update_and_cull_resident", "icg_ba_marginalize_resident_culled", "icg_ba_reintegrate_resident", "icg_ba_slide_resident", "icg_ba_slide_integrate_resident", "icg_ba_gnss_evaluate", "icg_ba_pose_prior_evaluate", "icg_ba_mix_prior_evaluate", "icg_ba_imu_error_evaluate", "icg_ba_marg_factor_evaluate",
 ]
diff --git a/ic_gvins_b200/csrc/ba.cu b/ic_gvins_b200/csrc/ba.cu
--- a/ic_gvins_b200/csrc/ba.cu
+++ b/ic_gvins_b200/csrc/ba.cu
@@ -67,7 +67,7 @@
     uint8_t *f_active;
     int *lm_off;
     int *lm_perm;
-    int *vb_lm0;
+    int4 *vis_rng;
     int *ref_nrun;
     int *f_meta_s;
     double *f_const_s;
@@ -122,33 +122,48 @@
 constexpr size_t LV_SMEM = sizeof(double) * (128 * LV_LD + (BA_MAX_NODES + 1) * NODE_FRAME_LD);
 __global__ void __launch_bounds__(128, 4) ba_lin_vis(BaCaps C, BaDev D, int at_cand) {
     extern __shared__ double lv_sm[];
-    __shared__ int s_ord[128], s_gbeg[BA_MAX_NODES], s_gend[BA_MAX_NODES], s_last, s_p0, s_np;
+    __shared__ int s_ord[128], s_gbeg[129], s_wcnt[4], s_last[BA_MAX_NODES], s_p0[BA_MAX_NODES], s_np[BA_MAX_NODES];
     double (*s_rec)[LV_LD] = (double (*)[LV_LD]) lv_sm;
     double (*s_frame)[NODE_FRAME_LD] = (double (*)[NODE_FRAME_LD]) (lv_sm + 128 * LV_LD);
     const int w = blockIdx.y;
+    const int4 *rng = D.vis_rng + (size_t) w * C.NVB;
+    const int nbin = rng[C.NVB - 1].x;
+    const int4 bn = rng[blockIdx.x];
     const LmState &st = D.st[w];
     if (st.done || !(at_cand ? st.step_valid : st.need_lin)) return;
+    if ((int) blockIdx.x >= nbin) return;
     const int b = at_cand ? 1 - st.lin_buf : st.lin_buf;
     const double *pose = at_cand ? D.pose_c : D.pose, *xext = at_cand ? D.ext_c : D.ext, *rho = at_cand ? D.rho_c : D.rho;
-    const int *vb = D.vb_lm0 + (size_t) w * C.NVB;
-    if ((int) blockIdx.x >= vb[C.NVB - 1]) return;
     const WinDims dm = D.dims[w];
     const int tid = threadIdx.x;
     const int *off = D.lm_off + (size_t) w * (C.L + 1);
-    const int pA = vb[blockIdx.x], pB = vb[blockIdx.x + 1];
-    const int s0 = off[pA], nslot = off[pB] - s0;
+    const int pA = bn.x, pB = bn.y, s0 = bn.z, nslot = bn.w - bn.z;
+    int4 meta = make_int4(0, 0, 0, 0);
+    if (tid < nslot) meta = ((const int4 *) D.f_meta_s)[(size_t) w * C.F + s0 + tid];
+#ifdef ICG_BA_PHASE_CLOCKS
+    unsigned long long vclk = D.clk ? clock64() : 0ull;
+#define VIS_CLK(k)                                                 \
+    if (D.clk && w == 0 && tid == 0) {                             \
+        const unsigned long long t_ = clock64();                   \
+        atomicAdd(&D.clk[48 + (k)], t_ - vclk), atomicAdd(&D.clk[56 + (k)], 1ull); \
+        vclk = t_;                                                 \
+    }
+#else
+#define VIS_CLK(k)
+#endif
     if (tid <= dm.K) node_frame(tid < dm.K ? pose + ((size_t) w * C.K + tid) * 7 : xext + (size_t) w * 8, s_frame[tid]);
-    if (tid < BA_MAX_NODES) s_gbeg[tid] = s_gend[tid] = 0;
-    if (tid == 0) s_np = 0;
+    if (tid < BA_MAX_NODES) s_last[tid] = s_np[tid] = 0;
+    int active = 0;
+    double rl = 0.0;
+    if (tid < nslot) active = D.f_active[(size_t) w * C.F + meta.w], rl = rho[(size_t) w * C.L + meta.x];
     __syncthreads();
     if (tid < nslot) {
         const int q = s0 + tid;
         double r[2], Ji[12], Jj[12], Je[12], Jr[2], Jt[2], cost = 0;
-        const int4 meta = ((const int4 *) D.f_meta_s)[(size_t) w * C.F + q];
         const int i = meta.y, j = meta.z, f = meta.w;
-        if (D.f_active[(size_t) w * C.F + f] != 0) {
+        if (active != 0) {
             const double *ext = xext + (size_t) w * 8;
-            reproj_eval_frames(s_frame[i], s_frame[j], s_frame[dm.K], rho[(size_t) w * C.L + meta.x], ext[7],
+            reproj_eval_frames(s_frame[i], s_frame[j], s_frame[dm.K], rl, ext[7],
                                D.f_const_s + ((size_t) w * C.F + q) * 14, dm.reproj_sinv, true, r, Ji, Jj, Je, Jr, Jt);
             if (dm.ext_const)
                 for (int k = 0; k < 12; k++) Je[k] = 0;
@@ -174,15 +189,24 @@
         sr[40] = Jr[0], sr[41] = Jr[1], sr[42] = (double) j, sr[43] = (double) i;
     }
     __syncthreads();
+    VIS_CLK(0)
     const int lane = tid & 31, warp = tid >> 5;
     if (nslot > 0) {
+        bool head = false;
         if (tid < nslot) {
             const int *ord = D.vis_ord + (size_t) w * C.F + s0;
-            const int v = ord[tid], ob = (int) s_rec[v & 255][42];
+            const int v = ord[tid];
             s_ord[tid] = v;
-            if (tid == 0 || (int) s_rec[ord[tid - 1] & 255][42] != ob) s_gbeg[ob] = tid;
-            if (tid == nslot - 1 || (int) s_rec[ord[tid + 1] & 255][42] != ob) s_gend[ob] = tid + 1;
-        }
+            head = tid == 0 || (ord[tid - 1] >> 8) != (v >> 8);
+        }
+        const unsigned hm = __ballot_sync(0xffffffffu, head);
+        if (lane == 0) s_wcnt[warp] = __popc(hm);
+        __syncthreads();
+        int gb = 0;
+        for (int k = 0; k < warp; k++) gb += s_wcnt[k];
+        if (head) s_gbeg[gb + __popc(hm & ((1u << lane) - 1u))] = tid;
+        const int ng = s_wcnt[0] + s_wcnt[1] + s_wcnt[2] + s_wcnt[3];
+        if (tid == 0) s_gbeg[ng] = nslot;
         __syncthreads();
         const int kk = lane & 3, g = lane >> 2;
         int o[3];
@@ -191,9 +215,8 @@
             const int a = 8 * t + g;
             o[t] = a < 20 ? jc_off(a) + (kk & 1) * jc_row1(a) : -1;
         }
-        for (int ob = warp; ob < dm.K; ob += 4) {
-            const int beg = s_gbeg[ob], end = s_gend[ob];
-            if (beg == end) continue;
+        for (int gi = warp; gi < ng; gi += 4) {
+            const int beg = s_gbeg[gi], end = s_gbeg[gi + 1];
             double c00[2] = {0, 0}, c01[2] = {0, 0}, c02[2] = {0, 0}, c11[2] = {0, 0}, c12[2] = {0, 0}, c22[2] = {0, 0};
             constexpr int UNR = 2;
             for (int base = beg; base < end; base += 2 * UNR) {
@@ -228,7 +251,9 @@
         }
         __threadfence();
     }
+    VIS_CLK(1)
     const int *perm = D.lm_perm + (size_t) w * C.L;
+    const int first = st.first;
     const int K = dm.K, NCV = 6 * K + 7, NCA = 4 * ((NCV + 1 + 3) / 4);
     const int grp = tid >> 3, sl = tid & 7;
     int o0[3], o1[3];
@@ -275,44 +300,62 @@
                 lin_gl(C, D, b, w)[l] = acc[t];
             } else if (c == 20) {
                 lin_hl(C, D, b, w)[l] = acc[t];
-                if (st.first) D.scale_l[(size_t) w * C.L + l] = 1.0 / (1.0 + sqrt(acc[t]));
-            }
-        }
-    }
-    if (nslot == 0) return;
-    const int rn = (int) s_rec[0][43];
+                if (first) D.scale_l[(size_t) w * C.L + l] = 1.0 / (1.0 + sqrt(acc[t]));
+            }
+        }
+    }
+    VIS_CLK(2)
+    if (nslot == 0) {
+        VIS_CLK(3)
+        return;
+    }
     __syncthreads();
-    if (tid == 0) s_last = atomicAdd(D.vis_cnt + (size_t) w * C.K + rn, 1) == D.ref_nrun[(size_t) w * C.K + rn] - 1;
-    __syncthreads();
-    if (!s_last) return;
+    int mine = 0;
+    if (tid < nslot) {
+        const int rn = (int) s_rec[tid][43];
+        if ((tid == 0 || (int) s_rec[tid - 1][43] != rn) &&
+            atomicAdd(D.vis_cnt + (size_t) w * C.K + rn, 1) == D.ref_nrun[(size_t) w * C.K + rn] - 1)
+            s_last[rn] = 1, mine = 1;
+    }
+    if (!__syncthreads_or(mine)) {
+        VIS_CLK(3)
+        return;
+    }
     __threadfence();
-    if (tid == 0) D.vis_cnt[(size_t) w * C.K + rn] = 0;
+    if (tid < BA_MAX_NODES && s_last[tid]) D.vis_cnt[(size_t) w * C.K + tid] = 0;
     const int PM = C.K * (C.K - 1), P = D.npairs[w];
     const int *pro = D.pair_ro + (size_t) w * PM, *poff = D.part_off + (size_t) w * (PM + 1);
-    for (int p = tid; p < P; p += 128)
-        if ((pro[p] >> 8) == rn) {
-            atomicAdd(&s_np, 1);
-            if (p == 0 || (pro[p - 1] >> 8) != rn) s_p0 = p;
-        }
+    for (int p = tid; p < P; p += 128) {
+        const int rn = pro[p] >> 8;
+        if (s_last[rn]) {
+            atomicAdd(&s_np[rn], 1);
+            if (p == 0 || (pro[p - 1] >> 8) != rn) s_p0[rn] = p;
+        }
+    }
     __syncthreads();
     const double *part = D.gpart + (size_t) w * C.GQ * 210;
     double *Mp = lin_Mp(C, D, b, w);
-    for (int p = s_p0 + warp; p < s_p0 + s_np; p += 4) {
-        const int k0 = poff[p], k1 = poff[p + 1];
-        double acc[7];
-#pragma unroll
-        for (int j = 0; j < 7; j++) acc[j] = lane + 32 * j < 210 ? __ldcg(part + (size_t) k0 * 210 + lane + 32 * j) : 0.0;
-        for (int k = k0 + 1; k < k1; k++) {
-            double v[7];
-#pragma unroll
-            for (int j = 0; j < 7; j++) v[j] = lane + 32 * j < 210 ? __ldcg(part + (size_t) k * 210 + lane + 32 * j) : 0.0;
-#pragma unroll
-            for (int j = 0; j < 7; j++) acc[j] += v[j];
-        }
-#pragma unroll
-        for (int j = 0; j < 7; j++)
-            if (lane + 32 * j < 210) Mp[(size_t) p * 210 + lane + 32 * j] = acc[j];
-    }
+    for (int rn = 0; rn < dm.K; rn++) {
+        if (!s_last[rn]) continue;
+        for (int p = s_p0[rn] + warp; p < s_p0[rn] + s_np[rn]; p += 4) {
+            const int k0 = poff[p], k1 = poff[p + 1];
+            double acc[7];
+#pragma unroll
+            for (int j = 0; j < 7; j++) acc[j] = lane + 32 * j < 210 ? __ldcg(part + (size_t) k0 * 210 + lane + 32 * j) : 0.0;
+            for (int k = k0 + 1; k < k1; k++) {
+                double v[7];
+#pragma unroll
+                for (int j = 0; j < 7; j++) v[j] = lane + 32 * j < 210 ? __ldcg(part + (size_t) k * 210 + lane + 32 * j) : 0.0;
+#pragma unroll
+                for (int j = 0; j < 7; j++) acc[j] += v[j];
+            }
+#pragma unroll
+            for (int j = 0; j < 7; j++)
+                if (lane + 32 * j < 210) Mp[(size_t) p * 210 + lane + 32 * j] = acc[j];
+        }
+    }
+    VIS_CLK(3)
+#undef VIS_CLK
 }
 
 
@@ -1591,7 +1634,10 @@
     HostDev<LmState> st;
     HostDev<double> pose, mix, ext, rho, imu_blob, imu_U, gnss_blh, gnss_std, lever, pose_prior, pose_prior_sinfo, mix_prior, mix_prior_std, marg_x0,
         marg_H0, marg_b0, marg_c0;
-    HostDev<int> f_meta_s, vb_lm0, ref_nrun;
+    HostDev<int> f_meta_s, vb_lm0, vis_bin, ref_nrun;
+    HostDev<int4> vis_rng;
+    int vis_nbin = 1;
+    int bin_max_runs = 0;
     HostDev<double> f_const_s;
     HostDev<int> lm_off, lm_perm, lm_fidx, gnss_node, marg_type, marg_node, part_off, pair_ro, vis_ord, npairs;
     HostDev<uint8_t> f_active;
@@ -1715,7 +1761,7 @@
     h->prof = getenv("ICG_BA_PROFILE") != nullptr;
     if (h->prof) {
         double *ck = nullptr;
-        if (dmalloc(h, &ck, 48) != ICG_OK) return ICG_ENOMEM;
+        if (dmalloc(h, &ck, 64) != ICG_OK) return ICG_ENOMEM;
         h->D.clk = (unsigned long long *) ck;
     }
     if (getenv("ICG_BA_PROFILE_SKIP")) h->prof_skip = atoi(getenv("ICG_BA_PROFILE_SKIP"));
@@ -1738,7 +1784,7 @@
     HD(pose_prior, NW * 7) HD(pose_prior_sinfo, NW * 6) HD(mix_prior, NW * 9) HD(mix_prior_std, NW * 9) HD(marg_x0, NW * BA_MARG_MAXB * 9)
     HD(marg_H0, NW * C.R * C.R) HD(marg_b0, NW * C.R) HD(marg_c0, NW)
     HD(lm_off, NW * (C.L + 1)) HD(lm_perm, NW * C.L) HD(lm_fidx, NW * C.F) HD(gnss_node, NW * C.G) HD(marg_type, NW * BA_MARG_MAXB) HD(marg_node, NW * BA_MARG_MAXB) HD(f_active, NW * C.F)
-    HD(scratch, 1024) HD(st_save, NW) HD(cull_counters, 2 * NW) HD(f_meta_s, NW * C.F * 4) HD(vb_lm0, NW * C.NVB) HD(ref_nrun, NW * C.K) HD(f_const_s, NW * C.F * 14)
+    HD(scratch, 1024) HD(st_save, NW) HD(cull_counters, 2 * NW) HD(f_meta_s, NW * C.F * 4) HD(vb_lm0, NW * C.NVB) HD(vis_bin, NW * C.NVB) HD(vis_rng, NW * C.NVB) HD(ref_nrun, NW * C.K) HD(f_const_s, NW * C.F * 14)
     HD(part_off, NW * ((size_t) C.K * (C.K - 1) + 1)) HD(pair_ro, NW * (size_t) C.K * (C.K - 1)) HD(vis_ord, NW * C.F) HD(npairs, NW)
 #undef HD
     ICG_CUDA(cudaMemsetAsync(h->st.d, 0, sizeof(LmState) * NW, h->stream));
@@ -1747,7 +1793,7 @@
     D.dims = h->dims.d, D.st = h->st.d, D.pose = h->pose.d, D.mix = h->mix.d, D.ext = h->ext.d, D.rho = h->rho.d;
     D.f_active = h->f_active.d;
     D.part_off = h->part_off.d, D.pair_ro = h->pair_ro.d, D.vis_ord = h->vis_ord.d, D.npairs = h->npairs.d;
-    D.f_meta_s = h->f_meta_s.d, D.vb_lm0 = h->vb_lm0.d, D.ref_nrun = h->ref_nrun.d, D.f_const_s = h->f_const_s.d;
+    D.f_meta_s = h->f_meta_s.d, D.vis_rng = h->vis_rng.d, D.ref_nrun = h->ref_nrun.d, D.f_const_s = h->f_const_s.d;
     D.lm_off = h->lm_off.d, D.lm_perm = h->lm_perm.d, D.imu_blob = h->imu_blob.d, D.imu_U = h->imu_U.d;
     D.gnss_node = h->gnss_node.d, D.gnss_blh = h->gnss_blh.d, D.gnss_std = h->gnss_std.d, D.lever = h->lever.d;
     D.pose_prior = h->pose_prior.d, D.pose_prior_sinfo = h->pose_prior_sinfo.d, D.mix_prior = h->mix_prior.d, D.mix_prior_std = h->mix_prior_std.d;
@@ -1809,7 +1855,7 @@
     h->imu_blob.release(), h->imu_U.release(), h->gnss_blh.release(), h->gnss_std.release(), h->lever.release(), h->pose_prior.release();
     h->pose_prior_sinfo.release(), h->mix_prior.release(), h->mix_prior_std.release(), h->marg_x0.release(), h->marg_H0.release(), h->marg_b0.release();
     h->marg_c0.release(), h->lm_off.release(), h->lm_perm.release(), h->lm_fidx.release(), h->gnss_node.release();
-    h->f_meta_s.release(), h->vb_lm0.release(), h->ref_nrun.release(), h->f_const_s.release(), h->marg_type.release(), h->marg_node.release(), h->f_active.release(), h->scratch.release(), h->st_save.release(), h->cull_counters.release(), h->part_off.release(), h->pair_ro.release(), h->vis_ord.release(), h->npairs.release();
+    h->f_meta_s.release(), h->vb_lm0.release(), h->vis_bin.release(), h->vis_rng.release(), h->ref_nrun.release(), h->f_const_s.release(), h->marg_type.release(), h->marg_node.release(), h->f_active.release(), h->scratch.release(), h->st_save.release(), h->cull_counters.release(), h->part_off.release(), h->pair_ro.release(), h->vis_ord.release(), h->npairs.release();
     split_release(h);
     if (h->marg_ready) h->marg_map.release(), h->marg_oJ0.release(), h->marg_oe0.release(), h->marg_oHp.release(), h->marg_obp.release(), h->marg_fmask.release();
     for (double *p : {h->M.H0, h->M.b0, h->M.G1, h->M.V1, h->M.lam1, h->M.Z})
@@ -1831,6 +1877,49 @@
     delete h;
 }
 
+static int lin_vis_pack(int L, const int *off, const int *ref, int max_runs, int cap, int *run_lm0, int *bin_run0, int *nrun_of, int K, int *nbin) {
+    for (int k = 0; k < K; k++) nrun_of[k] = 0;
+    int nrun = 0;
+    for (int l0 = 0; l0 < L;) {
+        int l1 = l0;
+        while (l1 < L && ref[l1] == ref[l0] && off[l1 + 1] - off[l0] <= 128) l1++;
+        if (l1 == l0 || nrun >= cap) return -1 - l0;
+        if (ref[l0] >= 0) nrun_of[ref[l0]]++;
+        run_lm0[nrun++] = l0;
+        l0 = l1;
+    }
+    run_lm0[nrun] = L;
+    *nbin = 0;
+    for (int r = 0; r < nrun;) {
+        int r1 = r + 1;
+        while (r1 < nrun && off[run_lm0[r1 + 1]] - off[run_lm0[r]] <= 128 && (max_runs <= 0 || r1 - r < max_runs)) r1++;
+        bin_run0[(*nbin)++] = r;
+        r = r1;
+    }
+    bin_run0[*nbin] = nrun;
+    return nrun;
+}
+
+int icg_ba_lin_vis_bins(int L, int K, const int32_t *off, const int32_t *ref, int max_runs, int32_t *run_lm0, int32_t *bin_run0, int32_t *nrun_of,
+                        int32_t *counts) {
+    if (L < 0 || K < 1 || K > BA_MAX_NODES || max_runs < 0 || (L > 0 && (!off || !ref)) || !run_lm0 || !bin_run0 || !nrun_of || !counts) {
+        set_error("icg_ba_lin_vis_bins: bad arguments");
+        return ICG_EINVAL;
+    }
+    for (int l = 0; l < L; l++)
+        if (ref[l] < -1 || ref[l] >= K || off[l + 1] < off[l]) {
+            set_error("icg_ba_lin_vis_bins: landmark position %d is invalid", l);
+            return ICG_EINVAL;
+        }
+    const int nrun = lin_vis_pack(L, off, ref, max_runs, L, run_lm0, bin_run0, nrun_of, K, &counts[1]);
+    if (nrun < 0) {
+        set_error("icg_ba_lin_vis_bins: landmark position %d has more than 128 factors", -1 - nrun);
+        return ICG_EINVAL;
+    }
+    counts[0] = nrun;
+    return ICG_OK;
+}
+
 #define PK_FAIL(code, ...)                          \
     do {                                            \
         char eb_[512];                              \
@@ -1896,19 +1985,19 @@
             std::vector<int> cur(off, off + p.L);
             for (int f = 0; f < p.F; f++) fidx[cur[pos_of[p.f_lm[f]]]++] = f;
             int *nrun_of = h->ref_nrun.h + (size_t) w * C.K;
-            for (int k = 0; k < C.K; k++) nrun_of[k] = 0;
-            int l0 = 0;
-            while (l0 < p.L) {
-                const int ref = refof[perm[l0]];
-                int l1 = l0;
-                while (l1 < p.L && refof[perm[l1]] == ref && off[l1 + 1] - off[l0] <= 128) l1++;
-                if (l1 == l0 || nrun >= C.NVB - 2) PK_FAIL(ICG_EINVAL, "icg_ba_upload: window %d: landmark %d has more than 128 factors or the run table overflows", w, perm[l0]);
-                if (ref >= 0) nrun_of[ref]++;
-                vbh[nrun++] = l0;
-                l0 = l1;
-            }
-            vbh[nrun] = p.L;
-            vbh[C.NVB - 1] = nrun;
+            std::vector<int> refpos(p.L);
+            for (int l = 0; l < p.L; l++) refpos[l] = refof[perm[l]];
+            int *bin = h->vis_bin.h + (size_t) w * C.NVB, nbin = 0;
+            nrun = lin_vis_pack(p.L, off, refpos.data(), h->bin_max_runs, C.NVB - 2, vbh, bin, nrun_of, C.K, &nbin);
+            if (nrun < 0)
+                PK_FAIL(ICG_EINVAL, "icg_ba_upload: window %d: landmark %d has more than 128 factors or the run table overflows", w, perm[-1 - nrun]);
+            bin[C.NVB - 1] = nbin;
+            int4 *rng = h->vis_rng.h + (size_t) w * C.NVB;
+            for (int bi = 0; bi < nbin; bi++) {
+                const int a = vbh[bin[bi]], e = vbh[bin[bi + 1]];
+                rng[bi] = make_int4(a, e, off[a], off[e]);
+            }
+            rng[C.NVB - 1] = make_int4(nbin, 0, 0, 0);
             double *fcs = h->f_const_s.h + (size_t) w * C.F * 14;
             for (int q = 0; q < p.F; q++) {
                 const int f = fidx[q];
@@ -1934,8 +2023,10 @@
             poff[0] = 0;
             for (int i = 0; i < P; i++) poff[i + 1] = poff[i] + npart[i];
             std::vector<int> cur(poff, poff + P), start(p.K), pidx(p.K);
-            for (int r = 0; r < nrun; r++) {
-                const int a = off[vbh[r]], b = off[vbh[r + 1]];
+            const int *bin = h->vis_bin.h + (size_t) w * C.NVB;
+            for (int bi = 0, r = 0; r < nrun; r++) {
+                if (r == bin[bi + 1]) bi++;
+                const int a = off[vbh[r]], b = off[vbh[r + 1]], bs = off[vbh[bin[bi]]];
                 if (a == b) continue;
                 const int ref = meta[4 * a + 1];
                 std::fill(start.begin(), start.end(), 0);
@@ -1947,7 +2038,7 @@
                 }
                 for (int q = a; q < b; q++) {
                     const int k = meta[4 * q + 2];
-                    ord[a + start[k]++] = (q - a) | (pidx[k] << 8);
+                    ord[a + start[k]++] = (q - bs) | (pidx[k] << 8);
                 }
             }
             h->npairs.h[w] = P;
@@ -2037,6 +2128,8 @@
             set_error("%s", errs[t].c_str());
             return rcs[t];
         }
+    h->vis_nbin = 1;
+    for (int w = 0; w < n; w++) h->vis_nbin = std::max(h->vis_nbin, h->vis_bin.h[(size_t) w * h->C.NVB + h->C.NVB - 1]);
     return ICG_OK;
 }
 
@@ -2047,7 +2140,7 @@
 #define UP(field, stride) ICG_CUDA(h->field.up(s, nn * (size_t) (stride)))
     UP(dims, 1); UP(ext, 8);
     UP(f_active, C.F);
-    UP(f_meta_s, C.F * 4); UP(vb_lm0, C.NVB); UP(lm_off, C.L + 1); UP(lm_perm, C.L); UP(ref_nrun, C.K); UP(part_off, PM + 1); UP(pair_ro, PM); UP(vis_ord, C.F);
+    UP(f_meta_s, C.F * 4); UP(vis_rng, C.NVB); UP(lm_off, C.L + 1); UP(lm_perm, C.L); UP(ref_nrun, C.K); UP(part_off, PM + 1); UP(pair_ro, PM); UP(vis_ord, C.F);
     UP(npairs, 1); UP(gnss_node, C.G); UP(lever, 3);
     UP(pose_prior, 7); UP(pose_prior_sinfo, 6); UP(mix_prior, 9); UP(mix_prior_std, 9);
     UP(marg_type, BA_MARG_MAXB); UP(marg_node, BA_MARG_MAXB); UP(marg_x0, BA_MARG_MAXB * 9);
@@ -2092,6 +2185,15 @@
     return ICG_OK;
 }
 
+int icg_ba_set_lin_vis_bin_runs(icg_ba *h, int max_runs) {
+    if (!h || max_runs < 0) {
+        set_error("icg_ba_set_lin_vis_bin_runs: bad arguments");
+        return ICG_EINVAL;
+    }
+    h->bin_max_runs = max_runs;
+    return ICG_OK;
+}
+
 static const char *PROF_NAMES[16] = {"(gap/other)", "lin_vis", "lin_lm", "lin at candidate", "","schur_dmma (+ epilogue)", "join lin_cam + lin_done",
                                      "signal", "solve", "cost (+cost_cam)", "exchange", "accept", "reduce", "join gram chain", "step_lm", ""};
 static void prof_mark(icg_ba *h, int tag) {
@@ -2129,9 +2231,22 @@
     for (int t = 0; t < 16; t++)
         if (h->prof_cnt[t])
             fprintf(stderr, "  %-28s %9.3f ms  %8.1f us  %5.1f %%\n", PROF_NAMES[t], h->prof_ms[t], 1e3 * h->prof_ms[t] / h->prof_cnt[t], 100.0 * h->prof_ms[t] / tot);
+    {
+        long nbin = 0, nrun = 0, nf = 0;
+        for (int w = 0; w < h->cur_windows; w++) {
+            const int *bins = h->vis_bin.h + (size_t) w * h->C.NVB;
+            nbin += bins[h->C.NVB - 1], nrun += bins[bins[h->C.NVB - 1]], nf += h->dims.h[w].F;
+        }
+        fprintf(stderr, "[icg_ba profile] ba_lin_vis grid: %ld CTAs launched, %ld bins, %ld runs, %.1f factors per bin\n", (long) h->vis_nbin * h->cur_windows,
+                nbin, nrun, nbin ? (double) nf / nbin : 0.0);
+    }
     if (h->D.clk) {
-        unsigned long long ck[48];
+        unsigned long long ck[64];
         if (cudaMemcpy(ck, h->D.clk, sizeof(ck), cudaMemcpyDeviceToHost) == cudaSuccess) {
+            static const char *vn[4] = {"node frames + factor eval.", "pair Gram (DMMA)", "landmark rows / A_W", "arrival + partial sums"};
+            fprintf(stderr, "[icg_ba profile] ba_lin_vis phases of window 0 (SM cycles per CTA, mean over %llu CTAs):\n", ck[56]);
+            for (int k = 0; k < 4; k++)
+                if (ck[56 + k]) fprintf(stderr, "  %-28s %9.0f cycles\n", vn[k], (double) ck[48 + k] / (double) ck[56 + k]);
             static const char *cn[6] = {"factor evaluation", "prior product + cost", "zero H_c", "prior blocks", "IMU J^T J", "GNSS / prior diagonals"};
             fprintf(stderr, "[icg_ba profile] ba_lin_cam phases of window 0 (SM cycles per call, mean):\n");
             for (int k = 0; k < 6; k++)
@@ -2180,7 +2295,7 @@
     const BaDev &D = h->D;
     const int n = h->cur_windows;
     cudaStream_t s = h->stream;
-    const dim3 g_vis(C.NVB - 2, n);
+    const dim3 g_vis(h->vis_nbin, n);
     auto enqueue_lin = [&](int at_cand) -> int {
         ICG_CUDA(cudaEventRecord(h->ev_fork, s));
         ICG_CUDA(cudaStreamWaitEvent(h->stream_cam, h->ev_fork, 0));
@@ -2306,7 +2421,7 @@
             set_error("landmark-sharded solve: peer %d is not connected (icg_ba_shard_connect)", r);
             return ICG_EINVAL;
         }
-    const dim3 g_vis(C.NVB - 2, n), g_cost(h->nblk_vis, n), g_nn(((C.NCV + 1) * (C.NCV + 1) + 255) / 256, n);
+    const dim3 g_vis(h->vis_nbin, n), g_cost(h->nblk_vis, n), g_nn(((C.NCV + 1) * (C.NCV + 1) + 255) / 256, n);
     for (int it = 0; it <= max_num_iterations; it++) {
         const unsigned long long epoch = ++h->epoch;
         ICG_CUDA(cudaEventRecord(h->ev_fork, s));
@@ -2667,7 +2782,7 @@
     }
     const size_t smem = sizeof(double) * (8 * 480 + 2 * (size_t) C.R) + sizeof(int) * (size_t) C.R + 64;
     marg_prepare<<<(n + 127) / 128, 128, 0, s>>>(D, M, n, 0);
-    ba_lin_vis<<<dim3(C.NVB - 2, n), 128, LV_SMEM, s>>>(C, D, 0);
+    ba_lin_vis<<<dim3(h->vis_nbin, n), 128, LV_SMEM, s>>>(C, D, 0);
     marg_assemble<<<n, 256, smem, s>>>(C, D, M);
     auto jacobi = [&](int which, int nmax) -> int {
         const bool cluster_ok = nmax <= MARG_CLUSTER_MAXN && h->marg_cluster_ok == 1;
@@ -3107,8 +3222,10 @@
         const int *fidx = h->lm_fidx.h + (size_t) w * C.F;
         for (int q = 0; q < old_dims[w].F; q++) old_slot[w][fidx[q]] = q;
     }
+    const int old_nbin = h->vis_nbin;
     auto fail = [&](int code) {
         memcpy(h->dims.h, old_dims.data(), sizeof(WinDims) * n);
+        h->vis_nbin = old_nbin;
         for (int w = 0; w < n; w++) {
             int *fidx = h->lm_fidx.h + (size_t) w * C.F;
             for (int f = 0; f < old_dims[w].F; f++) fidx[old_slot[w][f]] = f;
diff --git a/include/icgvins_b200.h b/include/icgvins_b200.h
--- a/include/icgvins_b200.h
+++ b/include/icgvins_b200.h
@@ -226,6 +226,9 @@
 void icg_ba_destroy(icg_ba *h);
 int icg_ba_solve(icg_ba *h, int n_windows, const icg_ba_problem *problems, int max_num_iterations, icg_ba_summary *summaries);
 int icg_ba_upload(icg_ba *h, int n_windows, const icg_ba_problem *problems);
+int icg_ba_set_lin_vis_bin_runs(icg_ba *h, int max_runs);
+int icg_ba_lin_vis_bins(int L, int K, const int32_t *off, const int32_t *ref, int max_runs, int32_t *run_lm0, int32_t *bin_run0,
+                        int32_t *nrun_of, int32_t *counts);
 int icg_ba_run(icg_ba *h, int max_num_iterations, int restart);
 int icg_ba_download(icg_ba *h, int n_windows, const icg_ba_problem *problems, icg_ba_summary *summaries);
 int icg_ba_gvins_optimization(icg_ba *h, int n_windows, const icg_ba_problem *problems, int num_iterations, icg_ba_summary *summaries,
```

Measured after the change: 24780 (median of 6 runs). No clear change (+0.7%).
